# circletile/smvp-toolkit

Measured on AMD Instinct MI355X. Metric: fp64 CSR SpMV GFLOP/s (2*nnz flop per product; achieved HBM GB/s in roofline), higher is better.
Workload: dtype f64; 1 GPU; memplus.mtx x944 block-diagonal (substitute for the SURVEY 8(d) random model; that model: roofline.frac_sur...; format=csr, kernel=csr_stream_owner<8, 5, false>, nnz=119085600, rows=16763552, exchange=none

## Files before the change

### include/smvp_amd.h

```cpp
#ifndef SMVP_AMD_H
#define SMVP_AMD_H

#include <stddef.h>
#include <stdint.h>
#include <stdio.h>

#ifdef __cplusplus
extern "C" {
#endif

#define SMVP_VERSION_MAJOR 0
#define SMVP_VERSION_MINOR 6
#define SMVP_VERSION_REVISION 4

enum {
    SMVP_OK = 0,
    SMVP_ERR_INVALID = 1,
    SMVP_ERR_NO_DEVICE = 2,
    SMVP_ERR_HIP = 3,
    SMVP_ERR_ALLOC = 4,
    SMVP_ERR_IO = 5,
    SMVP_ERR_UNSUPPORTED = 6,
    SMVP_MM_COULD_NOT_READ_FILE = 11,
    SMVP_MM_PREMATURE_EOF = 12,
    SMVP_MM_NOT_MTX = 13,
    SMVP_MM_NO_HEADER = 14,
    SMVP_MM_UNSUPPORTED_TYPE = 15,
    SMVP_MM_LINE_TOO_LONG = 16,
    SMVP_MM_COULD_NOT_WRITE_FILE = 17
};
const char *smvp_last_error(void);
const char *smvp_version_string(void);
int smvp_set_option(const char *name, int value);
int smvp_get_option(const char *name, int *value);

typedef struct smvp_coo {
    int row;
    int col;
    double val;
} smvp_coo_t;

typedef char smvp_mm_typecode[4];

typedef struct smvp_time_stats {
    double time_total, time_avg, time_stdev, time_min, time_max;
} smvp_time_stats_t;

int smvp_mm_read_banner(FILE *f, smvp_mm_typecode *matcode);
int smvp_mm_read_mtx_crd_size(FILE *f, int *rows, int *cols, int *nnz);
int smvp_mm_read_coo_entries(FILE *f, const smvp_mm_typecode matcode, int nnz, smvp_coo_t *out);
int smvp_mm_read_header_path(const char *path, smvp_mm_typecode *matcode, int *rows, int *cols, int *nnz);
int smvp_mm_read_coo_path(const char *path, smvp_coo_t *out, int capacity,
                          smvp_mm_typecode *matcode, int *rows, int *cols, int *nnz);

int smvp_mm_expanded_count(const smvp_mm_typecode matcode, const smvp_coo_t *coo, int nnz, int *count);
int smvp_mm_expand_symmetric(const smvp_mm_typecode matcode, const smvp_coo_t *coo, int nnz, int rows, int cols,
                             smvp_coo_t *out, int capacity, int *nnz_out);

int smvp_cache_write_csr(const char *cache_path, const char *mtx_path, const smvp_mm_typecode matcode, int flags,
                         int rows, int cols, int nnz, const int *row_ptr, const int *col_ind, const double *val);
int smvp_cache_read_header(const char *cache_path, const char *mtx_path, smvp_mm_typecode *matcode, int *flags,
                           int *rows, int *cols, int *nnz);
int smvp_cache_read_csr(const char *cache_path, int rows, int nnz, int *row_ptr, int *col_ind, double *val);
int smvp_coo_from_csr(int rows, const int *row_ptr, const int *col_ind, const double *val, smvp_coo_t *out);

int smvp_csr_from_coo(const smvp_coo_t *coo, int rows, int nnz,
                      int *row_ptr, int *col_ind, double *val);
int smvp_tjds_from_coo(const smvp_coo_t *coo, int rows, int cols, int nnz,
                       int *perm, int *start_pos, int start_pos_capacity,
                       int *row_ind, double *val,
                       int *num_diag, int *ref_num_tjdiag, int *last_diag_single);

int smvp_csr_from_coo_device(const smvp_coo_t *d_coo, int rows, int cols, int nnz,
                             int *d_row_ptr, int *d_col_ind, double *d_val, void *stream);
int smvp_tjds_from_coo_device(const smvp_coo_t *d_coo, int rows, int cols, int nnz,
                              int *d_perm, int *d_start_pos, int start_pos_capacity,
                              int *d_row_ind, double *d_val,
                              int *num_diag, int *ref_num_tjdiag, int *last_diag_single, void *stream);

int smvp_device_count(int *count);
int smvp_device_info(int device, char *name, size_t name_cap, int *compute_units,
                     size_t *hbm_bytes);

enum {
    SMVP_CSR_KERNEL_AUTO = 0,
    SMVP_CSR_KERNEL_VECTOR = 1,
    SMVP_CSR_KERNEL_STREAM = 2,
    SMVP_CSR_KERNEL_STREAM_CARRY = 3,
    SMVP_CSR_KERNEL_COLSWEEP = 4,
    SMVP_CSR_KERNEL_BINNED = 5
};
enum {
    SMVP_MEM_HOST = 0,
    SMVP_MEM_DEVICE = 1
};

typedef struct smvp_csr smvp_csr_t;
typedef struct smvp_tjds smvp_tjds_t;

int smvp_csr_create(smvp_csr_t **out, int device, int rows, int cols, int nnz,
                    const int *row_ptr, const int *col_ind, const double *val,
                    int mem_kind, const int *host_row_ptr);
int smvp_csr_create_block(smvp_csr_t **out, int device, int rows, int cols, int nnz,
                          const int *row_ptr, const int *col_ind, const double *val,
                          int mem_kind, const int *host_row_ptr, long long first_row);
int smvp_csr_set_kernel(smvp_csr_t *h, int kernel, int param);
int smvp_csr_get_kernel(const smvp_csr_t *h, int *kernel, int *param);
int smvp_csr_gather_spread(smvp_csr_t *h, double *spread);
int smvp_csr_far_share(smvp_csr_t *h, double *share);
int smvp_csr_spmv(smvp_csr_t *h, const double *d_x, double *d_y, void *stream);
int smvp_csr_describe(const smvp_csr_t *h, char *kernel_name, size_t cap, double *alg_bytes);
int smvp_csr_plan_launches(const smvp_csr_t *h, int *launches);
typedef struct smvp_plan_info {
    double matrix_bytes;
    double plan_bytes;
    double build_ms;
} smvp_plan_info_t;
int smvp_csr_plan_info(const smvp_csr_t *h, smvp_plan_info_t *out);
int smvp_csr_spmm(smvp_csr_t *h, int k, const double *d_X, long long ldx, double *d_Y, long long ldy, void *stream);
int smvp_csr_spmm_describe(const smvp_csr_t *h, int k, char *kernel_name, size_t cap, double *alg_bytes, smvp_plan_info_t *plan);
int smvp_csr_create_transposed(smvp_csr_t **out, const smvp_csr_t *h, void *stream);
int smvp_csr_device_arrays(const smvp_csr_t *h, const int **d_row_ptr, const int **d_col_ind, const double **d_val);
void smvp_csr_destroy(smvp_csr_t *h);

int smvp_tjds_create(smvp_tjds_t **out, int device, int rows, int cols, int nnz, int num_diag,
                     const int *perm, const int *start_pos, const int *row_ind,
                     const double *val, int mem_kind);
int smvp_tjds_set_x(smvp_tjds_t *h, const double *d_x, void *stream);
int smvp_tjds_zero_y(smvp_tjds_t *h, double *d_y, void *stream);
int smvp_tjds_spmv(smvp_tjds_t *h, double *d_y, void *stream);
enum {
    SMVP_TJDS_MODE_AUTO = 0,
    SMVP_TJDS_MODE_ATOMIC = 1,
    SMVP_TJDS_MODE_TWO_PHASE = 2,
    SMVP_TJDS_MODE_ROW_GATHER = 3
};
int smvp_tjds_set_mode(smvp_tjds_t *h, int mode);
int smvp_tjds_set_tile(smvp_tjds_t *h, int entries_per_tile);
int smvp_tjds_set_value_cache(smvp_tjds_t *h, int min_tiles);
int smvp_tjds_get_value_cache(const smvp_tjds_t *h, int *min_tiles, long long *cached_entries);
int smvp_tjds_set_ref_quirks(smvp_tjds_t *h, int enable, int ref_num_tjdiag, int last_diag_single);
int smvp_tjds_describe(const smvp_tjds_t *h, char *kernel_name, size_t cap, double *alg_bytes);
int smvp_tjds_plan_info(const smvp_tjds_t *h, smvp_plan_info_t *out);
int smvp_tjds_spmv_transposed(smvp_tjds_t *h, const double *d_x, double *d_y, void *stream);
int smvp_tjds_transposed_describe(const smvp_tjds_t *h, char *kernel_name, size_t cap, double *alg_bytes);
int smvp_tjds_spmm_transposed(smvp_tjds_t *h, int k, const double *d_X, long long ldx, double *d_Y, long long ldy, void *stream);
int smvp_tjds_spmm_transposed_describe(const smvp_tjds_t *h, int k, char *kernel_name, size_t cap, double *alg_bytes);
int smvp_tjds_spmm(smvp_tjds_t *h, int k, const double *d_X, long long ldx, double *d_Y, long long ldy, void *stream);
int smvp_tjds_spmm_describe(const smvp_tjds_t *h, int k, char *kernel_name, size_t cap, double *alg_bytes, smvp_plan_info_t *plan);
void smvp_tjds_destroy(smvp_tjds_t *h);

typedef struct smvp_sharded smvp_sharded_t;
enum { SMVP_EXCHANGE_RCCL = 0, SMVP_EXCHANGE_COPIES = 1, SMVP_EXCHANGE_DIRECT = 2, SMVP_EXCHANGE_AUTO = 3 };
typedef struct smvp_shard_opts {
    unsigned struct_size;
    int chunks;
    int balance;
    int exchange;
} smvp_shard_opts_t;
void smvp_shard_opts_default(smvp_shard_opts_t *o);
int smvp_csr_sharded_create(smvp_sharded_t **out, int ngpus, const int *devices, int rows, int cols, int nnz,
                            const int *row_ptr, const int *col_ind, const double *val);
int smvp_csr_sharded_create_ex(smvp_sharded_t **out, int ngpus, const int *devices, int rows, int cols, int nnz,
                               const int *row_ptr, const int *col_ind, const double *val, const smvp_shard_opts_t *opts);
int smvp_tjds_sharded_create(smvp_sharded_t **out, int ngpus, const int *devices, const smvp_coo_t *coo,
                             int rows, int cols, int nnz);
int smvp_tjds_sharded_create_ex(smvp_sharded_t **out, int ngpus, const int *devices, const smvp_coo_t *coo,
                                int rows, int cols, int nnz, const smvp_shard_opts_t *opts);
int smvp_sharded_set_csr_kernel(smvp_sharded_t *h, int kernel, int param);
int smvp_sharded_probe_exchange(smvp_sharded_t *h, int reps);
int smvp_sharded_exchange_info(const smvp_sharded_t *h, int *active, int *available, double *ms, int *rccl_ranks);
int smvp_sharded_set_exchange(smvp_sharded_t *h, int exchange);
int smvp_sharded_set_x(smvp_sharded_t *h, const double *x_host);
enum { SMVP_GATHER_NONE = 0, SMVP_GATHER_OVERLAPPED = 1, SMVP_GATHER_AFTER = 2 };
int smvp_sharded_spmv(smvp_sharded_t *h, int allgather, int timed);
int smvp_sharded_synchronize(smvp_sharded_t *h, double *ms_of_last_timed_product);
int smvp_sharded_feed_back(smvp_sharded_t *h, int normalize);
int smvp_sharded_get_y(smvp_sharded_t *h, int slot, int gathered, double *y_host);
int smvp_sharded_info(const smvp_sharded_t *h, int *ngpus, int *rows_per_gpu);
int smvp_sharded_layout(const smvp_sharded_t *h, int *chunks, int *bounds, int *chunk_bounds);
void smvp_sharded_destroy(smvp_sharded_t *h);

#define SMVP_CSR_SWEEP_PARTS(rows_per_block, parts) ((rows_per_block) | (((parts) == 8 ? 3 : (parts) == 4 ? 2 : (parts) == 2 ? 1 : 0) << 24))
#define SMVP_CSR_SWEEP_PARAM(rows_per_block, parts, chunks) \
    (SMVP_CSR_SWEEP_PARTS(rows_per_block, parts) | (((chunks) == 4 ? 3 : (chunks) == 2 ? 2 : (chunks) == 1 ? 1 : 0) << 26))

typedef struct smvp_run_opts {
    unsigned struct_size;
    int device;
    int csr_kernel;
    int csr_param;
    int tjds_ref_quirks;
    int convert_on_device;
    int ngpus;
    int iterate;
    int normalize;
    int tjds_mode;
    int timing;
    int shard_exchange;
    int repeat_patience_us;
    const double *x;
} smvp_run_opts_t;
void smvp_run_opts_default(smvp_run_opts_t *o);

enum { SMVP_TIMING_AUTO = 0, SMVP_TIMING_EVENTS = 1, SMVP_TIMING_DEVICE = 2,
       SMVP_TIMING_DEVICE_GRAPH = 3  };
typedef struct smvp_run_info {
    int timing;
    int graph_replays;
    double wall_ms;
    double device_clock_khz;
    int repeat_launches;
    int repeat_gave_up;
} smvp_run_info_t;
int smvp_last_run_info(smvp_run_info_t *out);

int smvp_csr_compute(const smvp_coo_t *coo, int rows, int cols, int nnz, int iters,
                     const smvp_run_opts_t *opts, double *y, double *time_each_ms,
                     smvp_time_stats_t *stats);
int smvp_tjds_compute(const smvp_coo_t *coo, int rows, int cols, int nnz, int iters,
                      const smvp_run_opts_t *opts, double *y, double *time_each_ms,
                      smvp_time_stats_t *stats);

int smvp_time_stats(const double *time_each_ms, int iters, smvp_time_stats_t *out);
int smvp_generate_report_text(const char *input_file_name, const char *report_dir,
                              const char *alg_name, int nnz, int rows, int iters,
                              const double *y, const smvp_time_stats_t *stats,
                              unsigned long unix_time, char *out_path, size_t out_path_cap);

int smvp_cisr_coegen(const smvp_coo_t *coo, int rows, int nnz, int slots, FILE *out);
int smvp_cisr_coegen_path(const smvp_coo_t *coo, int rows, int nnz, int slots, const char *path);

enum {
    SMVP_SYNTH_MEMPLUS_SHAPED = 1,
    SMVP_SYNTH_UNIFORM = 2
};
int smvp_synth_row_lengths(int kind, uint64_t seed, int64_t rows_total, int64_t cols_total,
                           int param, int64_t row_begin, int64_t row_end, int *lens);
int smvp_synth_fill(int kind, uint64_t seed, int64_t rows_total, int64_t cols_total,
                    int param, int64_t row_begin, int64_t row_end, const int *row_ptr,
                    int *col_ind, double *val, int threads);
int smvp_partition_rows(const int *row_ptr, int rows, int parts, int *bounds);
int smvp_vector_random(double *x, int64_t n, uint64_t seed);

#ifdef __cplusplus
}
#endif
#endif
```

### smvp-toolkit_amd/csrc/smvp_engine.hip

```cpp
#include "smvp_engine.h"

#include <cmath>
#include <cstring>

using smvp::check_block_operands;
using smvp::check_device_indices;
using smvp::DeviceScope;
using smvp::kMaxEntries;
using smvp::refuse_capture;
using smvp::TjdsSource;
using smvp::to_device;
using smvp::upload;
using smvp::usable_device;
using smvp::wall_ms;

int smvp::usable_device(int device)
{
    int n = 0;
    if (hipGetDeviceCount(&n) != hipSuccess || n <= 0)
        return smvp::fail(SMVP_ERR_NO_DEVICE, "no HIP device is visible (this engine has no CPU path)");
    if (device < 0 || device >= n)
        return smvp::fail(SMVP_ERR_INVALID, "device %d out of range (%d visible)", device, n);
    return SMVP_OK;
}


struct TilePlan {
    int ntiles = 0;
    int *d_tile_row = nullptr;
    int *d_tile_next = nullptr;
    unsigned short *d_col16 = nullptr;
    int *d_col_base = nullptr;
    unsigned short *d_row_rel = nullptr;
    int *d_carry_row = nullptr;
    double *d_carry = nullptr;
    int *d_pos_sorted = nullptr, *d_meta = nullptr, *d_ovf_ptr = nullptr, *d_ovf_k = nullptr;
    double *d_ovf_val = nullptr;
    int *d_cache_ptr = nullptr;
    double *d_val_cache = nullptr;
    int cached_total = 0, ovf_total = 0;
    unsigned short *d_group_run = nullptr;
    unsigned *d_word32 = nullptr;
    int *d_run_ptr = nullptr, *d_run_tab = nullptr;
    int runs_total = 0;
    int sweep_alternate = 1, sweep_backward = 0;
};

struct SweepPlan {
    int rb = 0, per_launch = 0;
    int parts = 1;
    int g = 0;
    long long *d_ptr = nullptr;
    int *d_col = nullptr;
    double *d_val = nullptr;
    unsigned short *d_row = nullptr;
    double *d_part = nullptr;
};

struct BinnedSide {
    smvp::BinnedPlan bin;
    smvp_csr *near = nullptr;
    hipStream_t side = nullptr;
    hipEvent_t ev_fork = nullptr, ev_join = nullptr;
};

struct SpmmPlan {
    int *d_order = nullptr;
    bool planned = false;
    double build_ms = 0.0;
};

struct smvp_csr {
    int device = 0;
    int rows = 0, cols = 0, nnz = 0;
    long long row0 = 0;
    int *d_row_ptr = nullptr;
    int *d_col_ind = nullptr;
    double *d_val = nullptr;
    bool own_row_ptr = false, own_col_ind = false, own_val = false;
    std::vector<int> h_row_ptr;
    int max_row_len = 0;

    int flavor = smvp::kFlavorCsr;
    TjdsSource src;
    int cache_min_tiles = 2;
    bool plain_only = false;

    int kernel = SMVP_CSR_KERNEL_AUTO;
    int lanes_per_row = 64;
    int vpt = 4;
    bool tile_chosen = false;
    double spread = -2.0;
    double far_share = -2.0;
    double plan_build_ms = 0.0;

    TilePlan tile;
    SweepPlan sweep;
    BinnedSide binned;
    SpmmPlan spmm;
};

namespace {

void free_tile_plan(TilePlan *p)
{
    for (void *q : {(void *)p->d_tile_row, (void *)p->d_tile_next, (void *)p->d_col16, (void *)p->d_col_base, (void *)p->d_row_rel,
                    (void *)p->d_carry_row, (void *)p->d_carry, (void *)p->d_pos_sorted, (void *)p->d_meta, (void *)p->d_ovf_ptr,
                    (void *)p->d_ovf_k, (void *)p->d_ovf_val, (void *)p->d_cache_ptr, (void *)p->d_val_cache, (void *)p->d_group_run,
                    (void *)p->d_word32, (void *)p->d_run_ptr, (void *)p->d_run_tab})
        if (q)
            (void)hipFree(q);
    *p = TilePlan{};
}

void free_sweep_plan(SweepPlan *p)
{
    for (void *q : {(void *)p->d_ptr, (void *)p->d_col, (void *)p->d_val, (void *)p->d_row, (void *)p->d_part})
        if (q)
            (void)hipFree(q);
    *p = SweepPlan{};
}

void free_binned_side(BinnedSide *p)
{
    smvp_csr_destroy(p->near);
    smvp::free_binned_plan(&p->bin);
    if (p->side)
        (void)hipStreamDestroy(p->side);
    for (hipEvent_t e : {p->ev_fork, p->ev_join})
        if (e)
            (void)hipEventDestroy(e);
    *p = BinnedSide{};
}

void free_spmm_plan(SpmmPlan *p)
{
    if (p->d_order)
        (void)hipFree(p->d_order);
    *p = SpmmPlan{};
}

inline bool tile_ordered(int flavor) { return flavor == smvp::kFlavorTjdsS || flavor == smvp::kFlavorTjdsH; }
inline bool runs_on_tile_plan(int k) { return k != SMVP_CSR_KERNEL_VECTOR && k != SMVP_CSR_KERNEL_COLSWEEP && k != SMVP_CSR_KERNEL_BINNED; }
inline int owner_flavor(const smvp_csr *h) { return h->tile.d_col16 ? smvp::kFlavorCsr16 : h->flavor; }
inline double csr_matrix_bytes(const smvp_csr *h) { return 12.0 * h->nnz + 4.0 * (h->rows + 1.0); }
inline int sweep_strip_rows(const SweepPlan &s) { return (s.parts == smvp::kSweepXcdParts ? s.rb : s.rb * s.parts) / smvp::kSweepWaves; }

constexpr int kSweepMaxRb = 20480;
double sweep_rate(int rb)
{
    const struct { double lg, rate; } pts[] = {{10.0, 0.70}, {11.0, 0.80}, {12.0, 0.86}, {13.0, 1.0}, {14.32, 1.10}};
    constexpr int N = (int)(sizeof pts / sizeof pts[0]);
    const double lg = std::log2((double)std::max(rb, 1));
    if (lg <= pts[0].lg)
        return pts[0].rate * std::max(0.25, lg / pts[0].lg);
    for (int i = 0; i + 1 < N; ++i)
        if (lg <= pts[i + 1].lg)
            return pts[i].rate + (pts[i + 1].rate - pts[i].rate) * (lg - pts[i].lg) / (pts[i + 1].lg - pts[i].lg);
    return pts[N - 1].rate;
}

void choose_sweep_shape(int rows, int cols, int nnz, int want_rb, int *rb, int *per_launch)
{
    const double mean = rows > 0 ? std::max(1.0, (double)nnz / rows) : 1.0;
    int floor_rb = 1024;
    while (floor_rb < 8192 && (double)floor_rb * mean * 160.0 < (double)cols)
        floor_rb <<= 1;
    auto generations = [](int nrb) { return (nrb + 255) / 256; };
    std::vector<int> heights;
    for (int hgt : {kSweepMaxRb, 16384, 8192, 4096, 2048, 1024})
        if (hgt >= floor_rb)
            heights.push_back(hgt);
    for (int g = 1; g <= 16 && rows > 0; ++g) {
        const long long want = ((long long)rows + 256ll * g - 1) / (256ll * g);
        const int h4 = (int)std::min<long long>(kSweepMaxRb, (want + 3) / 4 * 4);
        if (h4 >= std::max(1024, floor_rb / 2))
            heights.push_back(h4);
    }
    int r = floor_rb;
    double best = -1.0;
    int best_gen = 1 << 30;
    for (int hgt : heights) {
        const int nrb = (rows + hgt - 1) / hgt;
        const int gen = std::max(1, generations(nrb));
        const double score = (double)nrb / (gen * 256.0) * sweep_rate(hgt);
        if (score > best * 1.01 || (score > best * 0.99 && gen < best_gen)) {
            best = std::max(best, score);
            best_gen = gen;
            r = hgt;
        }
    }
    if (want_rb > 0)
        r = want_rb;
    const int nrb = (rows + r - 1) / r;
    const int gen = std::max(1, generations(nrb));
    *rb = r;
    *per_launch = std::max(1, (nrb + gen - 1) / gen);
}

constexpr int kSweepPartsShift = 24, kSweepChunksShift = 26;
inline int sweep_param_rb(int param) { return param & ((1 << kSweepPartsShift) - 1); }
inline int sweep_param_parts(int param) { return 1 << ((param >> kSweepPartsShift) & 3); }
inline int sweep_param_chunks(int param) { const int c = (param >> kSweepChunksShift) & 3; return c == 3 ? 4 : c; }
bool sweep_param_ok(int param)
{
    const int rb = sweep_param_rb(param), parts = sweep_param_parts(param);
    if (param < 0 || (param >> (kSweepChunksShift + 2)) != 0)
        return false;
    if (rb == 0)
        return true;
    if (parts == smvp::kSweepXcdParts)
        return rb >= 256 && rb % 4 == 0 && rb <= kSweepMaxRb;
    return rb >= 256 && rb % 4 == 0 && (long long)rb * parts <= kSweepMaxRb;
}

int build_sweep_plan(smvp_csr *h, int want)
{
    SweepPlan &s = h->sweep;
    free_sweep_plan(&s);
    const int want_rb = sweep_param_rb(want);
    s.parts = sweep_param_parts(want);
    const bool xcd = s.parts == smvp::kSweepXcdParts;
    if (xcd) {
        int rb = want_rb;
        if (rb == 0) {
            const long long per_gen_max = 32ll * kSweepMaxRb;
            const long long gens = std::max<long long>(1, ((long long)h->rows + per_gen_max - 1) / per_gen_max);
            rb = (int)std::min<long long>(kSweepMaxRb, std::max<long long>(256, (((long long)h->rows + 32 * gens - 1) / (32 * gens) + 3) / 4 * 4));
        }
        s.rb = rb;
        s.per_launch = 256;
    } else {
        choose_sweep_shape(h->rows, h->cols, h->nnz, want_rb, &s.rb, &s.per_launch);
        while (s.parts > 1 && (long long)s.rb * s.parts > kSweepMaxRb)
            s.parts >>= 1;
    }
    const int strip_rows = sweep_strip_rows(s);
    s.g = smvp::sweep_chunks_in_flight(strip_rows, sweep_param_chunks(want));
    if (const hipError_t pe = smvp::prepare_csr_colsweep(); pe != hipSuccess)
        return smvp::fail(SMVP_ERR_HIP, "the column sweep cannot have its LDS: %s", hipGetErrorString(pe));
    const int nstrips = (h->rows + strip_rows - 1) / strip_rows;
    const size_t n = (size_t)std::max(h->nnz, 4);
    if (hipMalloc((void **)&s.d_ptr, ((size_t)nstrips * s.parts + 2) * sizeof(long long)) != hipSuccess ||
        hipMalloc((void **)&s.d_col, n * sizeof(int)) != hipSuccess ||
        hipMalloc((void **)&s.d_val, n * sizeof(double)) != hipSuccess ||
        hipMalloc((void **)&s.d_row, n * sizeof(unsigned short)) != hipSuccess ||
        (xcd && hipMalloc((void **)&s.d_part, sizeof(double) * smvp::kSweepXcdParts * (size_t)std::max(h->rows, 1)) != hipSuccess))
        return smvp::fail(SMVP_ERR_ALLOC, "cannot allocate the column-sweep plan (%d entries)", h->nnz);
    return smvp::build_colsweep_plan(h->d_row_ptr, h->d_col_ind, h->d_val, h->rows, h->cols, h->nnz, strip_rows, s.parts, smvp::kSweepChunk,
                                     smvp::kSweepRowBits, smvp::kSweepTurnCap, s.d_ptr, s.d_col, s.d_val, s.d_row, nullptr);
}

constexpr int kSpreadSamples = 64;
double csr_gather_spread(const smvp_csr *h)
{
    if ((long long)h->nnz < (long long)kSpreadSamples * smvp::kSpreadSpan || !h->d_col_ind)
        return -1.0;
    int *d_bits = nullptr;
    if (hipMalloc((void **)&d_bits, sizeof(int) * kSpreadSamples) != hipSuccess)
        return -1.0;
    int bits[kSpreadSamples];
    hipError_t e = smvp::launch_csr_line_spread(h->d_col_ind, h->nnz, kSpreadSamples, d_bits, nullptr);
    if (e == hipSuccess)
        e = hipMemcpy(bits, d_bits, sizeof bits, hipMemcpyDeviceToHost);
    (void)hipFree(d_bits);
    if (e != hipSuccess) {
        (void)hipGetLastError();
        return -1.0;
    }
    const double m = 512.0 * 1024.0;
    double lines = 0.0;
    for (int b : bits)
        lines += -m * std::log(std::max(1.0 - b / m, 1.0 / m));
    return std::min(1.0, lines / ((double)kSpreadSamples * smvp::kSpreadSpan));
}

constexpr double kSweepMinSpread = 0.6;

double measured_spread(smvp_csr *h)
{
    if (h->spread < -1.5)
        h->spread = h->flavor == smvp::kFlavorCsr ? csr_gather_spread(h) : -1.0;
    return h->spread;
}

double measured_far_share(smvp_csr *h)
{
    if (h->far_share < -1.5) {
        double share = -1.0;
        if (h->flavor != smvp::kFlavorCsr ||
            smvp::csr_far_share(h->d_row_ptr, h->d_col_ind, h->rows, h->nnz, smvp::kBinNearBand, h->row0, &share, nullptr) != SMVP_OK) {
            (void)hipGetLastError();
            share = -1.0;
        }
        h->far_share = share;
    }
    return h->far_share;
}

bool sweep_suits(smvp_csr *h)
{
    if (h->plain_only || h->flavor != smvp::kFlavorCsr || h->nnz < 4 * 1024 * 1024 || h->rows < 4096)
        return false;
    const double mean = (double)h->nnz / h->rows;
    if (mean < 4.0 || (double)h->cols * 8.0 < 8.0 * 1024 * 1024 || 8192.0 * mean * 160.0 < (double)h->cols ||
        (double)h->max_row_len > 256.0 * mean)
        return false;
    return measured_spread(h) >= kSweepMinSpread;
}

constexpr double kBinnedMinSpread = 0.2, kBinnedMinFarShare = 0.1;
bool binned_suits(smvp_csr *h)
{
    if (h->plain_only || h->flavor != smvp::kFlavorCsr || h->nnz < 4 * 1024 * 1024 || h->rows < 4096 ||
        (double)h->cols * 8.0 < 16.0 * 1024 * 1024)
        return false;
    return measured_spread(h) >= kBinnedMinSpread && measured_far_share(h) >= kBinnedMinFarShare;
}

void try_column_offsets(smvp_csr *h)
{
    if (h->flavor != smvp::kFlavorCsr || h->kernel != SMVP_CSR_KERNEL_STREAM || h->vpt < 4 || h->nnz <= 0 ||
        smvp::option("csr_col16", 1) == 0)
        return;
    std::vector<int> tiles;
    if (!h->tile_chosen && h->nnz >= 12 * 1024 * 1024)
        tiles.push_back(2048);
    tiles.push_back(smvp::kStreamBlock * h->vpt);
    const size_t max_tiles = ((size_t)h->nnz + 1023) / 1024 + 1;
    int *col_base = nullptr;
    unsigned short *col16 = nullptr;
    if (hipMalloc((void **)&col_base, max_tiles * sizeof(int)) == hipSuccess &&
        hipMalloc((void **)&col16, ((size_t)h->nnz + 8) * sizeof(unsigned short)) == hipSuccess) {
        for (int tile : tiles) {
            int fits = 0;
            if (smvp::build_column_offsets(h->d_col_ind, h->nnz, tile, col_base, col16, &fits, nullptr) == SMVP_OK && fits) {
                h->vpt = tile / smvp::kStreamBlock;
                h->tile.d_col_base = col_base;
                h->tile.d_col16 = col16;
                return;
            }
        }
    }
    (void)hipGetLastError();
    for (void *p : {(void *)col16, (void *)col_base})
        if (p)
            (void)hipFree(p);
}

constexpr double kSweepAlternateMinBytes = 256.0 * 1024 * 1024;

int build_tile_plan(smvp_csr *h)
{
    TilePlan &t = h->tile;
    free_tile_plan(&t);
    try_column_offsets(h);
    const int tile = smvp::kStreamBlock * h->vpt;
    const long long nnz = h->nnz;
    const int ntiles = (int)std::max<long long>(1, (nnz + tile - 1) / tile);
    std::vector<int> tile_row((size_t)ntiles + 1), carry_row((size_t)ntiles), tile_next((size_t)ntiles);
    const int *rp = h->h_row_ptr.data();
    int r = 0;
    for (int b = 0; b < ntiles; ++b) {
        const long long s = (long long)b * tile;
        const long long e = std::min(s + tile, nnz);
        while (r < h->rows && rp[r] < s)
            ++r;
        tile_row[(size_t)b] = r;
        const long long first = r < h->rows ? rp[r] : nnz;
        carry_row[(size_t)b] = (std::min(first, e) > s) ? r - 1 : -1;
    }
    tile_row[(size_t)ntiles] = h->rows;
    for (int b = 0; b < ntiles; ++b)
        tile_next[(size_t)b] = rp[tile_row[(size_t)b + 1]];
    if (int rc = upload(&t.d_tile_row, tile_row))
        return rc;
    if (h->kernel == SMVP_CSR_KERNEL_STREAM) {
        if (int rc = upload(&t.d_tile_next, tile_next))
            return rc;
        if (h->rows > 0 && smvp::option("csr_rowrel", 1) != 0) {
            std::vector<unsigned short> rel((size_t)h->rows);
            for (int b = 0; b < ntiles; ++b) {
                const long long s0 = (long long)b * tile;
                for (int rr = tile_row[(size_t)b]; rr < tile_row[(size_t)b + 1]; ++rr)
                    rel[(size_t)rr] = (unsigned short)(rp[rr] - s0);
            }
            if (int rc = upload(&t.d_row_rel, rel))
                return rc;
        }
    } else {
        if (int rc = upload(&t.d_carry_row, carry_row))
            return rc;
        HIP_TRY(hipMalloc((void **)&t.d_carry, std::max(ntiles, 1) * sizeof(double)));
        HIP_TRY(hipMemset(t.d_carry, 0, std::max(ntiles, 1) * sizeof(double)));
    }
    t.ntiles = ntiles;
    const int alternate = smvp::option("csr_sweep_alternate", -1);
    t.sweep_alternate = alternate < 0 ? 12.0 * (double)h->nnz + 12.0 * h->rows + 8.0 * h->cols > kSweepAlternateMinBytes : alternate != 0;
    if (tile_ordered(h->flavor)) {
        std::vector<int> ovf_ptr((size_t)ntiles + 1, 0);
        for (int b = 0; b < ntiles; ++b) {
            const long long e = std::min((long long)(b + 1) * tile, nnz);
            const bool owns = tile_row[(size_t)b] != tile_row[(size_t)b + 1];
            ovf_ptr[(size_t)b + 1] = ovf_ptr[(size_t)b] + (owns ? (int)(tile_next[(size_t)b] - e) : 0);
        }
        const int total = ovf_ptr[(size_t)ntiles];
        t.ovf_total = total;
        if (int rc = upload(&t.d_ovf_ptr, ovf_ptr))
            return rc;
        const size_t n = (size_t)std::max(h->nnz, 4), m = (size_t)std::max(total, 4);
        const bool half = h->flavor == smvp::kFlavorTjdsH;
        const TjdsSource &src = h->src;
        if (hipMalloc((void **)&t.d_ovf_val, m * sizeof(double)) != hipSuccess ||
            hipMalloc((void **)&t.d_ovf_k, m * sizeof(int)) != hipSuccess ||
            hipMalloc((void **)&t.d_cache_ptr, ((size_t)ntiles + 2) * sizeof(int)) != hipSuccess ||
            hipMalloc(half ? (void **)&t.d_word32 : (void **)&t.d_pos_sorted, n * sizeof(int)) != hipSuccess ||
            hipMalloc(half ? (void **)&t.d_run_ptr : (void **)&t.d_meta, (half ? (size_t)ntiles + 2 : n) * sizeof(int)) != hipSuccess)
            return smvp::fail(SMVP_ERR_ALLOC, "cannot allocate the tile-ordered TJDS streams");
        if (int rc = half ? smvp::build_tile_half_streams(src.pos, h->nnz, tile, src.start_pos, src.num_diag, h->d_val, h->cache_min_tiles,
                                                          t.d_word32, t.d_cache_ptr, t.d_run_ptr, &t.d_val_cache, &t.d_run_tab,
                                                          &t.d_group_run, &t.cached_total, &t.runs_total, nullptr)
                          : smvp::sort_tile_windows(src.pos, h->nnz, tile, src.start_pos, src.num_diag, smvp::kSlotBits, h->d_val,
                                                    h->cache_min_tiles, t.d_pos_sorted, t.d_meta, t.d_cache_ptr, &t.d_val_cache,
                                                    &t.cached_total, nullptr))
            return rc;
        if (int rc = smvp::build_tile_overflow(src.pos, t.d_ovf_ptr, total, ntiles, tile, h->nnz, src.start_pos, src.num_diag, h->d_val,
                                               t.d_ovf_val, t.d_ovf_k, src.unit_operand ? 1 : 0, nullptr))
            return rc;
    }
    return SMVP_OK;
}

int pow2_at_least(double v)
{
    int p = 2;
    while (p < 64 && p < v)
        p <<= 1;
    return p;
}

constexpr int kOwnerMaxRow = 16 * 1024;

bool choose_csr_kernel(smvp_csr *h, int kernel, int param)
{
    const double mean = h->rows > 0 ? (double)h->nnz / h->rows : 0.0;
    if (kernel == SMVP_CSR_KERNEL_AUTO)
        kernel = h->max_row_len > kOwnerMaxRow ? SMVP_CSR_KERNEL_STREAM_CARRY
                 : sweep_suits(h)              ? SMVP_CSR_KERNEL_COLSWEEP
                 : binned_suits(h)             ? SMVP_CSR_KERNEL_BINNED
                                               : SMVP_CSR_KERNEL_STREAM;
    if (kernel == SMVP_CSR_KERNEL_STREAM && param != 0 && param != 256 && param != 1024 && param != 2048)
        return false;
    if (kernel == SMVP_CSR_KERNEL_STREAM_CARRY && param != 0 && param != 1024 && param != 2048)
        return false;
    if (kernel == SMVP_CSR_KERNEL_COLSWEEP && !sweep_param_ok(param))
        return false;
    if (kernel == SMVP_CSR_KERNEL_BINNED && param < 0)
        return false;
    h->kernel = kernel;
    if (kernel == SMVP_CSR_KERNEL_COLSWEEP || kernel == SMVP_CSR_KERNEL_BINNED)
        return true;
    if (kernel == SMVP_CSR_KERNEL_VECTOR) {
        h->lanes_per_row = param > 0 ? param : pow2_at_least(mean);
    } else {
        int tile = param > 0 ? param : 0;
        h->tile_chosen = param > 0;
        if (tile == 0) {
            tile = (kernel == SMVP_CSR_KERNEL_STREAM && h->nnz < 512 * 1024) ? 256 : 1024;
            if ((tile_ordered(h->flavor)) && tile == 1024 && h->nnz >= 12 * 1024 * 1024)
                tile = 2048;
        }
        h->vpt = tile / smvp::kStreamBlock;
    }
    return true;
}

}

static int csr_create_impl(smvp_csr_t **out, int device, int rows, int cols, int nnz, const int *row_ptr, const int *col_ind, const double *val,
                           int mem_kind, const int *host_row_ptr, int flavor, const TjdsSource *src = nullptr, bool plain_only = false,
                           long long first_row = 0);

static int build_binned(smvp_csr *h, int band)
{
    free_binned_side(&h->binned);
    if (hipError_t le = smvp::binned_reserve_lds(); le != hipSuccess) {
        (void)hipGetLastError();
        return smvp::fail(SMVP_ERR_UNSUPPORTED, "the binned plan needs 154 KB of LDS per workgroup: %s", hipGetErrorString(le));
    }
    const bool window = smvp::option("binned_near", 0) == 0;
    if (int rc = smvp::build_binned_plan(h->d_row_ptr, h->d_col_ind, h->d_val, h->rows, h->cols, h->nnz, band, h->row0, window, &h->binned.bin, nullptr))
        return rc;
    if (h->binned.bin.nw.on) {
        if (smvp::option("binned_overlap", 1) != 0 && h->binned.bin.nf > 0) {
            HIP_TRY(hipStreamCreateWithFlags(&h->binned.side, hipStreamNonBlocking));
            HIP_TRY(hipEventCreateWithFlags(&h->binned.ev_fork, hipEventDisableTiming));
            HIP_TRY(hipEventCreateWithFlags(&h->binned.ev_join, hipEventDisableTiming));
        }
        return SMVP_OK;
    }
    return csr_create_impl(&h->binned.near, h->device, h->rows, h->cols, h->binned.bin.nnz_near, h->binned.bin.near_ptr, h->binned.bin.near_col, h->binned.bin.near_val,
                           SMVP_MEM_DEVICE, nullptr, smvp::kFlavorCsr, nullptr, true, h->row0);
}

static int plan_csr(smvp_csr *h, int kernel, int param, bool silent_fallback)
{
    if (!choose_csr_kernel(h, kernel, param))
        return smvp::fail(SMVP_ERR_INVALID, "entries per tile must be 256 (stream only), 1024 or 2048 for the kernel "
                                            "this matrix resolves to (column sweep: 256 ... 20480 rows per block, a multiple of 4; binned: the near band, >= 0)");
    const double t0 = wall_ms();
    free_sweep_plan(&h->sweep);
    free_binned_side(&h->binned);
    int rc = SMVP_OK;
    if (runs_on_tile_plan(h->kernel)) {
        rc = build_tile_plan(h);
    } else {
        free_tile_plan(&h->tile);
        if (h->kernel != SMVP_CSR_KERNEL_VECTOR)
            rc = h->kernel == SMVP_CSR_KERNEL_COLSWEEP ? build_sweep_plan(h, param) : build_binned(h, param);
        if (rc != SMVP_OK) {
            const std::string why = smvp_last_error();
            (void)hipGetLastError();
            free_sweep_plan(&h->sweep);
            free_binned_side(&h->binned);
            h->spread = -1.0;
            choose_csr_kernel(h, SMVP_CSR_KERNEL_STREAM, 0);
            const int tile_rc = build_tile_plan(h);
            if (tile_rc != SMVP_OK)
                free_tile_plan(&h->tile);
            rc = silent_fallback ? tile_rc : smvp::fail(rc, "%s", why.c_str());
        }
    }
    h->plan_build_ms = wall_ms() - t0;
    return rc;
}

static int csr_create_impl(smvp_csr_t **out, int device, int rows, int cols, int nnz, const int *row_ptr, const int *col_ind, const double *val,
                           int mem_kind, const int *host_row_ptr, int flavor, const TjdsSource *src, bool plain_only, long long first_row)
{
    const bool plain = flavor == smvp::kFlavorCsr;
    if (!out || rows < 0 || cols < 0 || nnz < 0 || !row_ptr ||
        (nnz > 0 && ((!col_ind && !tile_ordered(flavor)) || !val)))
        return smvp::fail(SMVP_ERR_INVALID, "smvp_csr_create: bad argument");
    if (mem_kind != SMVP_MEM_HOST && mem_kind != SMVP_MEM_DEVICE)
        return smvp::fail(SMVP_ERR_INVALID, "smvp_csr_create: bad mem_kind");
    if (nnz > kMaxEntries)
        return smvp::fail(SMVP_ERR_UNSUPPORTED, "smvp_csr_create: %d entries: shard blocks this large by rows", nnz);
    if (int rc = usable_device(device))
        return rc;
    DeviceScope on(device);

    smvp_csr *h = new smvp_csr;
    h->device = device;
    h->flavor = flavor;
    h->plain_only = plain_only;
    h->row0 = first_row;
    if (src)
        h->src = *src;
    if (h->src.unit_operand)
        h->cache_min_tiles = 0;
    h->rows = rows, h->cols = cols, h->nnz = nnz;
    h->h_row_ptr.resize((size_t)rows + 1);
    int rc = SMVP_OK;
    if (mem_kind == SMVP_MEM_HOST || host_row_ptr) {
        memcpy(h->h_row_ptr.data(), mem_kind == SMVP_MEM_HOST ? row_ptr : host_row_ptr, sizeof(int) * ((size_t)rows + 1));
    } else if (hipMemcpy(h->h_row_ptr.data(), row_ptr, sizeof(int) * ((size_t)rows + 1), hipMemcpyDeviceToHost) != hipSuccess) {
        rc = smvp::fail(SMVP_ERR_HIP, "smvp_csr_create: cannot read row_ptr back from the device");
    }
    if (rc == SMVP_OK) {
        const std::vector<int> &rp = h->h_row_ptr;
        bool ok = rp[0] == 0 && rp[(size_t)rows] == nnz;
        for (int r = 0; r < rows && ok; ++r) {
            ok = rp[(size_t)r] <= rp[(size_t)r + 1];
            h->max_row_len = std::max(h->max_row_len, rp[(size_t)r + 1] - rp[(size_t)r]);
        }
        if (!ok)
            rc = smvp::fail(SMVP_ERR_INVALID, "smvp_csr_create: row_ptr is not a non-decreasing 0..nnz sequence");
    }
    if (rc == SMVP_OK && mem_kind == SMVP_MEM_HOST) {
        for (int j = 0; j < nnz; ++j)
            if (col_ind[j] < 0 || col_ind[j] >= cols) {
                rc = smvp::fail(SMVP_ERR_INVALID, "smvp_csr_create: col_ind[%d] = %d outside [0, %d)", j, col_ind[j], cols);
                break;
            }
    }
    if (rc == SMVP_OK && mem_kind == SMVP_MEM_DEVICE &&
        (((uintptr_t)col_ind | (plain ? (uintptr_t)val : 0)) & 15u) != 0)
        rc = smvp::fail(SMVP_ERR_INVALID, "smvp_csr_create: adopted device arrays must be 16-byte aligned");
    if (rc == SMVP_OK && mem_kind == SMVP_MEM_DEVICE && col_ind)
        rc = check_device_indices(col_ind, nnz, cols, "smvp_csr_create: col_ind");
    if (rc == SMVP_OK)
        rc = to_device(&h->d_row_ptr, row_ptr, (size_t)rows + 1, mem_kind, &h->own_row_ptr);
    if (rc == SMVP_OK && col_ind)
        rc = to_device(&h->d_col_ind, col_ind, (size_t)nnz, mem_kind, &h->own_col_ind);
    if (rc == SMVP_OK)
        rc = to_device(&h->d_val, val, (size_t)nnz, mem_kind, &h->own_val);
    if (rc == SMVP_OK) {
        const double t0 = wall_ms();
        rc = plan_csr(h, plain ? SMVP_CSR_KERNEL_AUTO : SMVP_CSR_KERNEL_STREAM, 0, true);
        h->plan_build_ms = wall_ms() - t0;
    }
    if (rc != SMVP_OK) {
        smvp_csr_destroy(h);
        return rc;
    }
    *out = h;
    return SMVP_OK;
}

int smvp::csr_create_tjds(smvp_csr_t **out, int device, int rows, int cols, int nnz, const int *d_row_ptr, const int *d_col_ind,
                          const double *d_val, int flavor, const TjdsSource &src)
{
    return csr_create_impl(out, device, rows, cols, nnz, d_row_ptr, d_col_ind, d_val, SMVP_MEM_DEVICE, nullptr, flavor, &src);
}

bool smvp::csr_value_cache(const smvp_csr_t *h, int *min_tiles, long long *cached_entries)
{
    const bool on = h && tile_ordered(h->flavor);
    if (min_tiles)
        *min_tiles = on ? h->cache_min_tiles : 0;
    if (cached_entries)
        *cached_entries = on ? h->tile.cached_total : 0;
    return on;
}

int smvp::csr_replan_value_cache(smvp_csr_t *h, int min_tiles)
{
    h->cache_min_tiles = min_tiles;
    return build_tile_plan(h);
}

extern "C" int smvp_csr_create(smvp_csr_t **out, int device, int rows, int cols, int nnz,
                               const int *row_ptr, const int *col_ind, const double *val,
                               int mem_kind, const int *host_row_ptr)
{
    return csr_create_impl(out, device, rows, cols, nnz, row_ptr, col_ind, val, mem_kind, host_row_ptr, smvp::kFlavorCsr);
}

extern "C" int smvp_csr_create_block(smvp_csr_t **out, int device, int rows, int cols, int nnz,
                                     const int *row_ptr, const int *col_ind, const double *val,
                                     int mem_kind, const int *host_row_ptr, long long first_row)
{
    if (first_row < 0)
        return smvp::fail(SMVP_ERR_INVALID, "smvp_csr_create_block: first_row < 0");
    return csr_create_impl(out, device, rows, cols, nnz, row_ptr, col_ind, val, mem_kind, host_row_ptr, smvp::kFlavorCsr, nullptr,
                           false, first_row);
}

extern "C" int smvp_csr_far_share(smvp_csr_t *h, double *share)
{
    if (!h || !share)
        return smvp::fail(SMVP_ERR_INVALID, "smvp_csr_far_share: bad argument");
    DeviceScope on(h->device);
    *share = measured_far_share(h);
    return SMVP_OK;
}

extern "C" int smvp_csr_set_kernel(smvp_csr_t *h, int kernel, int param)
{
    if (!h)
        return smvp::fail(SMVP_ERR_INVALID, "null handle");
    if (h->flavor != smvp::kFlavorCsr && kernel != SMVP_CSR_KERNEL_STREAM)
        return smvp::fail(SMVP_ERR_UNSUPPORTED, "this matrix flavour runs on the stream kernel only");
    if (kernel < SMVP_CSR_KERNEL_AUTO || kernel > SMVP_CSR_KERNEL_BINNED)
        return smvp::fail(SMVP_ERR_INVALID, "unknown CSR kernel %d", kernel);
    if (kernel == SMVP_CSR_KERNEL_VECTOR && param != 0 &&
        (param < 2 || param > 64 || (param & (param - 1)) != 0))
        return smvp::fail(SMVP_ERR_INVALID, "lanes per row must be a power of two in [2, 64]");
    DeviceScope on(h->device);
    h->spread = h->far_share = -2.0;
    return plan_csr(h, kernel, param, false);
}

extern "C" int smvp_csr_get_kernel(const smvp_csr_t *h, int *kernel, int *param)
{
    if (!h)
        return smvp::fail(SMVP_ERR_INVALID, "null handle");
    if (kernel)
        *kernel = h->kernel;
    if (param)
        *param = h->kernel == SMVP_CSR_KERNEL_VECTOR ? h->lanes_per_row
                 : h->kernel == SMVP_CSR_KERNEL_COLSWEEP ? (h->sweep.rb | ((h->sweep.parts == 8 ? 3 : h->sweep.parts == 4 ? 2 : h->sweep.parts == 2 ? 1 : 0) << kSweepPartsShift))
                 : h->kernel == SMVP_CSR_KERNEL_BINNED   ? h->binned.bin.band
                                                         : h->vpt * smvp::kStreamBlock;
    return SMVP_OK;
}

extern "C" int smvp_csr_gather_spread(smvp_csr_t *h, double *spread)
{
    if (!h || !spread)
        return smvp::fail(SMVP_ERR_INVALID, "smvp_csr_gather_spread: bad argument");
    DeviceScope on(h->device);
    *spread = measured_spread(h);
    return SMVP_OK;
}

static void fill_owner_launch(const smvp_csr_t *h, const double *d_x, double *d_y, unsigned long long *stamps, smvp::OwnerLaunch *out)
{
    smvp::OwnerLaunch &l = *out;
    l.row_ptr = h->d_row_ptr, l.col_ind = h->d_col_ind, l.val = h->d_val, l.x = d_x, l.y = d_y;
    l.tile_row = h->tile.d_tile_row, l.tile_next = h->tile.d_tile_next;
    l.pos = h->src.pos, l.start_pos = h->src.start_pos;
    if (tile_ordered(h->flavor)) {
        l.pos = h->tile.d_pos_sorted, l.col_ind = h->tile.d_meta;
        l.ovf_ptr = h->tile.d_ovf_ptr, l.ovf_val = h->tile.d_ovf_val, l.ovf_k = h->tile.d_ovf_k;
        l.cache_ptr = h->tile.d_cache_ptr, l.val_cache = h->tile.d_val_cache;
        l.word32 = h->tile.d_word32, l.group_run = h->tile.d_group_run, l.run_ptr = h->tile.d_run_ptr, l.run_tab = h->tile.d_run_tab;
    }
    l.stamps = stamps;
    l.rows = h->rows, l.nnz = h->nnz, l.ntiles = h->tile.ntiles;
    l.col16 = h->tile.d_col16, l.col_base = h->tile.d_col_base;
    l.row_rel = h->tile.d_row_rel;
    l.unit_x = h->src.unit_operand ? 1 : 0;
}

int smvp::csr_repeat_grid(const smvp_csr_t *h)
{
    if (!h || h->kernel != SMVP_CSR_KERNEL_STREAM || !h->tile.d_tile_row || h->rows <= 0)
        return 0;
    DeviceScope on(h->device);
    return smvp::owner_repeat_grid(h->vpt, owner_flavor(h), h->tile.ntiles);
}

int smvp::csr_spmv_repeat(smvp_csr_t *h, const double *d_x, double *d_y, void *stream, unsigned long long *stamps, int reps, int grid,
                          unsigned *ctl_words, bool first_of_run, unsigned long long patience)
{
    DeviceScope on(h->device);
    smvp::OwnerLaunch l{};
    fill_owner_launch(h, d_x, d_y, stamps, &l);
    const hipError_t e = smvp::launch_csr_stream_owner_repeat(h->vpt, owner_flavor(h), l, reps, grid, ctl_words,
                                                              first_of_run, patience, (hipStream_t)stream);
    if (e != hipSuccess)
        return smvp::fail(SMVP_ERR_HIP, "repeating CSR launch failed: %s", hipGetErrorString(e));
    return SMVP_OK;
}

static int launched(hipError_t e)
{
    return e == hipSuccess ? (int)SMVP_OK : smvp::fail(SMVP_ERR_HIP, "CSR launch failed: %s", hipGetErrorString(e));
}

int smvp::csr_spmv_stamped(smvp_csr_t *h, const double *d_x, double *d_y, void *stream, unsigned long long *stamps)
{
    if (!h || (h->rows > 0 && !d_y) || (h->nnz > 0 && !d_x))
        return smvp::fail(SMVP_ERR_INVALID, "smvp_csr_spmv: bad argument");
    if ((h->kernel == SMVP_CSR_KERNEL_COLSWEEP && !h->sweep.d_ptr) || (h->kernel == SMVP_CSR_KERNEL_BINNED && !h->binned.near && !h->binned.bin.nw.on) ||
        (runs_on_tile_plan(h->kernel) && !h->tile.d_tile_row))
        return smvp::fail(SMVP_ERR_INVALID, "smvp_csr_spmv: the handle has no launch plan (a re-plan failed earlier)");
    DeviceScope on(h->device);
    hipStream_t st = (hipStream_t)stream;
    hipError_t e;
    if (h->kernel == SMVP_CSR_KERNEL_BINNED) {
        if (h->binned.bin.nw.on && h->binned.side) {
            HIP_TRY(hipEventRecord(h->binned.ev_fork, st));
            HIP_TRY(hipStreamWaitEvent(h->binned.side, h->binned.ev_fork, 0));
            if (int rc = launched(smvp::launch_binned_products(h->binned.bin, d_x, h->binned.side)))
                return rc;
            int rc = SMVP_OK;
            hipError_t je = hipEventRecord(h->binned.ev_join, h->binned.side);
            if (je == hipSuccess) {
                rc = launched(smvp::launch_near_window(h->binned.bin.nw, d_x, d_y, st));
                je = hipStreamWaitEvent(st, h->binned.ev_join, 0);
            }
            if (je != hipSuccess) {
                (void)hipStreamSynchronize(h->binned.side);
                return smvp::fail(SMVP_ERR_HIP, "joining the binned plan's side stream failed: %s", hipGetErrorString(je));
            }
            if (rc != SMVP_OK)
                return rc;
            return launched(smvp::launch_binned_sums(h->binned.bin, d_y, st));
        }
        if (h->binned.bin.nw.on) {
            if (int rc = launched(smvp::launch_near_window(h->binned.bin.nw, d_x, d_y, st)))
                return rc;
        } else if (int rc = smvp::csr_spmv_stamped(h->binned.near, d_x, d_y, stream, nullptr))
            return rc;
        if (int rc = launched(smvp::launch_binned_products(h->binned.bin, d_x, st)))
            return rc;
        e = smvp::launch_binned_sums(h->binned.bin, d_y, st);
    } else if (h->kernel == SMVP_CSR_KERNEL_COLSWEEP)
        e = smvp::launch_csr_colsweep(h->sweep.d_ptr, h->sweep.d_col, h->sweep.d_val, h->sweep.d_row, d_x, d_y, h->rows,
                                      sweep_strip_rows(h->sweep), h->sweep.parts, h->sweep.per_launch, h->sweep.g, h->sweep.d_part, st);
    else if (h->kernel == SMVP_CSR_KERNEL_VECTOR)
        e = smvp::launch_csr_vector(h->lanes_per_row, h->d_row_ptr, h->d_col_ind, h->d_val, d_x, d_y, h->rows, st);
    else if (h->kernel == SMVP_CSR_KERNEL_STREAM) {
        smvp::OwnerLaunch l{};
        fill_owner_launch(h, d_x, d_y, stamps, &l);
        l.backward = h->tile.sweep_backward;
        h->tile.sweep_backward = h->tile.sweep_alternate ? !l.backward : 0;
        e = smvp::launch_csr_stream_owner(h->vpt, owner_flavor(h), l, st);
    } else
        e = smvp::launch_csr_stream(h->vpt, h->d_row_ptr, h->d_col_ind, h->d_val, d_x, d_y, h->tile.d_tile_row,
                                    h->tile.d_carry_row, h->tile.d_carry, h->rows, h->nnz, h->tile.ntiles, st);
    return launched(e);
}

extern "C" int smvp_csr_spmv(smvp_csr_t *h, const double *d_x, double *d_y, void *stream)
{
    return smvp::csr_spmv_stamped(h, d_x, d_y, stream, nullptr);
}

int smvp::csr_stamp_slots(const smvp_csr_t *h)
{
    return h && h->kernel == SMVP_CSR_KERNEL_STREAM && h->tile.d_tile_row ? smvp::owner_stamp_slots(h->tile.ntiles, h->flavor) : 0;
}

std::string smvp::csr_owner_kernel_name(const smvp_csr_t *h)
{
    char name[64];
    snprintf(name, sizeof name, "csr_stream_owner<%d, %d, false>", h ? h->vpt : 0, h ? owner_flavor(h) : 0);
    return name;
}

extern "C" int smvp_csr_describe(const smvp_csr_t *h, char *kernel_name, size_t cap, double *alg_bytes)
{
    if (!h)
        return smvp::fail(SMVP_ERR_INVALID, "null handle");
    if (kernel_name && cap) {
        if (h->kernel == SMVP_CSR_KERNEL_BINNED && h->binned.bin.nw.on)
            snprintf(kernel_name, cap, "csr_binned: csr_near_window + csr_binned_far_products<2> + csr_binned_far_sums<%d, %d, 2>", h->binned.bin.slots,
                     h->binned.bin.threads_b);
        else if (h->kernel == SMVP_CSR_KERNEL_BINNED)
            snprintf(kernel_name, cap, "csr_binned: %s + csr_binned_far_products<2> + csr_binned_far_sums<%d, %d, 2>",
                     smvp::csr_owner_kernel_name(h->binned.near).c_str(), h->binned.bin.slots, h->binned.bin.threads_b);
        else if (h->kernel == SMVP_CSR_KERNEL_COLSWEEP)
            if (h->sweep.parts == smvp::kSweepXcdParts)
                snprintf(kernel_name, cap, "csr_colsweep<%d> (8 column parts, one per XCD) + sweep_combine", h->sweep.g);
            else if (h->sweep.parts > 1)
                snprintf(kernel_name, cap, "csr_colsweep<%d> (%d column parts)", h->sweep.g, h->sweep.parts);
            else
                snprintf(kernel_name, cap, "csr_colsweep<%d>", h->sweep.g);
        else if (h->kernel == SMVP_CSR_KERNEL_VECTOR)
            snprintf(kernel_name, cap, "csr_vector_rows<%d>", h->lanes_per_row);
        else if (h->kernel == SMVP_CSR_KERNEL_STREAM)
            snprintf(kernel_name, cap, "%s", smvp::csr_owner_kernel_name(h).c_str());
        else
            snprintf(kernel_name, cap, "csr_stream_tiles<%d>", h->vpt);
    }
    if (alg_bytes)
        *alg_bytes = csr_matrix_bytes(h) + 8.0 * h->cols + 8.0 * h->rows;
    return SMVP_OK;
}

extern "C" int smvp_csr_plan_launches(const smvp_csr_t *h, int *launches)
{
    if (!h || !launches)
        return smvp::fail(SMVP_ERR_INVALID, "smvp_csr_plan_launches: bad argument");
    *launches = 1;
    if (h->kernel == SMVP_CSR_KERNEL_COLSWEEP && h->sweep.rb > 0 && h->sweep.per_launch > 0) {
        const bool xcd = h->sweep.parts == smvp::kSweepXcdParts;
        const int nwg = (h->rows + h->sweep.rb - 1) / h->sweep.rb * (xcd ? smvp::kSweepXcdParts : 1);
        *launches = std::max(1, (nwg + h->sweep.per_launch - 1) / h->sweep.per_launch) + (xcd ? 1 : 0);
    } else if (h->kernel == SMVP_CSR_KERNEL_STREAM_CARRY && h->tile.ntiles > 1) {
        *launches = 2;
    } else if (h->kernel == SMVP_CSR_KERNEL_BINNED && h->binned.bin.nw.on) {
        *launches = 1 + (h->binned.bin.nw.n_out > 0 ? 1 : 0) + (h->binned.bin.nf > 0 ? 2 : 0);
    } else if (h->kernel == SMVP_CSR_KERNEL_BINNED && h->binned.near) {
        int near = 1;
        (void)smvp_csr_plan_launches(h->binned.near, &near);
        *launches = near + (h->binned.bin.nf > 0 ? 2 : 0);
    }
    return SMVP_OK;
}

double smvp::csr_plan_bytes(const smvp_csr_t *h)
{
    const double n = h->nnz, t = h->tile.ntiles;
    if (h->kernel == SMVP_CSR_KERNEL_BINNED)
        return (double)h->binned.bin.plan_bytes + (h->binned.near ? smvp::csr_plan_bytes(h->binned.near) : 0.0);
    if (h->kernel == SMVP_CSR_KERNEL_COLSWEEP) {
        const bool xcd = h->sweep.parts == smvp::kSweepXcdParts;
        const int strip_rows = std::max(1, sweep_strip_rows(h->sweep));
        return 14.0 * n + 8.0 * ((double)((h->rows + strip_rows - 1) / strip_rows) * h->sweep.parts + 2) + (xcd ? 64.0 * h->rows : 0.0);
    }
    if (h->kernel == SMVP_CSR_KERNEL_VECTOR)
        return 0.0;
    double b = 4.0 * (t + 1) + 4.0 * t;
    if (h->kernel == SMVP_CSR_KERNEL_STREAM_CARRY)
        b += 8.0 * t;
    if (h->tile.d_col16)
        b += 2.0 * n + 4.0 * (n / 1024 + 1);
    if (h->tile.d_row_rel)
        b += 2.0 * h->rows;
    if (tile_ordered(h->flavor)) {
        b += 4.0 * (t + 1) + 12.0 * h->tile.ovf_total + 4.0 * (t + 2) + 8.0 * h->tile.cached_total;
        b += h->flavor == smvp::kFlavorTjdsH ? 4.0 * n + 4.0 * (t + 2) + 8.0 * h->tile.runs_total + 2.0 * (n / 32 + 1) : 8.0 * n;
    }
    return b;
}

extern "C" int smvp_csr_plan_info(const smvp_csr_t *h, smvp_plan_info_t *out)
{
    if (!h || !out)
        return smvp::fail(SMVP_ERR_INVALID, "smvp_csr_plan_info: bad argument");
    out->matrix_bytes = csr_matrix_bytes(h);
    out->plan_bytes = smvp::csr_plan_bytes(h);
    out->build_ms = h->plan_build_ms;
    return SMVP_OK;
}

extern "C" int smvp_csr_spmm(smvp_csr_t *h, int k, const double *d_X, long long ldx, double *d_Y, long long ldy, void *stream)
{
    if (!h)
        return smvp::fail(SMVP_ERR_INVALID, "smvp_csr_spmm: null handle");
    if (h->flavor != smvp::kFlavorCsr)
        return smvp::fail(SMVP_ERR_UNSUPPORTED, "smvp_csr_spmm: plain CSR handles only (this one belongs to a TJDS matrix)");
    if (int rc = check_block_operands("smvp_csr_spmm", k, d_X, ldx, h->cols, d_Y, ldy, h->rows, h->nnz))
        return rc;
    DeviceScope on(h->device);
    hipStream_t st = (hipStream_t)stream;
    if (!h->spmm.planned) {
        if (int rc = refuse_capture(st, "smvp_csr_spmm: the first call on a handle builds its plan and cannot be captured "
                                        "(call it once outside the capture)"))
            return rc;
        const double t0 = wall_ms();
        int *order = h->spmm.d_order;
        if (h->rows > 0 && !order && hipMalloc((void **)&order, sizeof(int) * (size_t)h->rows) != hipSuccess)
            return smvp::fail(SMVP_ERR_ALLOC, "smvp_csr_spmm: cannot allocate the plan (%d rows)", h->rows);
        h->spmm.d_order = order;
        if (int rc = smvp::build_spmm_order(h->d_row_ptr, h->rows, h->max_row_len, h->spmm.d_order, st))
            return rc;
        h->spmm.planned = true;
        h->spmm.build_ms = wall_ms() - t0;
    }
    const hipError_t e = smvp::launch_csr_spmm(h->d_row_ptr, h->d_col_ind, h->d_val, h->spmm.d_order, d_X, ldx, d_Y, ldy, h->rows, k, st);
    if (e != hipSuccess)
        return smvp::fail(SMVP_ERR_HIP, "smvp_csr_spmm: launch failed: %s", hipGetErrorString(e));
    return SMVP_OK;
}

extern "C" int smvp_csr_spmm_describe(const smvp_csr_t *h, int k, char *kernel_name, size_t cap, double *alg_bytes, smvp_plan_info_t *plan)
{
    if (!h)
        return smvp::fail(SMVP_ERR_INVALID, "smvp_csr_spmm_describe: null handle");
    if (h->flavor != smvp::kFlavorCsr)
        return smvp::fail(SMVP_ERR_UNSUPPORTED, "smvp_csr_spmm_describe: plain CSR handles only");
    if (k < 1)
        return smvp::fail(SMVP_ERR_INVALID, "smvp_csr_spmm_describe: k = %d (need k >= 1)", k);
    if (kernel_name && cap)
        smvp::spmm_kernel_name(k, kernel_name, cap);
    if (alg_bytes)
        *alg_bytes = csr_matrix_bytes(h) + 8.0 * k * ((double)h->cols + h->rows);
    if (plan) {
        plan->matrix_bytes = csr_matrix_bytes(h);
        plan->plan_bytes = h->spmm.planned ? 4.0 * h->rows : 0.0;
        plan->build_ms = h->spmm.planned ? h->spmm.build_ms : 0.0;
    }
    return SMVP_OK;
}

extern "C" int smvp_csr_device_arrays(const smvp_csr_t *h, const int **d_row_ptr, const int **d_col_ind, const double **d_val)
{
    if (!h)
        return smvp::fail(SMVP_ERR_INVALID, "smvp_csr_device_arrays: null handle");
    if (h->flavor != smvp::kFlavorCsr)
        return smvp::fail(SMVP_ERR_UNSUPPORTED, "smvp_csr_device_arrays: plain CSR handles only (this one belongs to a TJDS matrix)");
    if (d_row_ptr)
        *d_row_ptr = h->d_row_ptr;
    if (d_col_ind)
        *d_col_ind = h->d_col_ind;
    if (d_val)
        *d_val = h->d_val;
    return SMVP_OK;
}

extern "C" int smvp_csr_create_transposed(smvp_csr_t **out, const smvp_csr_t *h, void *stream)
{
    if (out)
        *out = nullptr;
    if (!out || !h)
        return smvp::fail(SMVP_ERR_INVALID, "smvp_csr_create_transposed: null %s", out ? "handle" : "out");
    if (h->flavor != smvp::kFlavorCsr)
        return smvp::fail(SMVP_ERR_UNSUPPORTED, "smvp_csr_create_transposed: plain CSR handles only (this one belongs to a TJDS matrix)");
    DeviceScope on(h->device);
    hipStream_t st = (hipStream_t)stream;
    if (int rc = refuse_capture(st, "smvp_csr_create_transposed: allocates and synchronises, so it cannot be captured "
                                    "(the stream is capturing)"))
        return rc;
    const int t_rows = h->cols, t_cols = h->rows, nnz = h->nnz;
    int *t_row_ptr = nullptr, *t_col_ind = nullptr;
    double *t_val = nullptr;
    smvp_coo_t *coo = nullptr;
    auto release = [&]() {
        for (void *p : {(void *)t_row_ptr, (void *)t_col_ind, (void *)t_val, (void *)coo})
            if (p)
                (void)hipFree(p);
    };
    if (hipMalloc((void **)&t_row_ptr, sizeof(int) * ((size_t)t_rows + 4)) != hipSuccess ||
        hipMalloc((void **)&t_col_ind, sizeof(int) * std::max<size_t>((size_t)nnz, 4)) != hipSuccess ||
        hipMalloc((void **)&t_val, sizeof(double) * std::max<size_t>((size_t)nnz, 4)) != hipSuccess ||
        hipMalloc((void **)&coo, sizeof(smvp_coo_t) * std::max<size_t>((size_t)nnz, 4)) != hipSuccess) {
        (void)hipGetLastError();
        release();
        return smvp::fail(SMVP_ERR_ALLOC, "smvp_csr_create_transposed: cannot allocate the transposed arrays and the entry list (%d entries)", nnz);
    }
    int rc = SMVP_OK;
    const hipError_t e = smvp::launch_csr_swapped_coo(h->d_row_ptr, h->d_col_ind, h->d_val, h->rows, nnz, coo, st);
    if (e != hipSuccess)
        rc = smvp::fail(SMVP_ERR_HIP, "smvp_csr_create_transposed: launch failed: %s", hipGetErrorString(e));
    if (rc == SMVP_OK) {
        rc = smvp_csr_from_coo_device(coo, t_rows, t_cols, nnz, t_row_ptr, t_col_ind, t_val, stream);
        if (rc == SMVP_ERR_HIP && strstr(smvp_last_error(), "out of memory")) {
            (void)hipGetLastError();
            rc = smvp::fail(SMVP_ERR_ALLOC, "smvp_csr_create_transposed: cannot allocate the sort's buffers (%d entries)", nnz);
        }
    }
    if (rc != SMVP_OK)
        (void)hipStreamSynchronize(st);
    (void)hipFree(coo);
    coo = nullptr;
    smvp_csr_t *t = nullptr;
    if (rc == SMVP_OK)
        rc = csr_create_impl(&t, h->device, t_rows, t_cols, nnz, t_row_ptr, t_col_ind, t_val, SMVP_MEM_DEVICE, nullptr, smvp::kFlavorCsr);
    if (rc != SMVP_OK) {
        release();
        return rc;
    }
    t->own_row_ptr = t->own_col_ind = t->own_val = true;
    *out = t;
    return SMVP_OK;
}

extern "C" void smvp_csr_destroy(smvp_csr_t *h)
{
    if (!h)
        return;
    DeviceScope on(h->device);
    smvp::debug_owner_phases();
    smvp::debug_binned_phases();
    free_tile_plan(&h->tile);
    free_sweep_plan(&h->sweep);
    free_binned_side(&h->binned);
    free_spmm_plan(&h->spmm);
    if (h->own_row_ptr && h->d_row_ptr)
        (void)hipFree(h->d_row_ptr);
    if (h->own_col_ind && h->d_col_ind)
        (void)hipFree(h->d_col_ind);
    if (h->own_val && h->d_val)
        (void)hipFree(h->d_val);
    delete h;
}
```

### smvp-toolkit_amd/csrc/smvp_error.cpp

```cpp
#include "smvp_common.h"

#include <atomic>
#include <cstring>

namespace {
thread_local char g_err[512] = "";
}

namespace smvp {
int fail(int code, const char *fmt, ...)
{
    va_list ap;
    va_start(ap, fmt);
    vsnprintf(g_err, sizeof g_err, fmt, ap);
    va_end(ap);
    return code;
}
void clear_error() { g_err[0] = '\0'; }
}

extern "C" const char *smvp_last_error(void) { return g_err; }

extern "C" const char *smvp_version_string(void)
{
    static char v[32];
    snprintf(v, sizeof v, "%d.%d.%d", SMVP_VERSION_MAJOR, SMVP_VERSION_MINOR, SMVP_VERSION_REVISION);
    return v;
}

namespace {
struct Option { const char *name; std::atomic<int> value; };
Option g_options[] = {
    {"csr_col16", {-1}},
    {"csr_rowrel", {-1}},
    {"csr_sweep_alternate", {-1}},
    {"binned_near", {-1}},
    {"binned_overlap", {-1}},
    {"tjds_index", {-1}},
    {"sharded_threads", {-1}},
    {"mm_threads", {-1}},
};
Option *find_option(const char *name)
{
    if (name)
        for (Option &o : g_options)
            if (!strcmp(o.name, name))
                return &o;
    return nullptr;
}
}

namespace smvp {
int option(const char *name, int fallback)
{
    const Option *o = find_option(name);
    const int v = o ? o->value.load(std::memory_order_relaxed) : -1;
    return v < 0 ? fallback : v;
}
}

extern "C" int smvp_set_option(const char *name, int value)
{
    Option *o = find_option(name);
    if (!o)
        return smvp::fail(SMVP_ERR_INVALID, "smvp_set_option: no option called '%s'", name ? name : "(null)");
    o->value.store(value < 0 ? -1 : value, std::memory_order_relaxed);
    return SMVP_OK;
}

extern "C" int smvp_get_option(const char *name, int *value)
{
    const Option *o = find_option(name);
    if (!o || !value)
        return smvp::fail(SMVP_ERR_INVALID, "smvp_get_option: no option called '%s'", name ? name : "(null)");
    *value = o->value.load(std::memory_order_relaxed);
    return SMVP_OK;
}
```

### smvp-toolkit_amd/csrc/smvp_kernels.h

```cpp
#pragma once
#include <hip/hip_runtime.h>

#include "smvp_amd.h"
#include "smvp_tile_map.h"

namespace smvp {

constexpr int kVectorBlock = 256;
constexpr int kStreamBlock = 256;
constexpr int kLongRow = 32;
constexpr int kStreamOver = 1024;
constexpr int kStreamTileGroup = 64;
constexpr int kTjdsTileGroup = 32;
constexpr int kSweepBlock = 256;
constexpr int kSweepWaves = kSweepBlock / 64;
constexpr int kSweepUnroll = 4;
constexpr int kSweepChunk = 64 * kSweepUnroll;
constexpr int kSweepXcdParts = 8;
constexpr int kSweepRowBits = 13;
constexpr int kSweepTurnCap = (1 << (16 - kSweepRowBits)) - 1;
constexpr int kTjdsBlock = 256;
constexpr int kTjdsDiagChunk = 8;

constexpr int kSpmmMaxVectors = 16;
constexpr int kSpmmBlockRows = 4096;
int build_spmm_order(const int *row_ptr, int rows, int longest_row, int *order, hipStream_t stream);
hipError_t launch_csr_spmm(const int *row_ptr, const int *col_ind, const double *val, const int *order, const double *X,
                           long long ldx, double *Y, long long ldy, int rows, int k, hipStream_t stream);
void spmm_kernel_name(int k, char *name, size_t cap);

hipError_t launch_tjds_transposed(const int *start_pos, const int *row_ind, const double *val, const int *perm, const double *x,
                                  double *y, int cols, int num_diag, hipStream_t stream);
const char *tjds_transposed_kernel_name();
hipError_t launch_tjds_spmm_transposed(const int *start_pos, const int *row_ind, const double *val, const int *perm, const double *X,
                                       long long ldx, double *Y, long long ldy, int cols, int num_diag, int k, hipStream_t stream);
void tjds_spmm_transposed_kernel_name(int k, char *name, size_t cap);
int build_tjds_spmm_plan(const int *row_ind, const int *start_pos, const int *perm, int num_diag, int nnz, int rows, int *ptr,
                         int *pos, int *col, int *order, hipStream_t stream);
hipError_t launch_tjds_spmm(const int *ptr, const int *pos, const int *col, const double *val, const int *order, const double *X,
                            long long ldx, double *Y, long long ldy, int rows, int k, hipStream_t stream);
void tjds_spmm_kernel_name(int k, char *name, size_t cap);
hipError_t launch_csr_swapped_coo(const int *row_ptr, const int *col_ind, const double *val, int rows, int nnz, smvp_coo_t *coo,
                                  hipStream_t stream);

hipError_t launch_csr_vector(int lanes_per_row, const int *row_ptr, const int *col_ind, const double *val,
                             const double *x, double *y, int rows, hipStream_t stream);
hipError_t launch_csr_stream(int vpt, const int *row_ptr, const int *col_ind, const double *val,
                             const double *x, double *y, const int *tile_row, const int *carry_row,
                             double *carry, int rows, int nnz, int ntiles, hipStream_t stream);
constexpr int kFlavorCsr = 0;
constexpr int kFlavorTjdsK = 2;
constexpr int kFlavorTjdsS = 3;
constexpr int kFlavorTjdsH = 4;
constexpr int kFlavorCsr16 = 5;
constexpr int kSlotBits = 11;

struct OwnerLaunch {
    const int *row_ptr = nullptr, *col_ind = nullptr;
    const double *val = nullptr, *x = nullptr;
    double *y = nullptr;
    const int *tile_row = nullptr, *tile_next = nullptr;
    const int *pos = nullptr;
    const int *start_pos = nullptr;
    unsigned long long *stamps = nullptr;
    const int *ovf_ptr = nullptr, *ovf_k = nullptr;
    const double *ovf_val = nullptr;
    const int *cache_ptr = nullptr;
    const double *val_cache = nullptr;
    const unsigned short *col16 = nullptr;
    const int *col_base = nullptr;
    const unsigned short *group_run = nullptr;
    const unsigned *word32 = nullptr;
    int unit_x = 0;
    const int *run_ptr = nullptr, *run_tab = nullptr;
    const unsigned short *row_rel = nullptr;
    int rows = 0, nnz = 0, ntiles = 0;
    int backward = 0;
};
hipError_t launch_csr_stream_owner(int vpt, int flavor, const OwnerLaunch &l, hipStream_t stream);
void debug_owner_phases();
void debug_binned_phases();
int owner_stamp_slots(int ntiles, int flavor);
constexpr int kRepeatCtlWords = 32 * 66;
constexpr unsigned kRepeatPatienceDefaultUs = 50000;
int owner_repeat_grid(int vpt, int flavor, int ntiles);
hipError_t launch_owner_csr_ilp(int vpt, int flavor, const OwnerLaunch &l, const void *extra, unsigned grid_x, int group, hipStream_t stream);
hipError_t launch_csr_stream_owner_repeat(int vpt, int flavor, const OwnerLaunch &l, int reps, int grid, unsigned *ctl_words,
                                          bool first_of_run, unsigned long long patience_ticks, hipStream_t stream);
inline unsigned long long repeat_patience_ticks(int us) { return us < 0 ? 0ull : 100ull * (unsigned)(us ? us : (int)kRepeatPatienceDefaultUs); }
hipError_t launch_stamp_reduce(const unsigned long long *stamps, int slots_per_product, int products,
                               unsigned long long *first_last, hipStream_t stream);
hipError_t launch_tjds_products(const int *start_pos, const double *val, const double *x_perm, double *prod,
                                const int4 *work, int nwork, int cols, hipStream_t stream);
hipError_t launch_tjds_scatter(bool operand_by_row, const int *start_pos, const int *row_ind, const double *val,
                               const double *x_perm, double *y, const int4 *work, int nwork, int cols,
                               hipStream_t stream);
hipError_t launch_tjds_permute(const int *perm, const double *x, double *x_perm, int cols, hipStream_t stream);
hipError_t launch_find_out_of_range(const int *a, long long n, int limit, int *bad, hipStream_t stream);
hipError_t launch_normalize_max(double *v, long long n, unsigned long long *scratch, hipStream_t stream);
hipError_t launch_fill(double *p, double v, long long n, hipStream_t stream);

hipError_t launch_csr_colsweep(const long long *strip_ptr, const int *e_col, const double *e_val, const unsigned short *e_row,
                               const double *x, double *y, int rows, int strip_rows, int parts, int per_launch, int g, double *ypart,
                               hipStream_t stream);
hipError_t prepare_csr_colsweep();
int sweep_chunks_in_flight(int strip_rows, int asked);
constexpr int kSpreadSpan = 64 * 1024;
hipError_t launch_csr_line_spread(const int *col_ind, long long nnz, int samples, int *distinct, hipStream_t stream);

constexpr int kBinColBits = 14;
constexpr int kBinSlots = 8192;
constexpr int kBinRowCap = 1024;
constexpr int kBinBucket = kBinSlots - kBinRowCap;
constexpr int kBinThreads = 1024;
constexpr int kBinShiftCap = 1024;
constexpr int kBinNearBand = 4096;

struct BinnedStream {
    int groups = 0, padded = 0, cells = 0;
    unsigned short *word = nullptr;
    int *chunk = nullptr;
    int *ptr = nullptr;
    int *shift_ptr = nullptr;
    int *shift = nullptr;
};

constexpr int kNwRowBlock = 8192;
constexpr int kNwBand = 4096;
constexpr int kNwShortCap = 16;
constexpr int kNwLongCap = 1024;
struct NearWindow {
    bool on = false;
    int rows = 0, cols = 0, nblocks = 0, n_out = 0;
    long long row0 = 0;
    long long slots = 0;
    int *wave_ptr = nullptr;
    int *wave_n1 = nullptr, *wave_n2 = nullptr;
    unsigned short *perm16 = nullptr;
    double *sval = nullptr;
    unsigned short *sword = nullptr;
    int *blk_long_ptr = nullptr;
    unsigned short *long_row16 = nullptr;
    int *out_row = nullptr, *out_ptr = nullptr, *out_col = nullptr;
    double *out_val = nullptr;
    size_t plan_bytes = 0;
};
void free_near_window(NearWindow *p);
int build_near_window(const int *near_ptr, const int *near_col, const double *near_val, const int *capped, int rows, int cols,
                      int nnz_near, int band, long long row0, NearWindow *out, hipStream_t stream);
hipError_t launch_near_window(const NearWindow &p, const double *x, double *y, hipStream_t stream);

struct BinnedPlan {
    int band = kBinNearBand;
    long long row0 = 0;
    int rows = 0, cols = 0, nnz = 0, nnz_near = 0, nf = 0;
    int ncb = 0, nrb = 0, q = 1, nfr = 0, splits = 1;
    int slots = kBinSlots, threads_b = kBinThreads;
    int *near_ptr = nullptr, *near_col = nullptr;
    double *near_val = nullptr;
    NearWindow nw;
    double *a_val = nullptr;
    BinnedStream a, b;
    double *bins = nullptr;
    int *fr_row = nullptr, *fr_ptr = nullptr, *blk_fr = nullptr;
    int4 *b_desc = nullptr;
    unsigned *fr32 = nullptr;
    size_t plan_bytes = 0;
};
void free_binned_plan(BinnedPlan *p);
int build_binned_plan(const int *d_row_ptr, const int *d_col_ind, const double *d_val, int rows, int cols, int nnz, int band,
                      long long row0, bool near_window, BinnedPlan *out, hipStream_t stream);
hipError_t binned_reserve_lds();
hipError_t near_window_reserve_lds();
hipError_t launch_binned_products(const BinnedPlan &p, const double *x, hipStream_t stream);
hipError_t launch_binned_sums(const BinnedPlan &p, double *y, hipStream_t stream);
int csr_far_share(const int *d_row_ptr, const int *d_col_ind, int rows, int nnz, int band, long long row0, double *share, hipStream_t stream);

template <int N>
__device__ __forceinline__ double dpp_row_shl(double v)
{
    int lo = __double2loint(v), hi = __double2hiint(v);
    lo = __builtin_amdgcn_update_dpp(0, lo, 0x100 + N, 0xf, 0xf, true);
    hi = __builtin_amdgcn_update_dpp(0, hi, 0x100 + N, 0xf, 0xf, true);
    return __hiloint2double(hi, lo);
}

__device__ __forceinline__ double wave_sum_dpp(double v)
{
#if defined(__HIP_DEVICE_COMPILE__) && !defined(__GFX9__)
#error "wave_sum_dpp: four DPP rows of 16 lanes = one wave64 (gfx9 / CDNA only)"
#endif
    v += dpp_row_shl<8>(v);
    v += dpp_row_shl<4>(v);
    v += dpp_row_shl<2>(v);
    v += dpp_row_shl<1>(v);
    const int lo = __double2loint(v), hi = __double2hiint(v);
    double r[4];
#pragma unroll
    for (int k = 0; k < 4; ++k)
        r[k] = __hiloint2double(__builtin_amdgcn_readlane(hi, 16 * k), __builtin_amdgcn_readlane(lo, 16 * k));
    return (r[0] + r[1]) + (r[2] + r[3]);
}


}
```

### smvp-toolkit_amd/csrc/smvp_kernels.hip

```cpp
#include "smvp_kernels.h"

#include <algorithm>
#include <cstdio>
#include <cstdlib>

namespace smvp {

template <int WIDTH>
__device__ __forceinline__ double shfl_down_sum(double v)
{
#pragma unroll
    for (int off = WIDTH / 2; off > 0; off >>= 1)
        v += __shfl_down(v, off, WIDTH);
    return v;
}


#ifndef SMVP_TU_ILP
template <int T>
__global__ __launch_bounds__(kVectorBlock) void csr_vector_rows(
    const int *__restrict__ row_ptr, const int *__restrict__ col_ind, const double *__restrict__ val,
    const double *__restrict__ x, double *__restrict__ y, int rows, int row0)
{
    const long long gid = (long long)blockIdx.x * kVectorBlock + threadIdx.x;
    const long long row = row0 + gid / T;
    const int lane = threadIdx.x & (T - 1);
    int a = 0, z = 0;
    if (row < rows) {
        a = row_ptr[row];
        z = row_ptr[row + 1];
    }
    double acc = 0.0;
    for (int j = a + lane; j < z; j += T)
        acc += val[j] * x[col_ind[j]];
    acc = shfl_down_sum<T>(acc);
    if (lane == 0 && row < rows)
        y[row] = acc;
}

template <int VPT>
__global__ __launch_bounds__(kStreamBlock) void csr_stream_tiles(
    const int *__restrict__ row_ptr, const int *__restrict__ col_ind, const double *__restrict__ val,
    const double *__restrict__ x, double *__restrict__ y, const int *__restrict__ tile_row,
    double *__restrict__ carry, int rows, int nnz, int ntiles, int tile_group)
{
    constexpr int TILE = kStreamBlock * VPT;
    constexpr int QCAP = TILE / kLongRow + 1;
    __shared__ double prod[TILE];
    __shared__ int long_rows[QCAP];
    __shared__ int long_count;

    const int b = tile_of_block(blockIdx.x, tile_group);
    if (b >= ntiles)
        return;
    const int t = threadIdx.x;
    const long long s = (long long)b * TILE;
    const int e = (int)(s + TILE < (long long)nnz ? s + TILE : (long long)nnz);
    if (t == 0)
        long_count = 0;
    const int rlo = tile_row[b];
    const int rhi = tile_row[b + 1];

    const long long j0 = s + (long long)t * VPT;
    double p[VPT];
    if (j0 + VPT <= (long long)nnz) {
        int c[VPT];
        double v[VPT];
#pragma unroll
        for (int k = 0; k < VPT; k += 4)
            *reinterpret_cast<int4 *>(&c[k]) = *reinterpret_cast<const int4 *>(col_ind + j0 + k);
#pragma unroll
        for (int k = 0; k < VPT; k += 2)
            *reinterpret_cast<double2 *>(&v[k]) = *reinterpret_cast<const double2 *>(val + j0 + k);
#pragma unroll
        for (int k = 0; k < VPT; ++k)
            p[k] = v[k] * x[c[k]];
    } else {
#pragma unroll
        for (int k = 0; k < VPT; ++k)
            p[k] = (j0 + k < (long long)nnz) ? val[j0 + k] * x[col_ind[j0 + k]] : 0.0;
    }
#pragma unroll
    for (int k = 0; k < VPT; k += 2)
        *reinterpret_cast<double2 *>(&prod[t * VPT + k]) = make_double2(p[k], p[k + 1]);
    __syncthreads();

    const int lo = (int)s;
    if (t < 64) {
        const int first = rlo < rows ? row_ptr[rlo] : nnz;
        const int head = (first < e ? first : e) - lo;
        double acc = 0.0;
        for (int i = t; i < head; i += 64)
            acc += prod[i];
        acc = shfl_down_sum<64>(acc);
        if (t == 0)
            carry[b] = acc;
    }

    for (int r = rlo + t; r < rhi; r += kStreamBlock) {
        const int a = row_ptr[r];
        const int nxt = row_ptr[r + 1];
        const int z = nxt < e ? nxt : e;
        if (z - a <= kLongRow) {
            double acc = 0.0;
            for (int i = a - lo; i < z - lo; ++i)
                acc += prod[i];
            y[r] = acc;
        } else {
            long_rows[atomicAdd(&long_count, 1)] = r;
        }
    }
    __syncthreads();

    const int nlong = long_count;
    const int lane = t & 63;
    for (int q = t >> 6; q < nlong; q += kStreamBlock / 64) {
        const int r = long_rows[q];
        const int a = row_ptr[r];
        const int nxt = row_ptr[r + 1];
        const int z = nxt < e ? nxt : e;
        double acc = 0.0;
        for (int i = a - lo + lane; i < z - lo; i += 64)
            acc += prod[i];
        acc = shfl_down_sum<64>(acc);
        if (lane == 0)
            y[r] = acc;
    }
}

#endif
typedef int int4v __attribute__((ext_vector_type(4)));

struct OwnerExtra {
    const int *pos = nullptr;
    const int *start_pos = nullptr;
    const int *ovf_ptr = nullptr;
    const double *ovf_val = nullptr;
    const int *ovf_k = nullptr;
    const int *cache_ptr = nullptr;
    const double *val_cache = nullptr;
    const unsigned short *col16 = nullptr;
    const int *col_base = nullptr;
    const unsigned *word32 = nullptr;
    const unsigned short *group_run = nullptr;
    const int *run_ptr = nullptr;
    const int *run_tab = nullptr;
    int unit_x = 0;
    const unsigned short *row_rel = nullptr;
    unsigned long long *stamps = nullptr;
    int back_grid = 0;
};

[[maybe_unused]] static inline OwnerExtra owner_extra_of(const OwnerLaunch &l, unsigned long long *stamps)
{
    OwnerExtra ex{};
    ex.pos = l.pos, ex.start_pos = l.start_pos, ex.ovf_ptr = l.ovf_ptr, ex.ovf_val = l.ovf_val, ex.ovf_k = l.ovf_k;
    ex.cache_ptr = l.cache_ptr, ex.val_cache = l.val_cache;
    ex.col16 = l.col16, ex.col_base = l.col_base;
    ex.unit_x = l.unit_x, ex.word32 = l.word32, ex.group_run = l.group_run, ex.run_ptr = l.run_ptr, ex.run_tab = l.run_tab;
    ex.row_rel = l.row_rel;
    ex.stamps = stamps;
    return ex;
}

struct OwnerArgs {
    const int *__restrict__ col_ind;
    const double *__restrict__ val;
    const double *__restrict__ x;
    const int *__restrict__ pos;
    const int *__restrict__ start_pos;
    const double *__restrict__ ovf_val;
    const int *__restrict__ ovf_k;
    int unit_x;
};

template <int FLAVOR>
__device__ __forceinline__ double owner_product_slow(const OwnerArgs &a, long long j)
{
    if constexpr (FLAVOR == kFlavorCsr || FLAVOR == kFlavorCsr16)
        return a.val[j] * a.x[a.col_ind[j]];
    else if constexpr (FLAVOR == kFlavorTjdsK)
        return a.val[a.pos[j]] * a.x[a.col_ind[j]];
    else {
        const int p = a.pos[j];
        return a.val[p] * a.x[p - a.start_pos[(unsigned)a.col_ind[j] >> kSlotBits]];
    }
}

template <int FLAVOR>
__device__ __forceinline__ double owner_overflow_product(const OwnerArgs &a, int ovf_base, int e, int i)
{
    if constexpr (FLAVOR == kFlavorTjdsS || FLAVOR == kFlavorTjdsH)
        return a.unit_x ? a.val[a.ovf_k[ovf_base + i]] : a.ovf_val[ovf_base + i] * a.x[a.ovf_k[ovf_base + i]];
    else
        return owner_product_slow<FLAVOR>(a, (long long)e + i);
}

#if defined(SMVP_PHASE_STAMPS) && defined(SMVP_TU_ILP)
#undef SMVP_PHASE_STAMPS
#define SMVP_ILP_UNIT_UNUSED
#endif
#ifdef SMVP_PHASE_STAMPS
__device__ unsigned long long g_owner_phase[8];
#define SMVP_PHASE(n)                                                                        \
    do {                                                                                     \
        if (threadIdx.x == 0 && (blockIdx.x & 127) == 5) {                                   \
            const unsigned long long now_ = wall_clock64();                                  \
            if ((n) > 0)                                                                     \
                atomicAdd(&g_owner_phase[(n)-1], now_ - phase_prev_);                        \
            else                                                                             \
                atomicAdd(&g_owner_phase[7], 1ull);                                          \
            phase_prev_ = now_;                                                              \
        }                                                                                    \
    } while (0)
#else
#define SMVP_PHASE(n) do { } while (0)
#endif

#ifndef SMVP_TJDS_NEUTRALISE
#define SMVP_TJDS_NEUTRALISE 0
#endif

template <int VPT, int FLAVOR, bool STAMPED>
__device__ __forceinline__ void owner_body(
    const int *__restrict__ row_ptr, const int *__restrict__ col_ind, const double *__restrict__ val,
    const double *__restrict__ x, double *__restrict__ y, const int *__restrict__ tile_row,
    const int *__restrict__ tile_next, int rows, int nnz_arg, int ntiles, int tile_group_arg, const OwnerExtra &ex, const int block)
{
    const OwnerArgs a = {col_ind, val, x, ex.pos, ex.start_pos, ex.ovf_val, ex.ovf_k, FLAVOR == kFlavorTjdsH ? ex.unit_x : 0};
    constexpr int TILE = kStreamBlock * VPT;
    constexpr int QCAP = (TILE + kStreamOver) / kLongRow + 1;
    constexpr bool CSR = FLAVOR == kFlavorCsr || FLAVOR == kFlavorCsr16;
    constexpr bool COL16 = FLAVOR == kFlavorCsr16;
    constexpr bool HALF = FLAVOR == kFlavorTjdsH;
    constexpr bool TJDS = FLAVOR == kFlavorTjdsK || FLAVOR == kFlavorTjdsS || HALF;
    constexpr bool SORTED = FLAVOR == kFlavorTjdsS || HALF;
    static_assert(TILE <= (1 << kSlotBits), "slot bits");
    __shared__ double prod[TILE + kStreamOver];
    __shared__ int long_rows[QCAP];
    __shared__ int long_a[QCAP];
    __shared__ int long_z[QCAP];
    __shared__ int long_count;
    __shared__ double wave_sum[kStreamBlock / 64];

    const int t = threadIdx.x;
#ifdef SMVP_PHASE_STAMPS
    unsigned long long phase_prev_ = 0;
#endif
    unsigned long long *stamp = nullptr;
    if constexpr (STAMPED) {
        stamp = ex.stamps + 2 * ((size_t)block * (kStreamBlock / 64) + (t >> 6));
        if ((t & 63) == 0)
            stamp[0] = wall_clock64();
    }
#define SMVP_OWNER_EXIT()                                         \
    do {                                                          \
        if constexpr (STAMPED) {                                  \
            asm volatile("s_waitcnt vmcnt(0)" ::: "memory");      \
            if ((t & 63) == 0)                                    \
                stamp[1] = wall_clock64();                        \
        }                                                         \
        return;                                                   \
    } while (0)

    const int b = tile_of_block_swept(block, tile_group_arg, ex.back_grid);
    if (b >= ntiles)
        SMVP_OWNER_EXIT();
    const int nnz = nnz_arg;
    const long long s = (long long)b * TILE;
    const long long j0 = s + (long long)t * VPT;

    const bool whole = j0 + VPT <= (long long)nnz;
    int c[VPT];
    int pj[VPT];
    double v[VPT];
    const bool full_tile = s + TILE <= (long long)nnz;
    int grp[HALF ? VPT : 1];
    int run0 = 0;
    int2 run_tbl = make_int2(0, 0);
    if constexpr (HALF) {
        if (full_tile) {
            run0 = ex.run_ptr[b];
            const int nruns = ex.run_ptr[b + 1] - run0;
            const int ln = t & 63;
            if (ln < nruns)
                run_tbl = reinterpret_cast<const int2 *>(ex.run_tab)[run0 + ln];
        }
    }
    if constexpr (HALF) {
        if (full_tile) {
#pragma unroll
            for (int k = 0; k < VPT; ++k) {
                if constexpr (VPT == 1) {
                    pj[k] = (int)ex.word32[s + k * kStreamBlock + t];
                } else {
                    pj[k] = (int)__builtin_nontemporal_load(ex.word32 + s + k * kStreamBlock + t);
                }
                const unsigned gw = reinterpret_cast<const unsigned *>(ex.group_run)[((size_t)b * (TILE / 32) + k * (kStreamBlock / 32) +
                                                                                     2 * __builtin_amdgcn_readfirstlane(t >> 6)) >> 1];
                grp[k] = (t & 32) ? (int)(gw >> 16) : (int)(gw & 0xffffu);
            }
        }
    } else if constexpr (SORTED) {
        if (full_tile) {
#pragma unroll
            for (int k = 0; k < VPT; ++k) {
                if constexpr (VPT > 1) {
                    pj[k] = __builtin_nontemporal_load(a.pos + s + k * kStreamBlock + t);
                    c[k] = __builtin_nontemporal_load(a.col_ind + s + k * kStreamBlock + t);
                } else {
                    pj[k] = a.pos[s + k * kStreamBlock + t];
                    c[k] = a.col_ind[s + k * kStreamBlock + t];
                }
            }
        }
    } else if (whole) {
        if constexpr (VPT >= 4) {
            if constexpr (COL16) {
                const int base = ex.col_base[b];
                if (base >= 0) {
#pragma unroll
                    for (int k = 0; k < VPT; k += 4) {
                        const uint2 w = *reinterpret_cast<const uint2 *>(ex.col16 + j0 + k);
                        c[k] = base + (int)(w.x & 0xffffu), c[k + 1] = base + (int)(w.x >> 16);
                        c[k + 2] = base + (int)(w.y & 0xffffu), c[k + 3] = base + (int)(w.y >> 16);
                    }
                } else {
#pragma unroll
                    for (int k = 0; k < VPT; k += 4)
                        *reinterpret_cast<int4 *>(&c[k]) = *reinterpret_cast<const int4 *>(a.col_ind + j0 + k);
                }
            } else {
#pragma unroll
                for (int k = 0; k < VPT; k += 4)
                    *reinterpret_cast<int4 *>(&c[k]) = *reinterpret_cast<const int4 *>(a.col_ind + j0 + k);
            }
            if constexpr (TJDS) {
#pragma unroll
                for (int k = 0; k < VPT; k += 4)
                    *reinterpret_cast<int4v *>(&pj[k]) = __builtin_nontemporal_load(reinterpret_cast<const int4v *>(a.pos + j0 + k));
            }
            if constexpr (CSR) {
#pragma unroll
                for (int k = 0; k < VPT; k += 2)
                    *reinterpret_cast<double2 *>(&v[k]) = *reinterpret_cast<const double2 *>(a.val + j0 + k);
            }
        } else {
            c[0] = a.col_ind[j0];
            if constexpr (TJDS)
                pj[0] = a.pos[j0];
            if constexpr (CSR)
                v[0] = a.val[j0];
        }
    }
    const int rlo = tile_row[b];
    const int rhi = tile_row[b + 1];
    if (rlo == rhi)
        SMVP_OWNER_EXIT();
    SMVP_PHASE(0);
    const int lo = (int)s;
    const int e = (int)(s + TILE < (long long)nnz ? s + TILE : (long long)nnz);
    const int zend = tile_next[b];
    const int ext = zend - e;
    const unsigned short *__restrict__ row_rel = ex.row_rel;
    auto row_bounds = [&](int r, int &ra, int &rz) {
        if (row_rel) {
            ra = row_rel[r];
            rz = r + 1 < rhi ? (int)row_rel[r + 1] : zend - lo;
        } else {
            ra = row_ptr[r] - lo;
            rz = row_ptr[r + 1] - lo;
        }
    };
    const bool giant = ext > kStreamOver;
    if (t == 0)
        long_count = 0;
    const bool over0 = !giant && t < ext;
    double p[VPT];
    double po = 0.0;
    int rp_a = 0, rp_b = 0, rp_a2 = 0, rp_b2 = 0;
    int ovf_base = 0, cache0 = 0, in_place = 0;
    if constexpr (SORTED) {
        ovf_base = ex.ovf_ptr[b];
        cache0 = ex.cache_ptr[b];
        in_place = (e - lo) - (ex.cache_ptr[b + 1] - cache0);
    }
    if constexpr (SORTED) {
        if (full_tile && rlo + t < rhi)
            row_bounds(rlo + t, rp_a, rp_b);
        if (full_tile && rlo + t + kStreamBlock < rhi)
            row_bounds(rlo + t + kStreamBlock, rp_a2, rp_b2);
        int co = 0;
        double vo = 0.0;
        const bool unit_x = HALF && ex.unit_x;
        if (over0 && !(SMVP_TJDS_NEUTRALISE & 8)) {
            co = a.ovf_k[ovf_base + t];
            if (!unit_x)
                vo = a.ovf_val[ovf_base + t];
        }
        if (full_tile) {
            int slot[VPT];
#pragma unroll
            for (int k = 0; k < VPT; ++k) {
                if constexpr (HALF)
                    c[k] = (int)((unsigned)pj[k] >> 16), pj[k] &= 0xffff;
                slot[k] = c[k] & ((1 << kSlotBits) - 1);
                if constexpr (HALF) {
                    const int r = grp[k] + (((c[k] >> kSlotBits) - grp[k]) & 31);
                    int base = __shfl(run_tbl.x, r & 63), sub = __shfl(run_tbl.y, r & 63);
                    if (r >= 64) {
                        const int2 w = reinterpret_cast<const int2 *>(ex.run_tab)[run0 + r];
                        base = w.x, sub = w.y;
                    }
                    pj[k] += base;
                    c[k] = pj[k] - sub;
                } else {
                    c[k] = pj[k] - a.start_pos[(unsigned)c[k] >> kSlotBits];
                }
            }
            double xk[VPT];
#pragma unroll
            for (int k = 0; k < VPT; ++k) {
                const int idx = k * kStreamBlock + t;
                const double *src = idx < in_place ? a.val + pj[k] : ex.val_cache + (cache0 + (idx - in_place));
                if ((SMVP_TJDS_NEUTRALISE & 2) && idx < in_place)
                    v[k] = 1.0;
                else if ((SMVP_TJDS_NEUTRALISE & 4) && idx >= in_place)
                    v[k] = 1.0;
                else
                    v[k] = *src;
            }
            double xo = 0.0;
            if (unit_x) {
#pragma unroll
                for (int k = 0; k < VPT; ++k)
                    xk[k] = 1.0;
                if (over0)
                    vo = a.val[co], xo = 1.0;
            } else {
#pragma unroll
                for (int k = 0; k < VPT; ++k)
                    xk[k] = (SMVP_TJDS_NEUTRALISE & 1) ? 1.0 : a.x[c[k]];
                xo = over0 && !(SMVP_TJDS_NEUTRALISE & 8) ? a.x[co] : 0.0;
            }
#pragma unroll
            for (int k = 0; k < VPT; ++k)
                prod[slot[k]] = v[k] * xk[k];
            po = vo * xo;
        } else {
            for (int k = 0; k < VPT; ++k) {
                const int idx = k * kStreamBlock + t;
                if (s + idx < (long long)nnz) {
                    if constexpr (HALF) {
                        const unsigned w32 = ex.word32[s + idx];
                        const int m = (int)(w32 >> 16), g = ex.group_run[(size_t)b * (TILE / 32) + (idx >> 5)];
                        const int r = g + (((m >> kSlotBits) - g) & 31);
                        const int2 w = reinterpret_cast<const int2 *>(ex.run_tab)[ex.run_ptr[b] + r];
                        const int pw = w.x + (int)(w32 & 0xffffu);
                        const double vv = idx < in_place ? a.val[pw] : ex.val_cache[cache0 + (idx - in_place)];
                        prod[m & ((1 << kSlotBits) - 1)] = unit_x ? vv : vv * a.x[pw - w.y];
                    } else {
                        const int pw = a.pos[s + idx];
                        const double vv = idx < in_place ? a.val[pw] : ex.val_cache[cache0 + (idx - in_place)];
                        const int m = a.col_ind[s + idx];
                        prod[m & ((1 << kSlotBits) - 1)] = vv * a.x[pw - a.start_pos[(unsigned)m >> kSlotBits]];
                    }
                }
            }
            if (over0)
                po = unit_x ? a.val[co] : vo * a.x[co];
        }
    } else if (whole) {
        if (rlo + t < rhi)
            row_bounds(rlo + t, rp_a, rp_b);
        if (rlo + t + kStreamBlock < rhi)
            row_bounds(rlo + t + kStreamBlock, rp_a2, rp_b2);
        int co = 0, pjo = 0;
        double vo = 0.0;
        if (over0) {
            co = a.col_ind[e + t];
            if constexpr (TJDS)
                pjo = a.pos[e + t];
            if constexpr (CSR)
                vo = a.val[e + t];
        }
        double xk[VPT];
        if constexpr (TJDS) {
#pragma unroll
            for (int k = 0; k < VPT; ++k)
                v[k] = a.val[pj[k]];
            if (over0)
                vo = a.val[pjo];
        }
#pragma unroll
        for (int k = 0; k < VPT; ++k)
            xk[k] = a.x[c[k]];
        const double xo = over0 ? a.x[co] : 0.0;
#pragma unroll
        for (int k = 0; k < VPT; ++k)
            p[k] = v[k] * xk[k];
        po = vo * xo;
    } else {
#pragma unroll
        for (int k = 0; k < VPT; ++k)
            p[k] = (j0 + k < (long long)nnz) ? owner_product_slow<FLAVOR>(a, j0 + k) : 0.0;
        if (over0)
            po = owner_product_slow<FLAVOR>(a, e + t);
    }
    if constexpr (!SORTED) {
        if constexpr (VPT >= 2) {
#pragma unroll
            for (int k = 0; k < VPT; k += 2)
                *reinterpret_cast<double2 *>(&prod[t * VPT + k]) = make_double2(p[k], p[k + 1]);
        } else {
            prod[t] = p[0];
        }
    }
    if (over0)
        prod[e - lo + t] = po;
    if (!giant)
        for (int i = t + kStreamBlock; i < ext; i += kStreamBlock)
            prod[e - lo + i] = owner_overflow_product<FLAVOR>(a, ovf_base, e, i);
    SMVP_PHASE(1);
    __syncthreads();
    SMVP_PHASE(2);

    const int last = rhi - 1;
    auto finish_row = [&](int r, int ra, int rz) {
        if (rz - ra <= kLongRow) {
            double acc = 0.0;
            for (int i = ra; i < rz; i += 4) {
                const double v0 = prod[i], v1 = prod[i + 1 < rz ? i + 1 : i], v2 = prod[i + 2 < rz ? i + 2 : i],
                             v3 = prod[i + 3 < rz ? i + 3 : i];
                acc += v0;
                if (i + 1 < rz)
                    acc += v1;
                if (i + 2 < rz)
                    acc += v2;
                if (i + 3 < rz)
                    acc += v3;
            }
            if constexpr (VPT == 1)
                y[r] = acc;
            else
                __builtin_nontemporal_store(acc, &y[r]);
        } else {
            const int q = atomicAdd(&long_count, 1);
            long_rows[q] = r;
            long_a[q] = ra;
            long_z[q] = rz;
        }
    };
    int r_next = rlo + t;
    if (full_tile) {
        if (r_next < rhi && !(giant && r_next == last))
            finish_row(r_next, rp_a, rp_b);
        r_next += kStreamBlock;
        if (r_next < rhi && !(giant && r_next == last))
            finish_row(r_next, rp_a2, rp_b2);
        r_next += kStreamBlock;
    }
    for (int r = r_next; r < rhi; r += kStreamBlock) {
        if (giant && r == last)
            continue;
        int ra, rz;
        row_bounds(r, ra, rz);
        finish_row(r, ra, rz);
    }
    SMVP_PHASE(3);
    __syncthreads();
    SMVP_PHASE(4);

    const int nlong = long_count;
    const int lane = t & 63;
    for (int q = t >> 6; q < nlong; q += kStreamBlock / 64) {
        const int zq = long_z[q];
        double acc = 0.0;
        for (int i = long_a[q] + lane; i < zq; i += 64)
            acc += prod[i];
        acc = wave_sum_dpp(acc);
        if (lane == 0)
            y[long_rows[q]] = acc;
    }
    SMVP_PHASE(5);

    if (giant) {
        const int ra = row_ptr[last];
        double acc = 0.0;
        for (int i = ra - lo + t; i < e - lo; i += kStreamBlock)
            acc += prod[i];
        for (int j = e + t; j < zend; j += 4 * kStreamBlock) {
            double pg[4];
#pragma unroll
            for (int u = 0; u < 4; ++u) {
                const int jj = j + u * kStreamBlock;
                pg[u] = jj < zend ? owner_overflow_product<FLAVOR>(a, ovf_base, e, jj - e) : 0.0;
            }
#pragma unroll
            for (int u = 0; u < 4; ++u)
                acc += pg[u];
        }
        acc = shfl_down_sum<64>(acc);
        if (lane == 0)
            wave_sum[t >> 6] = acc;
        __syncthreads();
        if (t == 0) {
            double total = 0.0;
#pragma unroll
            for (int w = 0; w < kStreamBlock / 64; ++w)
                total += wave_sum[w];
            y[last] = total;
        }
    }
    SMVP_OWNER_EXIT();
#undef SMVP_OWNER_EXIT
}

template <int VPT, int FLAVOR, bool STAMPED>
__global__ __launch_bounds__(kStreamBlock) void csr_stream_owner(
    const int *__restrict__ row_ptr, const int *__restrict__ col_ind, const double *__restrict__ val,
    const double *__restrict__ x, double *__restrict__ y, const int *__restrict__ tile_row,
    const int *__restrict__ tile_next, int rows, int nnz_arg, int ntiles, int tile_group_arg, const OwnerExtra ex)
{
    owner_body<VPT, FLAVOR, STAMPED>(row_ptr, col_ind, val, x, y, tile_row, tile_next, rows, nnz_arg, ntiles, tile_group_arg, ex,
                                     (int)blockIdx.x);
}

#ifndef SMVP_TU_ILP
constexpr int kRepeatMaxShards = 32;
constexpr unsigned kRepeatAbort = 0x80000000u;

struct RepeatCtl {
    unsigned *sticky = nullptr;
    unsigned *shard = nullptr;
    unsigned *top = nullptr;
    unsigned *go = nullptr;
    unsigned long long *stamps = nullptr;
    int reps = 0, grid_virtual = 0, slots_per_product = 0;
    int shards = 1;
    unsigned long long patience = 0;
};

template <int VPT, int FLAVOR>
__global__ __launch_bounds__(kStreamBlock) void csr_stream_owner_repeat(
    const int *__restrict__ row_ptr, const int *__restrict__ col_ind, const double *__restrict__ val,
    const double *__restrict__ x, double *__restrict__ y, const int *__restrict__ tile_row,
    const int *__restrict__ tile_next, int rows, int nnz_arg, int ntiles, int tile_group_arg, const OwnerExtra ex, const RepeatCtl ctl)
{
    __shared__ unsigned go;
    const int t = threadIdx.x;
    const unsigned nwg = gridDim.x, me = blockIdx.x;
    const unsigned S = (unsigned)ctl.shards;
    const unsigned sh = me % S;
    const unsigned members = (nwg - sh + S - 1) / S;
    const unsigned arrivals = S > 1 ? (nwg < S ? nwg : S) : nwg;
    unsigned long long *stamp = ctl.stamps + 2 * ((size_t)me * (kStreamBlock / 64) + (t >> 6));
    if (t == 0) {
        go = __hip_atomic_load(ctl.sticky, __ATOMIC_RELAXED, __HIP_MEMORY_SCOPE_AGENT) ? 0u : 1u;
        if (!go)
            atomicOr(ctl.top, kRepeatAbort);
    }
    __syncthreads();
    if (!go)
        return;
    for (int rep = 0; rep < ctl.reps; ++rep) {
        __syncthreads();
        if (t == 0) {
            const unsigned gen = (unsigned)rep + 1u;
            const unsigned long long t0 = wall_clock64();
            unsigned seen = 0;
            if (S > 1) {
                const unsigned before = atomicAdd(ctl.shard + 32 * sh, 1u);
                if (before + 1u == members * gen) {
                    const unsigned tb = atomicAdd(ctl.top, 1u);
                    if ((tb & ~kRepeatAbort) + 1u == arrivals * gen)
                        for (unsigned q = 0; q < S; ++q)
                            __hip_atomic_fetch_max(ctl.go + 32 * q, gen, __ATOMIC_RELAXED, __HIP_MEMORY_SCOPE_AGENT);
                }
                for (;;) {
                    const unsigned g = __hip_atomic_load(ctl.go + 32 * sh, __ATOMIC_RELAXED, __HIP_MEMORY_SCOPE_AGENT);
                    if (g >= gen && g != kRepeatAbort)
                        break;
                    if (g == kRepeatAbort) {
                        seen = kRepeatAbort;
                        break;
                    }
                    if (wall_clock64() - t0 > ctl.patience) {
                        atomicOr(ctl.top, kRepeatAbort);
                        __hip_atomic_store(ctl.sticky, 1u, __ATOMIC_RELAXED, __HIP_MEMORY_SCOPE_AGENT);
                        for (unsigned q = 0; q < S; ++q)
                            __hip_atomic_fetch_max(ctl.go + 32 * q, kRepeatAbort, __ATOMIC_RELAXED, __HIP_MEMORY_SCOPE_AGENT);
                        seen = kRepeatAbort;
                        break;
                    }
                    __builtin_amdgcn_s_sleep(2);
                }
            } else {
                atomicAdd(ctl.top, 1u);
                for (;;) {
                    seen = __hip_atomic_load(ctl.top, __ATOMIC_RELAXED, __HIP_MEMORY_SCOPE_AGENT);
                    if ((seen & kRepeatAbort) || (seen & ~kRepeatAbort) >= arrivals * gen)
                        break;
                    if (wall_clock64() - t0 > ctl.patience) {
                        atomicOr(ctl.top, kRepeatAbort);
                        __hip_atomic_store(ctl.sticky, 1u, __ATOMIC_RELAXED, __HIP_MEMORY_SCOPE_AGENT);
                        seen = kRepeatAbort;
                        break;
                    }
                    __builtin_amdgcn_s_sleep(1);
                }
            }
            go = seen & kRepeatAbort ? 0u : 1u;
        }
        __syncthreads();
        if (!go)
            return;
        if ((t & 63) == 0)
            stamp[0] = wall_clock64();
        for (int vb = (int)me; vb < ctl.grid_virtual; vb += (int)nwg) {
            if (vb != (int)me)
                __syncthreads();
            owner_body<VPT, FLAVOR, false>(row_ptr, col_ind, val, x, y, tile_row, tile_next, rows, nnz_arg, ntiles, tile_group_arg, ex, vb);
        }
        asm volatile("s_waitcnt vmcnt(0)" ::: "memory");
        if ((t & 63) == 0)
            stamp[1] = wall_clock64();
        stamp += 2 * (size_t)ctl.slots_per_product;
    }
}

__global__ __launch_bounds__(256) void stamp_reduce(const unsigned long long *__restrict__ stamps, int slots_per_product,
                                                    unsigned long long *__restrict__ first_last)
{
    __shared__ unsigned long long lo_s[256 / 64], hi_s[256 / 64];
    const unsigned long long *s = stamps + (size_t)blockIdx.x * slots_per_product * 2;
    unsigned long long lo = ~0ull, hi = 0ull;
    for (int i = threadIdx.x; i < slots_per_product; i += 256) {
        const unsigned long long f = s[2 * i], l = s[2 * i + 1];
        lo = f < lo ? f : lo;
        hi = l > hi ? l : hi;
    }
#pragma unroll
    for (int off = 32; off > 0; off >>= 1) {
        const unsigned long long ol = __shfl_down(lo, off, 64), oh = __shfl_down(hi, off, 64);
        lo = ol < lo ? ol : lo;
        hi = oh > hi ? oh : hi;
    }
    if ((threadIdx.x & 63) == 0) {
        lo_s[threadIdx.x >> 6] = lo;
        hi_s[threadIdx.x >> 6] = hi;
    }
    __syncthreads();
    if (threadIdx.x == 0) {
        for (int w = 1; w < 256 / 64; ++w) {
            lo = lo_s[w] < lo ? lo_s[w] : lo;
            hi = hi_s[w] > hi ? hi_s[w] : hi;
        }
        first_last[2 * blockIdx.x] = lo;
        first_last[2 * blockIdx.x + 1] = hi;
    }
}

__global__ __launch_bounds__(256) void csr_stream_carry_fixup(
    const int *__restrict__ carry_row, const double *__restrict__ carry, double *__restrict__ y, int ntiles)
{
    const int b = blockIdx.x * 256 + threadIdx.x;
    if (b >= ntiles)
        return;
    const int r = carry_row[b];
    if (r < 0 || (b > 0 && carry_row[b - 1] == r))
        return;
    double acc = y[r];
    for (int k = b; k < ntiles && carry_row[k] == r; ++k)
        acc += carry[k];
    y[r] = acc;
}

template <bool OPERAND_BY_ROW>
__global__ __launch_bounds__(kTjdsBlock) void tjds_colmajor_scatter(
    const int *__restrict__ start_pos, const int *__restrict__ row_ind, const double *__restrict__ val,
    const double *__restrict__ x_perm, double *__restrict__ y, const int4 *__restrict__ work, int cols)
{
    const int4 w = work[blockIdx.x];
    const int k = w.x + threadIdx.x;
    const double xk = (!OPERAND_BY_ROW && k < cols) ? x_perm[k] : 0.0;
    int r[kTjdsDiagChunk];
    double v[kTjdsDiagChunk];
#pragma unroll
    for (int i = 0; i < kTjdsDiagChunk; ++i) {
        const int d = w.y + i;
        r[i] = -1;
        v[i] = 0.0;
        if (d < w.z) {
            const int base = start_pos[d];
            if (k < start_pos[d + 1] - base) {
                r[i] = row_ind[base + k];
                v[i] = val[base + k];
            }
        }
    }
#pragma unroll
    for (int i = 0; i < kTjdsDiagChunk; ++i) {
        if (r[i] >= 0) {
            const double xv = OPERAND_BY_ROW ? x_perm[r[i]] : xk;
            unsafeAtomicAdd(&y[r[i]], v[i] * xv);
        }
    }
}

__global__ __launch_bounds__(kTjdsBlock) void tjds_colmajor_products(
    const int *__restrict__ start_pos, const double *__restrict__ val, const double *__restrict__ x_perm,
    double *__restrict__ prod, const int4 *__restrict__ work, int cols)
{
    const int4 w = work[blockIdx.x];
    const int k = w.x + threadIdx.x;
    const double xk = k < cols ? x_perm[k] : 0.0;
    int j[kTjdsDiagChunk];
    double v[kTjdsDiagChunk];
#pragma unroll
    for (int i = 0; i < kTjdsDiagChunk; ++i) {
        const int d = w.y + i;
        j[i] = -1;
        v[i] = 0.0;
        if (d < w.z) {
            const int base = start_pos[d];
            if (k < start_pos[d + 1] - base) {
                j[i] = base + k;
                v[i] = val[base + k];
            }
        }
    }
#pragma unroll
    for (int i = 0; i < kTjdsDiagChunk; ++i)
        if (j[i] >= 0)
            __builtin_nontemporal_store(v[i] * xk, &prod[j[i]]);
}

__global__ __launch_bounds__(256) void tjds_permute_operand(
    const int *__restrict__ perm, const double *__restrict__ x, double *__restrict__ x_perm, int cols)
{
    const int k = blockIdx.x * 256 + threadIdx.x;
    if (k < cols)
        x_perm[k] = x[perm[k]];
}

__global__ __launch_bounds__(256) void find_out_of_range(const int *__restrict__ a, long long n, int limit,
                                                          int *__restrict__ bad)
{
    const long long stride = (long long)gridDim.x * 256;
    for (long long i = (long long)blockIdx.x * 256 + threadIdx.x; i < n; i += stride) {
        const int v = a[i];
        if (v < 0 || v >= limit)
            atomicMax(bad, (int)(i < 2147483646ll ? i + 1 : 2147483647ll));
    }
}

__global__ __launch_bounds__(256) void vector_absmax(const double *__restrict__ v, long long n,
                                                      unsigned long long *__restrict__ bits)
{
    double m = 0.0;
    const long long stride = (long long)gridDim.x * 256;
    for (long long i = (long long)blockIdx.x * 256 + threadIdx.x; i < n; i += stride) {
        const double a = fabs(v[i]);
        m = a > m ? a : m;
    }
#pragma unroll
    for (int off = 32; off > 0; off >>= 1) {
        const double o = __shfl_down(m, off, 64);
        m = o > m ? o : m;
    }
    if ((threadIdx.x & 63) == 0)
        atomicMax(bits, (unsigned long long)__double_as_longlong(m));
}

__global__ __launch_bounds__(256) void vector_divide(double *__restrict__ v, long long n,
                                                      const unsigned long long *__restrict__ bits)
{
    const double m = __longlong_as_double((long long)*bits);
    const long long i = (long long)blockIdx.x * 256 + threadIdx.x;
    if (i < n && m > 0.0)
        v[i] = v[i] / m;
}

__global__ __launch_bounds__(256) void fill_value(double *__restrict__ p, double v, long long n)
{
    const long long i = (long long)blockIdx.x * 256 + threadIdx.x;
    if (i < n)
        p[i] = v;
}

static hipError_t launch_csr_vector_rows(int lanes_per_row, const int *row_ptr, const int *col_ind, const double *val,
                                         const double *x, double *y, int rows, int row0, int n, hipStream_t stream)
{
    const unsigned grid = (unsigned)(((long long)n * lanes_per_row + kVectorBlock - 1) / kVectorBlock);
#define SMVP_VEC_CASE(T)                                                                              \
    case T:                                                                                           \
        hipLaunchKernelGGL(csr_vector_rows<T>, dim3(grid), dim3(kVectorBlock), 0, stream, row_ptr,   \
                           col_ind, val, x, y, rows, row0);                                           \
        break;
    switch (lanes_per_row) {
        SMVP_VEC_CASE(2)
        SMVP_VEC_CASE(4)
        SMVP_VEC_CASE(8)
        SMVP_VEC_CASE(16)
        SMVP_VEC_CASE(32)
        SMVP_VEC_CASE(64)
    default:
        return hipErrorInvalidValue;
    }
#undef SMVP_VEC_CASE
    return hipGetLastError();
}

hipError_t launch_csr_vector(int lanes_per_row, const int *row_ptr, const int *col_ind, const double *val,
                             const double *x, double *y, int rows, hipStream_t stream)
{
    if (lanes_per_row < 1)
        return hipErrorInvalidValue;
    const int chunk = (int)(((long long)1 << 31) / lanes_per_row);
    for (int row0 = 0; row0 < rows; row0 += chunk) {
        const int n = std::min(chunk, rows - row0);
        if (hipError_t e = launch_csr_vector_rows(lanes_per_row, row_ptr, col_ind, val, x, y, rows, row0, n, stream))
            return e;
        if (rows - row0 <= chunk)
            break;
    }
    return hipSuccess;
}

static int tile_group(int ntiles, int wanted = kStreamTileGroup) { return tile_group_of(ntiles, wanted); }

hipError_t launch_csr_stream(int vpt, const int *row_ptr, const int *col_ind, const double *val,
                             const double *x, double *y, const int *tile_row, const int *carry_row,
                             double *carry, int rows, int nnz, int ntiles, hipStream_t stream)
{
    if (rows <= 0)
        return hipSuccess;
    const int group = tile_group(ntiles);
    const dim3 grid((unsigned)((ntiles + 8 * group - 1) / (8 * group)) * 8u * group);
    switch (vpt) {
    case 4:
        hipLaunchKernelGGL(csr_stream_tiles<4>, grid, dim3(kStreamBlock), 0, stream, row_ptr, col_ind, val, x, y,
                           tile_row, carry, rows, nnz, ntiles, group);
        break;
    case 8:
        hipLaunchKernelGGL(csr_stream_tiles<8>, grid, dim3(kStreamBlock), 0, stream, row_ptr, col_ind, val, x, y,
                           tile_row, carry, rows, nnz, ntiles, group);
        break;
    default:
        return hipErrorInvalidValue;
    }
    hipError_t e = hipGetLastError();
    if (e != hipSuccess)
        return e;
    if (ntiles > 1) {
        hipLaunchKernelGGL(csr_stream_carry_fixup, dim3((ntiles + 255) / 256), dim3(256), 0, stream, carry_row,
                           carry, y, ntiles);
        e = hipGetLastError();
    }
    return e;
}

static unsigned owner_grid(int ntiles, int group) { return tile_grid_of(ntiles, group); }

static int flavor_group(int flavor) { return flavor == kFlavorTjdsS || flavor == kFlavorTjdsH ? kTjdsTileGroup : kStreamTileGroup; }

int owner_stamp_slots(int ntiles, int flavor)
{
    return (int)owner_grid(ntiles, tile_group(ntiles, flavor_group(flavor))) * (kStreamBlock / 64);
}

hipError_t launch_csr_stream_owner(int vpt, int flavor, const OwnerLaunch &l, hipStream_t stream)
{
    if (l.rows <= 0)
        return hipSuccess;
    const int group = tile_group(l.ntiles, flavor_group(flavor));
    const dim3 grid(owner_grid(l.ntiles, group));
    OwnerExtra ex = owner_extra_of(l, l.stamps);
    ex.back_grid = l.backward ? (int)grid.x : 0;
#define SMVP_OWNER_ST(V, F, S)                                                                                     \
    hipLaunchKernelGGL((csr_stream_owner<V, F, S>), grid, dim3(kStreamBlock), 0, stream, l.row_ptr, l.col_ind, l.val, \
                       l.x, l.y, l.tile_row, l.tile_next, l.rows, l.nnz, l.ntiles, group, ex)
#define SMVP_OWNER(V, F)                  \
    if (vpt == V && flavor == F) {        \
        if (l.stamps)                     \
            SMVP_OWNER_ST(V, F, true);    \
        else                              \
            SMVP_OWNER_ST(V, F, false);   \
        return hipGetLastError();         \
    }
#ifdef SMVP_PHASE_STAMPS
    SMVP_OWNER(1, kFlavorCsr)
    SMVP_OWNER(4, kFlavorCsr)
    SMVP_OWNER(8, kFlavorCsr)
    SMVP_OWNER(4, kFlavorCsr16)
    SMVP_OWNER(8, kFlavorCsr16)
#else
    if (flavor == kFlavorCsr || flavor == kFlavorCsr16)
        return launch_owner_csr_ilp(vpt, flavor, l, &ex, grid.x, group, stream);
#endif
    SMVP_OWNER(1, kFlavorTjdsK)
    SMVP_OWNER(4, kFlavorTjdsK)
    SMVP_OWNER(8, kFlavorTjdsK)
    SMVP_OWNER(1, kFlavorTjdsS)
    SMVP_OWNER(4, kFlavorTjdsS)
    SMVP_OWNER(8, kFlavorTjdsS)
    SMVP_OWNER(1, kFlavorTjdsH)
    SMVP_OWNER(4, kFlavorTjdsH)
    SMVP_OWNER(8, kFlavorTjdsH)
#undef SMVP_OWNER
#undef SMVP_OWNER_ST
    return hipErrorInvalidValue;
}

template <int V, int F>
static int repeat_capacity()
{
    int per_cu = 0, dev = 0, cus = 0;
    if (hipOccupancyMaxActiveBlocksPerMultiprocessor(&per_cu, csr_stream_owner_repeat<V, F>, kStreamBlock, 0) != hipSuccess ||
        hipGetDevice(&dev) != hipSuccess || hipDeviceGetAttribute(&cus, hipDeviceAttributeMultiprocessorCount, dev) != hipSuccess) {
        (void)hipGetLastError();
        return 0;
    }
    return per_cu > 1 ? (per_cu - 1) * cus * 3 / 4 : 0;
}

#define SMVP_REPEAT_FORMS(X) \
    X(1, kFlavorCsr) X(4, kFlavorCsr) X(8, kFlavorCsr) X(4, kFlavorCsr16) X(8, kFlavorCsr16) \
    X(1, kFlavorTjdsS) X(4, kFlavorTjdsS) X(8, kFlavorTjdsS) X(1, kFlavorTjdsH) X(4, kFlavorTjdsH) X(8, kFlavorTjdsH)

int owner_repeat_grid(int vpt, int flavor, int ntiles)
{
    if (ntiles <= 0)
        return 0;
    int cap = 0;
#define X(V, F)                     \
    if (vpt == V && flavor == F)    \
        cap = repeat_capacity<V, F>();
    SMVP_REPEAT_FORMS(X)
#undef X
    if (cap <= 0)
        return 0;
    const int full = (int)owner_grid(ntiles, tile_group(ntiles, flavor_group(flavor)));
    return full <= cap ? full : 0;
}

hipError_t launch_csr_stream_owner_repeat(int vpt, int flavor, const OwnerLaunch &l, int reps, int grid, unsigned *ctl_words,
                                          bool first_of_run, unsigned long long patience_ticks, hipStream_t stream)
{
    if (l.rows <= 0)
        return hipSuccess;
    const int group = tile_group(l.ntiles, flavor_group(flavor));
    RepeatCtl ctl{};
    ctl.sticky = ctl_words;
    ctl.shard = ctl_words + 32, ctl.go = ctl_words + 32 * (1 + kRepeatMaxShards), ctl.top = ctl_words + kRepeatCtlWords - 32;
    ctl.shards = grid <= 24 ? 1 : grid <= 640 ? 8 : 16;
    ctl.stamps = l.stamps;
    ctl.reps = reps, ctl.grid_virtual = (int)owner_grid(l.ntiles, group), ctl.slots_per_product = grid * (kStreamBlock / 64);
    ctl.patience = patience_ticks;
    if (reps <= 0 || grid <= 0 || ctl.grid_virtual <= 0 || !ctl.stamps || !ctl_words)
        return hipErrorInvalidValue;
    static_assert(kRepeatCtlWords == 32 * (2 + 2 * kRepeatMaxShards), "sticky + shards + go words + top, one 128-byte line each");
    hipError_t e = first_of_run ? hipMemsetAsync(ctl_words, 0, sizeof(unsigned) * kRepeatCtlWords, stream)
                                : hipMemsetAsync(ctl_words + 32, 0, sizeof(unsigned) * (kRepeatCtlWords - 32), stream);
    if (e != hipSuccess)
        return e;
    const OwnerExtra ex = owner_extra_of(l, nullptr);
#define X(V, F)                                                                                                                    \
    if (vpt == V && flavor == F) {                                                                                                 \
        hipLaunchKernelGGL((csr_stream_owner_repeat<V, F>), dim3((unsigned)grid), dim3(kStreamBlock), 0, stream, l.row_ptr, l.col_ind, \
                           l.val, l.x, l.y, l.tile_row, l.tile_next, l.rows, l.nnz, l.ntiles, group, ex, ctl);                     \
        return hipGetLastError();                                                                                                  \
    }
    SMVP_REPEAT_FORMS(X)
#undef X
    return hipErrorInvalidValue;
}

#ifdef SMVP_PHASE_STAMPS
void debug_owner_phases()
{
    unsigned long long h[8] = {0, 0, 0, 0, 0, 0, 0, 0}, z[8] = {0, 0, 0, 0, 0, 0, 0, 0};
    if (hipMemcpyFromSymbol(h, HIP_SYMBOL(g_owner_phase), sizeof h) != hipSuccess || h[7] == 0)
        return;
    const double n = (double)h[7];
    fprintf(stderr, "[owner dbg] mean us per workgroup over %.0f: loads + gathers + LDS writes %.2f | barrier %.2f | lane-per-row sums %.2f | "
                    "barrier %.2f | long rows %.2f\n", n, h[0] * 0.01 / n, h[1] * 0.01 / n, h[2] * 0.01 / n, h[3] * 0.01 / n, h[4] * 0.01 / n);
    (void)hipMemcpyToSymbol(HIP_SYMBOL(g_owner_phase), z, sizeof z);
}
#else
void debug_owner_phases() {}
#endif

hipError_t launch_stamp_reduce(const unsigned long long *stamps, int slots_per_product, int products,
                               unsigned long long *first_last, hipStream_t stream)
{
    if (products <= 0)
        return hipSuccess;
    hipLaunchKernelGGL(stamp_reduce, dim3(products), dim3(256), 0, stream, stamps, slots_per_product, first_last);
    return hipGetLastError();
}

hipError_t launch_tjds_products(const int *start_pos, const double *val, const double *x_perm, double *prod,
                                const int4 *work, int nwork, int cols, hipStream_t stream)
{
    if (nwork <= 0)
        return hipSuccess;
    hipLaunchKernelGGL(tjds_colmajor_products, dim3(nwork), dim3(kTjdsBlock), 0, stream, start_pos, val, x_perm, prod,
                       work, cols);
    return hipGetLastError();
}

hipError_t launch_tjds_scatter(bool operand_by_row, const int *start_pos, const int *row_ind, const double *val,
                               const double *x_perm, double *y, const int4 *work, int nwork, int cols,
                               hipStream_t stream)
{
    if (nwork <= 0)
        return hipSuccess;
    if (operand_by_row)
        hipLaunchKernelGGL(tjds_colmajor_scatter<true>, dim3(nwork), dim3(kTjdsBlock), 0, stream, start_pos,
                           row_ind, val, x_perm, y, work, cols);
    else
        hipLaunchKernelGGL(tjds_colmajor_scatter<false>, dim3(nwork), dim3(kTjdsBlock), 0, stream, start_pos,
                           row_ind, val, x_perm, y, work, cols);
    return hipGetLastError();
}

hipError_t launch_tjds_permute(const int *perm, const double *x, double *x_perm, int cols, hipStream_t stream)
{
    if (cols <= 0)
        return hipSuccess;
    hipLaunchKernelGGL(tjds_permute_operand, dim3((cols + 255) / 256), dim3(256), 0, stream, perm, x, x_perm, cols);
    return hipGetLastError();
}

hipError_t launch_find_out_of_range(const int *a, long long n, int limit, int *bad, hipStream_t stream)
{
    if (n <= 0)
        return hipSuccess;
    const long long want = (n + 255) / 256;
    hipLaunchKernelGGL(find_out_of_range, dim3((unsigned)(want < 8192 ? want : 8192)), dim3(256), 0, stream, a, n,
                       limit, bad);
    return hipGetLastError();
}

hipError_t launch_normalize_max(double *v, long long n, unsigned long long *scratch, hipStream_t stream)
{
    if (n <= 0)
        return hipSuccess;
    hipError_t e = hipMemsetAsync(scratch, 0, sizeof(unsigned long long), stream);
    if (e != hipSuccess)
        return e;
    const long long want = (n + 255) / 256;
    hipLaunchKernelGGL(vector_absmax, dim3((unsigned)(want < 2048 ? want : 2048)), dim3(256), 0, stream, v, n, scratch);
    hipLaunchKernelGGL(vector_divide, dim3((unsigned)want), dim3(256), 0, stream, v, n, scratch);
    return hipGetLastError();
}

hipError_t launch_fill(double *p, double v, long long n, hipStream_t stream)
{
    if (n <= 0)
        return hipSuccess;
    hipLaunchKernelGGL(fill_value, dim3((unsigned)((n + 255) / 256)), dim3(256), 0, stream, p, v, n);
    return hipGetLastError();
}

#else
#ifdef SMVP_ILP_UNIT_UNUSED
hipError_t launch_owner_csr_ilp(int, int, const OwnerLaunch &, const void *, unsigned, int, hipStream_t) { return hipErrorInvalidValue; }
#else
hipError_t launch_owner_csr_ilp(int vpt, int flavor, const OwnerLaunch &l, const void *extra, unsigned grid_x, int group, hipStream_t stream)
{
    const OwnerExtra &ex = *static_cast<const OwnerExtra *>(extra);
    const dim3 grid(grid_x);
#define SMVP_OWNER_ST(V, F, S)                                                                                     \
    hipLaunchKernelGGL((csr_stream_owner<V, F, S>), grid, dim3(kStreamBlock), 0, stream, l.row_ptr, l.col_ind, l.val, \
                       l.x, l.y, l.tile_row, l.tile_next, l.rows, l.nnz, l.ntiles, group, ex)
#define SMVP_OWNER(V, F)                  \
    if (vpt == V && flavor == F) {        \
        if (l.stamps)                     \
            SMVP_OWNER_ST(V, F, true);    \
        else                              \
            SMVP_OWNER_ST(V, F, false);   \
        return hipGetLastError();         \
    }
    SMVP_OWNER(1, kFlavorCsr)
    SMVP_OWNER(4, kFlavorCsr)
    SMVP_OWNER(8, kFlavorCsr)
    SMVP_OWNER(4, kFlavorCsr16)
    SMVP_OWNER(8, kFlavorCsr16)
#undef SMVP_OWNER
#undef SMVP_OWNER_ST
    return hipErrorInvalidValue;
}
#endif
#endif

}

namespace smvp {

#ifdef SMVP_TU_ILP
template <int G>
__global__ __launch_bounds__(kSweepBlock) void csr_colsweep(
    const long long *__restrict__ strip_ptr, const int *__restrict__ e_col, const double *__restrict__ e_val,
    const unsigned short *__restrict__ e_row, const double *__restrict__ x, double *__restrict__ y, int rows, int strip_rows,
    int nstrips, int wg_first, int parts, double *__restrict__ ypart, long long ypart_stride)
{
    constexpr int U = kSweepUnroll, E = G * U;
    constexpr long long STEP = (long long)G * kSweepChunk;
    extern __shared__ double sums_all[];
    const int lane = threadIdx.x & 63;
    const int wave = __builtin_amdgcn_readfirstlane((int)threadIdx.x >> 6);
    int strip = (wg_first + (int)blockIdx.x) * kSweepWaves + wave;
    bool live = strip < nstrips * parts;
    long long part_rows0 = -1;
    if (parts == kSweepXcdParts) {
        const int b = wg_first + (int)blockIdx.x, part = b % kSweepXcdParts, real = (b / kSweepXcdParts) * kSweepWaves + wave;
        live = real < nstrips;
        strip = real * kSweepXcdParts + part;
        part_rows0 = (long long)part * ypart_stride + (long long)real * strip_rows;
        if (!live)
            return;
    }
    if (!live && parts == 1)
        return;
    typedef __attribute__((address_space(3))) volatile double lds_double;
    lds_double *sums = (lds_double *)sums_all + (size_t)wave * strip_rows;
    const long long a = live ? strip_ptr[strip] : 0, z = live ? strip_ptr[strip + 1] : 0;

    auto fetch = [&](long long base, int (&c)[E], double (&v)[E], int (&w)[E]) {
        if (base + STEP <= z) {
#pragma unroll
            for (int e = 0; e < E; ++e) {
                const long long j = base + e * 64 + lane;
                c[e] = __builtin_nontemporal_load(e_col + j);
                v[e] = __builtin_nontemporal_load(e_val + j);
                w[e] = __builtin_nontemporal_load(e_row + j);
            }
        } else {
#pragma unroll
            for (int e = 0; e < E; ++e) {
                const long long j = base + e * 64 + lane;
                const bool in = j < z;
                c[e] = in ? e_col[j] : 0;
                v[e] = in ? e_val[j] : 0.0;
                w[e] = in ? (int)e_row[j] : -1;
            }
        }
    };
    int c[E], w[E];
    double v[E];
    if (a < z)
        fetch(a, c, v, w);
    for (int i = lane; i < strip_rows; i += 64)
        sums[i] = 0.0;
    for (long long base = a; base < z; base += STEP) {
        double p[E];
#pragma unroll
        for (int e = 0; e < E; ++e)
            p[e] = x[c[e]];
        int cn[E], wn[E];
        double vn[E];
        if (base + STEP < z)
            fetch(base + STEP, cn, vn, wn);
#pragma unroll
        for (int e = 0; e < E; ++e)
            p[e] = v[e] * p[e];
#pragma unroll
        for (int g = 0; g < G; ++g) {
            int row[U], turn[U];
#pragma unroll
            for (int u = 0; u < U; ++u) {
                row[u] = w[g * U + u] < 0 ? 0 : w[g * U + u] & ((1 << kSweepRowBits) - 1);
                turn[u] = w[g * U + u] >> kSweepRowBits;
            }
            for (int k = 0;; ++k) {
                double cur[U];
                bool later = false;
#pragma unroll
                for (int u = 0; u < U; ++u)
                    cur[u] = sums[row[u]];
#pragma unroll
                for (int u = 0; u < U; ++u) {
                    if (turn[u] == k)
                        sums[row[u]] = cur[u] + p[g * U + u];
                    later = later || (turn[u] > k && turn[u] < kSweepTurnCap);
                }
                if (!__any(later))
                    break;
            }
#pragma unroll
            for (int u = 0; u < U; ++u) {
                unsigned long long m = __ballot(turn[u] == kSweepTurnCap);
                while (m) {
                    const int l = __ffsll((long long)m) - 1;
                    if (lane == l)
                        sums[row[u]] = sums[row[u]] + p[g * U + u];
                    m &= m - 1;
                }
            }
        }
#pragma unroll
        for (int e = 0; e < E; ++e) {
            c[e] = cn[e];
            v[e] = vn[e];
            w[e] = wn[e];
        }
    }
    if (parts == kSweepXcdParts) {
        const long long r0 = part_rows0 - (part_rows0 / ypart_stride) * ypart_stride;
        for (int i = lane; i < strip_rows && r0 + i < rows; i += 64)
            ypart[part_rows0 + i] = sums[i];
        return;
    }
    if (parts == 1) {
        const long long r0 = (long long)strip * strip_rows;
        for (int i = lane; i < strip_rows && r0 + i < rows; i += 64)
            __builtin_nontemporal_store(sums[i], &y[r0 + i]);
        return;
    }
    __syncthreads();
    const int strips_here = kSweepWaves / parts;
    lds_double *all = (lds_double *)sums_all;
    for (int s = 0; s < strips_here; ++s) {
        const long long r0 = ((long long)(wg_first + (int)blockIdx.x) * strips_here + s) * strip_rows;
        for (int i = (int)threadIdx.x; i < strip_rows && r0 + i < rows; i += kSweepBlock) {
            double acc = all[(size_t)(s * parts) * strip_rows + i];
            for (int q = 1; q < parts; ++q)
                acc += all[(size_t)(s * parts + q) * strip_rows + i];
            __builtin_nontemporal_store(acc, &y[r0 + i]);
        }
    }
}

__global__ __launch_bounds__(256) void sweep_combine(const double *__restrict__ ypart, long long stride, double *__restrict__ y, int rows)
{
    const long long r = (long long)blockIdx.x * 256 + threadIdx.x;
    if (r >= rows)
        return;
    double acc = ypart[r];
#pragma unroll
    for (int q = 1; q < kSweepXcdParts; ++q)
        acc += ypart[(long long)q * stride + r];
    __builtin_nontemporal_store(acc, &y[r]);
}

int sweep_chunks_in_flight(int strip_rows, int asked)
{
    return asked == 1 || asked == 2 || asked == 4 ? asked : (strip_rows >= 768 ? 2 : 1);
}

constexpr size_t kSweepMaxLds = 160u * 1024;
hipError_t prepare_csr_colsweep()
{
    for (const void *f : {(const void *)csr_colsweep<1>, (const void *)csr_colsweep<2>, (const void *)csr_colsweep<4>}) {
        const hipError_t e = hipFuncSetAttribute(f, hipFuncAttributeMaxDynamicSharedMemorySize, (int)kSweepMaxLds);
        if (e != hipSuccess)
            return e;
    }
    return hipSuccess;
}

hipError_t launch_csr_colsweep(const long long *strip_ptr, const int *e_col, const double *e_val, const unsigned short *e_row,
                               const double *x, double *y, int rows, int strip_rows, int parts, int per_launch, int g, double *ypart,
                               hipStream_t stream)
{
    if (rows <= 0)
        return hipSuccess;
    const bool xcd = parts == kSweepXcdParts;
    if ((parts != 1 && parts != 2 && parts != 4 && !xcd) || (xcd && (!ypart || (per_launch > 0 && per_launch % kSweepXcdParts != 0))))
        return hipErrorInvalidValue;
    const int nstrips = (rows + strip_rows - 1) / strip_rows;
    const int nwg = xcd ? (nstrips + kSweepWaves - 1) / kSweepWaves * kSweepXcdParts
                        : (int)(((long long)nstrips * parts + kSweepWaves - 1) / kSweepWaves);
    const long long ypart_stride = rows;
    const size_t lds = sizeof(double) * (size_t)strip_rows * kSweepWaves;
    if (per_launch <= 0)
        per_launch = nwg;
    if (lds > kSweepMaxLds)
        return hipErrorInvalidValue;
    for (int first = 0; first < nwg; first += per_launch) {
        const unsigned grid = (unsigned)(nwg - first < per_launch ? nwg - first : per_launch);
#define SMVP_SWEEP(GG)                                                                                                   \
    hipLaunchKernelGGL(csr_colsweep<GG>, dim3(grid), dim3(kSweepBlock), lds, stream, strip_ptr, e_col, e_val, e_row, x, y, \
                       rows, strip_rows, nstrips, first, parts, ypart, ypart_stride)
        if (g == 4)
            SMVP_SWEEP(4);
        else if (g == 2)
            SMVP_SWEEP(2);
        else
            SMVP_SWEEP(1);
#undef SMVP_SWEEP
    }
    if (xcd)
        hipLaunchKernelGGL(sweep_combine, dim3((unsigned)((rows + 255) / 256)), dim3(256), 0, stream, ypart, ypart_stride, y, rows);
    return hipGetLastError();
}

#else
__global__ __launch_bounds__(1024) void csr_line_spread(const int *__restrict__ col_ind, long long nnz, int samples,
                                                        int *__restrict__ set_bits)
{
    constexpr int WORDS = 16 * 1024;
    __shared__ unsigned map[WORDS];
    __shared__ int total;
    for (int i = threadIdx.x; i < WORDS; i += 1024)
        map[i] = 0u;
    if (threadIdx.x == 0)
        total = 0;
    __syncthreads();
    const long long first = samples > 1 ? (nnz - kSpreadSpan) / (samples - 1) * blockIdx.x : 0;
    for (int i = threadIdx.x; i < kSpreadSpan; i += 1024) {
        const long long j = first + i;
        if (j < nnz) {
            const unsigned line = (unsigned)col_ind[j] >> 4;
            const unsigned h = (line * 2654435761u) >> (32 - 19);
            atomicOr(&map[h >> 5], 1u << (h & 31));
        }
    }
    __syncthreads();
    int n = 0;
    for (int i = threadIdx.x; i < WORDS; i += 1024)
        n += __popc(map[i]);
    atomicAdd(&total, n);
    __syncthreads();
    if (threadIdx.x == 0)
        set_bits[blockIdx.x] = total;
}

hipError_t launch_csr_line_spread(const int *col_ind, long long nnz, int samples, int *set_bits, hipStream_t stream)
{
    if (samples <= 0 || nnz < kSpreadSpan)
        return hipErrorInvalidValue;
    hipLaunchKernelGGL(csr_line_spread, dim3(samples), dim3(1024), 0, stream, col_ind, nnz, samples, set_bits);
    return hipGetLastError();
}

#endif

}
```

### smvp-toolkit_amd/csrc/smvp_tile_map.h

```cpp
#pragma once

#if defined(__HIPCC__)
#define SMVP_HOST_DEVICE __host__ __device__
#else
#define SMVP_HOST_DEVICE
#endif

namespace smvp {

inline int tile_group_of(int ntiles, int wanted)
{
    const int fit = ntiles / 64;
    return fit < 1 ? 1 : (fit < wanted ? fit : wanted);
}

inline unsigned tile_grid_of(int ntiles, int group) { return (unsigned)((ntiles + 8 * group - 1) / (8 * group)) * 8u * group; }

SMVP_HOST_DEVICE inline __attribute__((always_inline)) int tile_of_block(int block, int group)
{
    const int xcd = block & 7, seq = block >> 3;
    return (seq / group) * (8 * group) + xcd * group + seq % group;
}

SMVP_HOST_DEVICE inline __attribute__((always_inline)) int tile_of_block_swept(int block, int group, int back_grid)
{
    return tile_of_block(back_grid ? back_grid - 1 - block : block, group);
}

}
```

### smvp-toolkit_amd/python/smvp_toolkit_amd/__init__.py

```python
import ctypes as C
import os

import numpy as np

_HERE = os.path.dirname(os.path.abspath(__file__))
PKG_ROOT = os.path.dirname(os.path.dirname(_HERE))
REPO_ROOT = os.path.dirname(PKG_ROOT)
LIB_PATH = os.environ.get("SMVP_LIB_PATH") or os.path.join(PKG_ROOT, "lib", "libsmvp_amd.so")
CLI_PATH = os.path.join(PKG_ROOT, "bin", "smvp-toolkit-cli")

OK = 0
ERR_INVALID, ERR_NO_DEVICE, ERR_HIP, ERR_ALLOC, ERR_IO, ERR_UNSUPPORTED = 1, 2, 3, 4, 5, 6
MM_COULD_NOT_READ_FILE, MM_PREMATURE_EOF, MM_NOT_MTX, MM_NO_HEADER, MM_UNSUPPORTED_TYPE = 11, 12, 13, 14, 15
CSR_KERNEL_AUTO, CSR_KERNEL_VECTOR, CSR_KERNEL_STREAM, CSR_KERNEL_STREAM_CARRY, CSR_KERNEL_COLSWEEP = 0, 1, 2, 3, 4
CSR_KERNEL_BINNED = 5
MEM_HOST, MEM_DEVICE = 0, 1
SYNTH_MEMPLUS_SHAPED, SYNTH_UNIFORM = 1, 2
TJDS_MODE_AUTO, TJDS_MODE_ATOMIC, TJDS_MODE_TWO_PHASE, TJDS_MODE_ROW_GATHER = 0, 1, 2, 3
TIMING_AUTO, TIMING_EVENTS, TIMING_DEVICE, TIMING_DEVICE_GRAPH = 0, 1, 2, 3
MAX_ENTRIES = 2 ** 31 - 1 - 65536

COO_DTYPE = np.dtype([("row", "<i4"), ("col", "<i4"), ("val", "<f8")], align=True)


def set_option(name, value):
    _check(lib().smvp_set_option(name.encode(), -1 if value is None else int(value)), "smvp_set_option")


def get_option(name):
    v = C.c_int()
    _check(lib().smvp_get_option(name.encode(), C.byref(v)), "smvp_get_option")
    return v.value


class option:

    def __init__(self, name, value):
        self.name, self.value = name, value

    def __enter__(self):
        self.old = get_option(self.name)
        set_option(self.name, self.value)
        return self

    def __exit__(self, *exc):
        set_option(self.name, self.old)
        return False


def sweep_parts(rows_per_block, parts, chunks=0):
    return int(rows_per_block) | ({1: 0, 2: 1, 4: 2, 8: 3}[int(parts)] << 24) | ({0: 0, 1: 1, 2: 2, 4: 3}[int(chunks)] << 26)


class TimeStats(C.Structure):
    _fields_ = [(n, C.c_double) for n in ("time_total", "time_avg", "time_stdev", "time_min", "time_max")]


class RunOpts(C.Structure):
    _fields_ = [("struct_size", C.c_uint), ("device", C.c_int), ("csr_kernel", C.c_int), ("csr_param", C.c_int),
                ("tjds_ref_quirks", C.c_int), ("convert_on_device", C.c_int), ("ngpus", C.c_int),
                ("iterate", C.c_int), ("normalize", C.c_int), ("tjds_mode", C.c_int), ("timing", C.c_int),
                ("shard_exchange", C.c_int), ("repeat_patience_us", C.c_int), ("x", C.c_void_p)]


class PlanInfo(C.Structure):
    _fields_ = [("matrix_bytes", C.c_double), ("plan_bytes", C.c_double), ("build_ms", C.c_double)]


class RunInfo(C.Structure):
    _fields_ = [("timing", C.c_int), ("graph_replays", C.c_int), ("wall_ms", C.c_double), ("device_clock_khz", C.c_double),
                ("repeat_launches", C.c_int), ("repeat_gave_up", C.c_int)]


class ShardOpts(C.Structure):
    _fields_ = [("struct_size", C.c_uint), ("chunks", C.c_int), ("balance", C.c_int), ("exchange", C.c_int)]


GATHER_NONE, GATHER_OVERLAPPED, GATHER_AFTER = 0, 1, 2
EXCHANGE_RCCL, EXCHANGE_COPIES, EXCHANGE_DIRECT, EXCHANGE_AUTO = 0, 1, 2, 3
EXCHANGE_NAMES = {EXCHANGE_RCCL: "rccl", EXCHANGE_COPIES: "copies", EXCHANGE_DIRECT: "direct", EXCHANGE_AUTO: "auto"}


class SmvpError(RuntimeError):
    def __init__(self, code, where, msg=None):
        self.code = code
        if msg is None:
            msg = lib().smvp_last_error().decode(errors="replace")
        super().__init__("%s failed with status %d: %s" % (where, code, msg))


def _check_entries(nnz, where):
    if nnz > MAX_ENTRIES:
        raise SmvpError(ERR_UNSUPPORTED, where, "%d entries: more than the %d a matrix may hold" % (nnz, MAX_ENTRIES))


_lib = None

EXPORTS = [
    "smvp_last_error", "smvp_version_string", "smvp_set_option", "smvp_get_option",
    "smvp_mm_read_banner", "smvp_mm_read_mtx_crd_size", "smvp_mm_read_coo_entries",
    "smvp_mm_read_header_path", "smvp_mm_read_coo_path", "smvp_mm_expanded_count", "smvp_mm_expand_symmetric",
    "smvp_cache_write_csr", "smvp_cache_read_header", "smvp_cache_read_csr", "smvp_coo_from_csr",
    "smvp_csr_from_coo", "smvp_tjds_from_coo", "smvp_csr_from_coo_device", "smvp_tjds_from_coo_device",
    "smvp_device_count", "smvp_device_info", "smvp_csr_plan_info", "smvp_tjds_plan_info",
    "smvp_csr_create", "smvp_csr_create_block", "smvp_csr_far_share", "smvp_csr_set_kernel", "smvp_csr_get_kernel", "smvp_csr_gather_spread", "smvp_csr_spmv",
    "smvp_csr_describe", "smvp_csr_plan_launches", "smvp_csr_destroy", "smvp_csr_spmm", "smvp_csr_spmm_describe",
    "smvp_csr_create_transposed", "smvp_csr_device_arrays", "smvp_tjds_spmv_transposed", "smvp_tjds_transposed_describe",
    "smvp_tjds_spmm_transposed", "smvp_tjds_spmm_transposed_describe", "smvp_tjds_spmm", "smvp_tjds_spmm_describe",
    "smvp_tjds_create", "smvp_tjds_set_x", "smvp_tjds_zero_y", "smvp_tjds_spmv",
    "smvp_tjds_set_ref_quirks", "smvp_tjds_set_mode", "smvp_tjds_set_tile", "smvp_tjds_set_value_cache", "smvp_tjds_get_value_cache", "smvp_tjds_describe", "smvp_tjds_destroy",
    "smvp_shard_opts_default", "smvp_csr_sharded_create", "smvp_csr_sharded_create_ex", "smvp_tjds_sharded_create",
    "smvp_tjds_sharded_create_ex", "smvp_sharded_layout", "smvp_sharded_set_csr_kernel", "smvp_sharded_probe_exchange", "smvp_sharded_exchange_info", "smvp_sharded_set_exchange", "smvp_sharded_set_x", "smvp_sharded_spmv",
    "smvp_sharded_synchronize", "smvp_sharded_feed_back", "smvp_sharded_get_y", "smvp_sharded_info", "smvp_sharded_destroy",
    "smvp_run_opts_default", "smvp_csr_compute", "smvp_tjds_compute", "smvp_last_run_info",
    "smvp_time_stats", "smvp_generate_report_text", "smvp_cisr_coegen", "smvp_cisr_coegen_path",
    "smvp_synth_row_lengths", "smvp_synth_fill", "smvp_partition_rows", "smvp_vector_random",
]


def lib():
    global _lib
    if _lib is None:
        if not os.path.exists(LIB_PATH):
            raise RuntimeError("%s is missing: run `python -c 'import __graft_entry__ as g; g.build()'` "
                               "or `make -C smvp-toolkit_amd` first" % LIB_PATH)
        L = C.CDLL(LIB_PATH)
        L.smvp_last_error.restype = C.c_char_p
        L.smvp_version_string.restype = C.c_char_p
        L.smvp_set_option.argtypes = [C.c_char_p, C.c_int]
        L.smvp_get_option.argtypes = [C.c_char_p, C.POINTER(C.c_int)]
        vp, ci = C.c_void_p, C.c_int
        L.smvp_csr_create.argtypes = [C.POINTER(vp), ci, ci, ci, ci, vp, vp, vp, ci, vp]
        L.smvp_csr_create_block.argtypes = [C.POINTER(vp), ci, ci, ci, ci, vp, vp, vp, ci, vp, C.c_longlong]
        L.smvp_csr_far_share.argtypes = [vp, C.POINTER(C.c_double)]
        L.smvp_csr_set_kernel.argtypes = [vp, ci, ci]
        L.smvp_csr_get_kernel.argtypes = [vp, C.POINTER(ci), C.POINTER(ci)]
        L.smvp_csr_gather_spread.argtypes = [vp, C.POINTER(C.c_double)]
        L.smvp_csr_spmv.argtypes = [vp, vp, vp, vp]
        L.smvp_csr_describe.argtypes = [vp, C.c_char_p, C.c_size_t, C.POINTER(C.c_double)]
        L.smvp_csr_plan_launches.argtypes = [vp, C.POINTER(ci)]
        L.smvp_csr_plan_info.argtypes = [vp, C.POINTER(PlanInfo)]
        L.smvp_tjds_plan_info.argtypes = [vp, C.POINTER(PlanInfo)]
        L.smvp_csr_destroy.argtypes = [vp]
        L.smvp_csr_destroy.restype = None
        L.smvp_csr_spmm.argtypes = [vp, ci, vp, C.c_longlong, vp, C.c_longlong, vp]
        L.smvp_csr_spmm_describe.argtypes = [vp, ci, C.c_char_p, C.c_size_t, C.POINTER(C.c_double), C.POINTER(PlanInfo)]
        L.smvp_csr_create_transposed.argtypes = [C.POINTER(vp), vp, vp]
        L.smvp_csr_device_arrays.argtypes = [vp, C.POINTER(vp), C.POINTER(vp), C.POINTER(vp)]
        L.smvp_tjds_spmv_transposed.argtypes = [vp, vp, vp, vp]
        L.smvp_tjds_transposed_describe.argtypes = [vp, C.c_char_p, C.c_size_t, C.POINTER(C.c_double)]
        L.smvp_tjds_spmm_transposed.argtypes = [vp, ci, vp, C.c_longlong, vp, C.c_longlong, vp]
        L.smvp_tjds_spmm_transposed_describe.argtypes = [vp, ci, C.c_char_p, C.c_size_t, C.POINTER(C.c_double)]
        L.smvp_tjds_spmm.argtypes = [vp, ci, vp, C.c_longlong, vp, C.c_longlong, vp]
        L.smvp_tjds_spmm_describe.argtypes = [vp, ci, C.c_char_p, C.c_size_t, C.POINTER(C.c_double), C.POINTER(PlanInfo)]
        L.smvp_tjds_create.argtypes = [C.POINTER(vp), ci, ci, ci, ci, ci, vp, vp, vp, vp, ci]
        L.smvp_tjds_set_x.argtypes = [vp, vp, vp]
        L.smvp_tjds_zero_y.argtypes = [vp, vp, vp]
        L.smvp_tjds_spmv.argtypes = [vp, vp, vp]
        L.smvp_tjds_set_ref_quirks.argtypes = [vp, ci, ci, ci]
        L.smvp_tjds_set_mode.argtypes = [vp, ci]
        L.smvp_tjds_set_tile.argtypes = [vp, ci]
        L.smvp_tjds_set_value_cache.argtypes = [vp, ci]
        L.smvp_tjds_get_value_cache.argtypes = [vp, C.POINTER(ci), C.POINTER(C.c_longlong)]
        L.smvp_last_run_info.argtypes = [C.POINTER(RunInfo)]
        L.smvp_tjds_describe.argtypes = [vp, C.c_char_p, C.c_size_t, C.POINTER(C.c_double)]
        L.smvp_tjds_destroy.argtypes = [vp]
        L.smvp_tjds_destroy.restype = None
        L.smvp_csr_from_coo.argtypes = [vp, ci, ci, vp, vp, vp]
        L.smvp_tjds_from_coo.argtypes = [vp, ci, ci, ci, vp, vp, ci, vp, vp, C.POINTER(ci), C.POINTER(ci), C.POINTER(ci)]
        L.smvp_csr_sharded_create.argtypes = [C.POINTER(vp), ci, vp, ci, ci, ci, vp, vp, vp]
        L.smvp_tjds_sharded_create.argtypes = [C.POINTER(vp), ci, vp, vp, ci, ci, ci]
        L.smvp_csr_sharded_create_ex.argtypes = [C.POINTER(vp), ci, vp, ci, ci, ci, vp, vp, vp, C.POINTER(ShardOpts)]
        L.smvp_tjds_sharded_create_ex.argtypes = [C.POINTER(vp), ci, vp, vp, ci, ci, ci, C.POINTER(ShardOpts)]
        L.smvp_shard_opts_default.argtypes = [C.POINTER(ShardOpts)]
        L.smvp_shard_opts_default.restype = None
        L.smvp_sharded_layout.argtypes = [vp, C.POINTER(ci), vp, vp]
        L.smvp_sharded_set_csr_kernel.argtypes = [vp, ci, ci]
        L.smvp_sharded_probe_exchange.argtypes = [vp, ci]
        L.smvp_sharded_exchange_info.argtypes = [vp, C.POINTER(ci), C.POINTER(ci), vp, C.POINTER(ci)]
        L.smvp_sharded_set_exchange.argtypes = [vp, ci]
        L.smvp_sharded_set_x.argtypes = [vp, vp]
        L.smvp_sharded_spmv.argtypes = [vp, ci, ci]
        L.smvp_sharded_synchronize.argtypes = [vp, C.POINTER(C.c_double)]
        L.smvp_sharded_get_y.argtypes = [vp, ci, ci, vp]
        L.smvp_sharded_feed_back.argtypes = [vp, ci]
        L.smvp_sharded_info.argtypes = [vp, C.POINTER(ci), C.POINTER(ci)]
        L.smvp_sharded_destroy.argtypes = [vp]
        L.smvp_sharded_destroy.restype = None
        L.smvp_csr_from_coo_device.argtypes = [vp, ci, ci, ci, vp, vp, vp, vp]
        L.smvp_tjds_from_coo_device.argtypes = [vp, ci, ci, ci, vp, vp, ci, vp, vp, C.POINTER(ci), C.POINTER(ci),
                                                C.POINTER(ci), vp]
        L.smvp_csr_compute.argtypes = [vp, ci, ci, ci, ci, C.POINTER(RunOpts), vp, vp, C.POINTER(TimeStats)]
        L.smvp_tjds_compute.argtypes = [vp, ci, ci, ci, ci, C.POINTER(RunOpts), vp, vp, C.POINTER(TimeStats)]
        L.smvp_run_opts_default.argtypes = [C.POINTER(RunOpts)]
        L.smvp_run_opts_default.restype = None
        L.smvp_time_stats.argtypes = [vp, ci, C.POINTER(TimeStats)]
        L.smvp_generate_report_text.argtypes = [C.c_char_p, C.c_char_p, C.c_char_p, ci, ci, ci, vp,
                                                C.POINTER(TimeStats), C.c_ulong, C.c_char_p, C.c_size_t]
        i64, u64 = C.c_int64, C.c_uint64
        L.smvp_synth_row_lengths.argtypes = [ci, u64, i64, i64, ci, i64, i64, vp]
        L.smvp_synth_fill.argtypes = [ci, u64, i64, i64, ci, i64, i64, vp, vp, vp, ci]
        L.smvp_partition_rows.argtypes = [vp, ci, ci, vp]
        L.smvp_vector_random.argtypes = [vp, C.c_int64, C.c_uint64]
        L.smvp_mm_read_header_path.argtypes = [C.c_char_p, vp, C.POINTER(ci), C.POINTER(ci), C.POINTER(ci)]
        L.smvp_mm_read_coo_path.argtypes = [C.c_char_p, vp, ci, vp, C.POINTER(ci), C.POINTER(ci), C.POINTER(ci)]
        L.smvp_mm_expanded_count.argtypes = [vp, vp, ci, C.POINTER(ci)]
        L.smvp_mm_expand_symmetric.argtypes = [vp, vp, ci, ci, ci, vp, ci, C.POINTER(ci)]
        L.smvp_cache_write_csr.argtypes = [C.c_char_p, C.c_char_p, vp, ci, ci, ci, ci, vp, vp, vp]
        L.smvp_cache_read_header.argtypes = [C.c_char_p, C.c_char_p, vp, C.POINTER(ci), C.POINTER(ci), C.POINTER(ci), C.POINTER(ci)]
        L.smvp_cache_read_csr.argtypes = [C.c_char_p, ci, ci, vp, vp, vp]
        L.smvp_coo_from_csr.argtypes = [ci, vp, vp, vp, vp]
        L.smvp_cisr_coegen_path.argtypes = [vp, ci, ci, ci, C.c_char_p]
        L.smvp_device_count.argtypes = [C.POINTER(ci)]
        L.smvp_device_info.argtypes = [ci, C.c_char_p, C.c_size_t, C.POINTER(ci), C.POINTER(C.c_size_t)]
        _lib = L
    return _lib


def _check(code, where):
    if code != OK:
        raise SmvpError(code, where)


def _p(a):
    return a.ctypes.data_as(C.c_void_p)


def _arr(a, dtype):
    a = np.ascontiguousarray(a, dtype=dtype)
    return a if a.size else np.zeros(1, dtype=dtype)


def mm_read_header(path):
    tc = C.create_string_buffer(4)
    m, n, nz = C.c_int(), C.c_int(), C.c_int()
    rc = lib().smvp_mm_read_header_path(os.fsencode(path), C.cast(tc, C.c_void_p), C.byref(m), C.byref(n), C.byref(nz))
    return rc, tc.raw.decode(), m.value, n.value, nz.value


def mm_read_coo(path):
    rc, tc, m, n, nz = mm_read_header(path)
    _check(rc, "smvp_mm_read_header_path")
    coo = np.zeros(max(nz, 1), dtype=COO_DTYPE)
    tcb = C.create_string_buffer(4)
    mm, nn, nzz = C.c_int(), C.c_int(), C.c_int()
    _check(lib().smvp_mm_read_coo_path(os.fsencode(path), _p(coo), nz, C.cast(tcb, C.c_void_p), C.byref(mm),
                                       C.byref(nn), C.byref(nzz)), "smvp_mm_read_coo_path")
    return tcb.raw.decode(), mm.value, nn.value, coo[:nz]


def mm_expand_symmetric(typecode, coo, rows, cols):
    nnz = len(coo)
    coo = _arr(coo, COO_DTYPE)
    tc = C.create_string_buffer(typecode.encode()[:4].ljust(4), 4)
    want = C.c_int()
    _check(lib().smvp_mm_expanded_count(C.cast(tc, C.c_void_p), _p(coo), nnz, C.byref(want)), "smvp_mm_expanded_count")
    out = np.zeros(max(want.value, 1), dtype=COO_DTYPE)
    got = C.c_int()
    _check(lib().smvp_mm_expand_symmetric(C.cast(tc, C.c_void_p), _p(coo), nnz, rows, cols, _p(out), want.value,
                                          C.byref(got)), "smvp_mm_expand_symmetric")
    return out[:got.value]


def cache_write_csr(cache_path, mtx_path, typecode, rows, cols, row_ptr, col_ind, val, expanded=False):
    rp, ci, v = _arr(row_ptr, np.int32), _arr(col_ind, np.int32), _arr(val, np.float64)
    tc = C.create_string_buffer(typecode.encode()[:4].ljust(4), 4)
    _check(lib().smvp_cache_write_csr(os.fsencode(cache_path), os.fsencode(mtx_path), C.cast(tc, C.c_void_p), int(expanded),
                                      rows, cols, int(rp[rows]), _p(rp), _p(ci), _p(v)), "smvp_cache_write_csr")


def cache_read_csr(cache_path, mtx_path=None):
    tc = C.create_string_buffer(4)
    fl, m, n, nz = C.c_int(), C.c_int(), C.c_int(), C.c_int()
    _check(lib().smvp_cache_read_header(os.fsencode(cache_path), None if mtx_path is None else os.fsencode(mtx_path),
                                        C.cast(tc, C.c_void_p), C.byref(fl), C.byref(m), C.byref(n), C.byref(nz)),
           "smvp_cache_read_header")
    rp = np.zeros(m.value + 1, dtype=np.int32)
    ci = np.zeros(max(nz.value, 1), dtype=np.int32)
    v = np.zeros(max(nz.value, 1), dtype=np.float64)
    _check(lib().smvp_cache_read_csr(os.fsencode(cache_path), m.value, nz.value, _p(rp), _p(ci), _p(v)), "smvp_cache_read_csr")
    return tc.raw.decode(), bool(fl.value & 1), m.value, n.value, rp, ci[:nz.value], v[:nz.value]


def coo_from_csr(rows, row_ptr, col_ind, val):
    rp, ci, v = _arr(row_ptr, np.int32), _arr(col_ind, np.int32), _arr(val, np.float64)
    out = np.zeros(max(int(rp[rows]), 1), dtype=COO_DTYPE)
    _check(lib().smvp_coo_from_csr(rows, _p(rp), _p(ci), _p(v), _p(out)), "smvp_coo_from_csr")
    return out[:int(rp[rows])]


def cisr_coegen(coo, rows, slots, path):
    n = len(coo)
    _check(lib().smvp_cisr_coegen_path(_p(_arr(coo, COO_DTYPE)), rows, n, slots, os.fsencode(path)), "smvp_cisr_coegen_path")
    return open(path).read()


def make_coo(rows_idx, cols_idx, vals):
    coo = np.zeros(len(rows_idx), dtype=COO_DTYPE)
    coo["row"], coo["col"], coo["val"] = rows_idx, cols_idx, vals
    return coo


def csr_from_coo(coo, rows):
    coo = np.ascontiguousarray(coo, dtype=COO_DTYPE)
    nnz = len(coo)
    row_ptr = np.zeros(rows + 1, dtype=np.int32)
    col_ind = np.zeros(max(nnz, 1), dtype=np.int32)
    val = np.zeros(max(nnz, 1), dtype=np.float64)
    _check(lib().smvp_csr_from_coo(_p(_arr(coo, COO_DTYPE)), rows, nnz, _p(row_ptr), _p(col_ind), _p(val)),
           "smvp_csr_from_coo")
    return row_ptr, col_ind[:nnz], val[:nnz]


class TjdsArrays:
    """perm / start_pos / row_ind / val plus the two reference-quirk scalars."""


def tjds_from_coo(coo, rows, cols):
    coo = np.ascontiguousarray(coo, dtype=COO_DTYPE)
    nnz = len(coo)
    t = TjdsArrays()
    t.rows, t.cols, t.nnz = rows, cols, nnz
    perm = np.zeros(max(cols, 1), dtype=np.int32)
    cap = max(rows, nnz) + 2
    sp = np.zeros(cap, dtype=np.int32)
    row_ind = np.zeros(max(nnz, 1), dtype=np.int32)
    val = np.zeros(max(nnz, 1), dtype=np.float64)
    nd, rn, ls = C.c_int(), C.c_int(), C.c_int()
    _check(lib().smvp_tjds_from_coo(_p(_arr(coo, COO_DTYPE)), rows, cols, nnz, _p(perm), _p(sp), cap, _p(row_ind),
                                    _p(val), C.byref(nd), C.byref(rn), C.byref(ls)), "smvp_tjds_from_coo")
    t.num_diag, t.ref_num_tjdiag, t.last_diag_single = nd.value, rn.value, ls.value
    t.perm, t.start_pos = perm[:cols], sp[:t.num_diag + 1].copy()
    t.row_ind, t.val = row_ind[:nnz], val[:nnz]
    return t


def csr_from_coo_device(d_coo, rows, cols, nnz, stream=None):
    import torch

    _check_entries(nnz, "smvp_csr_from_coo_device")

    row_ptr = torch.empty(rows + 1, dtype=torch.int32, device=d_coo.device)
    col_ind = torch.empty(max(nnz, 1), dtype=torch.int32, device=d_coo.device)
    val = torch.empty(max(nnz, 1), dtype=torch.float64, device=d_coo.device)
    _check(lib().smvp_csr_from_coo_device(_dev_ptr(d_coo), rows, cols, nnz, _dev_ptr(row_ptr), _dev_ptr(col_ind),
                                          _dev_ptr(val), _stream_ptr(stream)), "smvp_csr_from_coo_device")
    return row_ptr, col_ind[:nnz], val[:nnz]


def tjds_from_coo_device(d_coo, rows, cols, nnz, stream=None):
    import torch

    _check_entries(nnz, "smvp_tjds_from_coo_device")

    t = TjdsArrays()
    t.rows, t.cols, t.nnz = rows, cols, nnz
    cap = max(rows, nnz) + 2
    perm = torch.empty(max(cols, 1), dtype=torch.int32, device=d_coo.device)
    sp = torch.empty(cap, dtype=torch.int32, device=d_coo.device)
    row_ind = torch.empty(max(nnz, 1), dtype=torch.int32, device=d_coo.device)
    val = torch.empty(max(nnz, 1), dtype=torch.float64, device=d_coo.device)
    nd, rn, ls = C.c_int(), C.c_int(), C.c_int()
    _check(lib().smvp_tjds_from_coo_device(_dev_ptr(d_coo), rows, cols, nnz, _dev_ptr(perm), _dev_ptr(sp), cap,
                                           _dev_ptr(row_ind), _dev_ptr(val), C.byref(nd), C.byref(rn), C.byref(ls),
                                           _stream_ptr(stream)), "smvp_tjds_from_coo_device")
    t.num_diag, t.ref_num_tjdiag, t.last_diag_single = nd.value, rn.value, ls.value
    t.perm, t.start_pos = perm[:cols], sp[:t.num_diag + 1]
    t.row_ind, t.val = row_ind[:nnz], val[:nnz]
    return t


def partition_rows(row_ptr, parts):
    row_ptr = np.ascontiguousarray(row_ptr, dtype=np.int32)
    bounds = np.zeros(parts + 1, dtype=np.int32)
    _check(lib().smvp_partition_rows(_p(row_ptr), len(row_ptr) - 1, parts, _p(bounds)), "smvp_partition_rows")
    return bounds


def vector_random(n, seed=67890):
    x = np.zeros(max(n, 1), dtype=np.float64)
    _check(lib().smvp_vector_random(_p(x), n, seed), "smvp_vector_random")
    return x[:n]


def synth_csr(kind, seed, rows_total, cols_total, param=0, row_begin=0, row_end=None, threads=None):
    row_end = rows_total if row_end is None else row_end
    n = row_end - row_begin
    lens = np.zeros(max(n, 1), dtype=np.int32)
    _check(lib().smvp_synth_row_lengths(kind, seed, rows_total, cols_total, param, row_begin, row_end, _p(lens)),
           "smvp_synth_row_lengths")
    row_ptr64 = np.zeros(n + 1, dtype=np.int64)
    np.cumsum(lens[:n], out=row_ptr64[1:])
    if row_ptr64[-1] >= 2 ** 31:
        raise ValueError("row block holds %d entries: 32-bit indices (the reference's) cannot address it" % row_ptr64[-1])
    row_ptr = row_ptr64.astype(np.int32)
    nnz = int(row_ptr[-1])
    col_ind = np.empty(max(nnz, 1), dtype=np.int32)
    val = np.empty(max(nnz, 1), dtype=np.float64)
    if threads is None:
        threads = max(1, min(16, (os.cpu_count() or 1)))
    _check(lib().smvp_synth_fill(kind, seed, rows_total, cols_total, param, row_begin, row_end, _p(row_ptr),
                                 _p(col_ind), _p(val), threads), "smvp_synth_fill")
    return row_ptr, col_ind[:nnz], val[:nnz]


def device_count():
    n = C.c_int()
    _check(lib().smvp_device_count(C.byref(n)), "smvp_device_count")
    return n.value


def device_info(device=0):
    name = C.create_string_buffer(256)
    cus, mem = C.c_int(), C.c_size_t()
    _check(lib().smvp_device_info(device, name, 256, C.byref(cus), C.byref(mem)), "smvp_device_info")
    return name.value.decode(), cus.value, mem.value


def _dev_ptr(t):
    if t is None:
        return None
    if isinstance(t, int):
        return C.c_void_p(t)
    return C.c_void_p(t.data_ptr())


def _stream_ptr(stream):
    if stream is None:
        return None
    if isinstance(stream, int):
        return C.c_void_p(stream)
    return C.c_void_p(stream.cuda_stream)


def spmm_operands(X, Y, rows, cols):
    for name, t, n in (("X", X, cols), ("Y", Y, rows)):
        if not hasattr(t, "stride") or not hasattr(t, "dim") or t.dim() != 2:
            raise ValueError("%s must be a 2-D tensor" % name)
        if str(t.dtype) != "torch.float64":
            raise ValueError("%s must be float64, not %s" % (name, t.dtype))
        if t.shape[0] != n:
            raise ValueError("%s has %d rows, the matrix needs %d" % (name, t.shape[0], n))
    k = X.shape[1]
    if k < 1 or Y.shape[1] != k:
        raise ValueError("X and Y need the same number of columns k >= 1 (X has %d, Y %d)" % (X.shape[1], Y.shape[1]))
    for name, t in (("X", X), ("Y", Y)):
        if t.stride(1) != 1 or t.stride(0) < k:
            raise ValueError("%s must be row-major with contiguous rows (stride(1) == 1, stride(0) >= k); its strides are %s"
                             % (name, tuple(t.stride())))
    return k, X.stride(0), Y.stride(0)


def transposed_operands(x, y, rows, cols):
    for name, t, n in (("x", x, rows), ("y", y, cols)):
        if not hasattr(t, "is_contiguous") or not hasattr(t, "numel"):
            raise ValueError("%s must be a tensor" % name)
        if str(t.dtype) != "torch.float64":
            raise ValueError("%s must be float64, not %s" % (name, t.dtype))
        if t.numel() != n:
            raise ValueError("%s has %d elements, the matrix needs %d" % (name, t.numel(), n))
        if not t.is_contiguous():
            raise ValueError("%s must be contiguous; its strides are %s" % (name, tuple(t.stride())))


class CsrMatrix:

    def __init__(self, rows, cols, row_ptr, col_ind, val, device=0, first_row=0):
        self.rows, self.cols = rows, cols
        self._h = C.c_void_p()
        self._keep = None
        if isinstance(row_ptr, np.ndarray):
            rp, ci, v = _arr(row_ptr, np.int32), _arr(col_ind, np.int32), _arr(val, np.float64)
            self.nnz = int(rp[rows]) if rows >= 0 else 0
            _check(lib().smvp_csr_create_block(C.byref(self._h), device, rows, cols, self.nnz, _p(rp), _p(ci), _p(v),
                                               MEM_HOST, None, int(first_row)), "smvp_csr_create_block")
        else:
            host_rp = _arr(row_ptr.cpu().numpy(), np.int32)
            self.nnz = int(host_rp[rows])
            self._keep = (row_ptr, col_ind, val)
            _check(lib().smvp_csr_create_block(C.byref(self._h), device, rows, cols, self.nnz, _dev_ptr(row_ptr),
                                               _dev_ptr(col_ind), _dev_ptr(val), MEM_DEVICE, _p(host_rp), int(first_row)),
                   "smvp_csr_create_block")

    def set_kernel(self, kernel, param=0):
        _check(lib().smvp_csr_set_kernel(self._h, kernel, param), "smvp_csr_set_kernel")

    def get_kernel(self):
        k, p = C.c_int(), C.c_int()
        _check(lib().smvp_csr_get_kernel(self._h, C.byref(k), C.byref(p)), "smvp_csr_get_kernel")
        return k.value, p.value

    def launches(self):
        n = C.c_int()
        _check(lib().smvp_csr_plan_launches(self._h, C.byref(n)), "smvp_csr_plan_launches")
        return n.value

    def plan_info(self):
        i = PlanInfo()
        _check(lib().smvp_csr_plan_info(self._h, C.byref(i)), "smvp_csr_plan_info")
        return {"matrix_bytes": i.matrix_bytes, "plan_bytes": i.plan_bytes, "build_ms": i.build_ms}

    def far_share(self):
        v = C.c_double()
        _check(lib().smvp_csr_far_share(self._h, C.byref(v)), "smvp_csr_far_share")
        return v.value

    def gather_spread(self):
        v = C.c_double()
        _check(lib().smvp_csr_gather_spread(self._h, C.byref(v)), "smvp_csr_gather_spread")
        return v.value

    def spmv(self, x, y, stream=None):
        _check(lib().smvp_csr_spmv(self._h, _dev_ptr(x), _dev_ptr(y), _stream_ptr(stream)), "smvp_csr_spmv")

    def describe(self):
        name = C.create_string_buffer(256)
        b = C.c_double()
        _check(lib().smvp_csr_describe(self._h, name, 256, C.byref(b)), "smvp_csr_describe")
        return name.value.decode(), b.value

    def spmm(self, X, Y, stream=None):
        k, ldx, ldy = spmm_operands(X, Y, self.rows, self.cols)
        if not (X.is_cuda and Y.is_cuda):
            raise ValueError("X and Y must be device tensors")
        _check(lib().smvp_csr_spmm(self._h, k, _dev_ptr(X), ldx, _dev_ptr(Y), ldy, _stream_ptr(stream)), "smvp_csr_spmm")

    def spmm_describe(self, k):
        name = C.create_string_buffer(256)
        b = C.c_double()
        i = PlanInfo()
        _check(lib().smvp_csr_spmm_describe(self._h, k, name, 256, C.byref(b), C.byref(i)), "smvp_csr_spmm_describe")
        return name.value.decode(), b.value, {"plan_bytes": i.plan_bytes, "build_ms": i.build_ms}

    @classmethod
    def _wrap(cls, handle, rows, cols, nnz):
        m = cls.__new__(cls)
        m.rows, m.cols, m.nnz = rows, cols, nnz
        m._h, m._keep = handle, None
        return m

    def transposed(self, stream=None):
        h = C.c_void_p()
        _check(lib().smvp_csr_create_transposed(C.byref(h), self._h, _stream_ptr(stream)), "smvp_csr_create_transposed")
        return CsrMatrix._wrap(h, self.cols, self.rows, self.nnz)

    def device_arrays(self):
        rp, ci, v = C.c_void_p(), C.c_void_p(), C.c_void_p()
        _check(lib().smvp_csr_device_arrays(self._h, C.byref(rp), C.byref(ci), C.byref(v)), "smvp_csr_device_arrays")
        return rp.value or 0, ci.value or 0, v.value or 0

    def close(self):
        if self._h:
            lib().smvp_csr_destroy(self._h)
            self._h = C.c_void_p()

    def __del__(self):
        try:
            self.close()
        except Exception:
            pass


class TjdsMatrix:

    def __init__(self, t, device=0):
        self.rows, self.cols, self.nnz = t.rows, t.cols, t.nnz
        self._t = t
        self._h = C.c_void_p()
        if isinstance(t.perm, np.ndarray):
            _check(lib().smvp_tjds_create(C.byref(self._h), device, t.rows, t.cols, t.nnz, t.num_diag,
                                          _p(_arr(t.perm, np.int32)), _p(_arr(t.start_pos, np.int32)),
                                          _p(_arr(t.row_ind, np.int32)), _p(_arr(t.val, np.float64)), MEM_HOST),
                   "smvp_tjds_create")
        else:
            _check(lib().smvp_tjds_create(C.byref(self._h), device, t.rows, t.cols, t.nnz, t.num_diag,
                                          _dev_ptr(t.perm), _dev_ptr(t.start_pos), _dev_ptr(t.row_ind),
                                          _dev_ptr(t.val), MEM_DEVICE), "smvp_tjds_create")

    def set_x(self, x, stream=None):
        _check(lib().smvp_tjds_set_x(self._h, _dev_ptr(x), _stream_ptr(stream)), "smvp_tjds_set_x")

    def zero_y(self, y, stream=None):
        _check(lib().smvp_tjds_zero_y(self._h, _dev_ptr(y), _stream_ptr(stream)), "smvp_tjds_zero_y")

    def spmv(self, y, stream=None):
        _check(lib().smvp_tjds_spmv(self._h, _dev_ptr(y), _stream_ptr(stream)), "smvp_tjds_spmv")

    def spmv_transposed(self, x, y, stream=None):
        transposed_operands(x, y, self.rows, self.cols)
        if not (x.is_cuda and y.is_cuda):
            raise ValueError("x and y must be device tensors")
        _check(lib().smvp_tjds_spmv_transposed(self._h, _dev_ptr(x), _dev_ptr(y), _stream_ptr(stream)),
               "smvp_tjds_spmv_transposed")

    def transposed_describe(self):
        name = C.create_string_buffer(128)
        b = C.c_double()
        _check(lib().smvp_tjds_transposed_describe(self._h, name, 128, C.byref(b)), "smvp_tjds_transposed_describe")
        return name.value.decode(), b.value

    def spmm_transposed(self, X, Y, stream=None):
        k, ldx, ldy = spmm_operands(X, Y, self.cols, self.rows)
        if not (X.is_cuda and Y.is_cuda):
            raise ValueError("X and Y must be device tensors")
        _check(lib().smvp_tjds_spmm_transposed(self._h, k, _dev_ptr(X), ldx, _dev_ptr(Y), ldy, _stream_ptr(stream)),
               "smvp_tjds_spmm_transposed")

    def spmm_transposed_describe(self, k):
        name = C.create_string_buffer(256)
        b = C.c_double()
        _check(lib().smvp_tjds_spmm_transposed_describe(self._h, k, name, 256, C.byref(b)), "smvp_tjds_spmm_transposed_describe")
        return name.value.decode(), b.value

    def spmm(self, X, Y, stream=None):
        k, ldx, ldy = spmm_operands(X, Y, self.rows, self.cols)
        if not (X.is_cuda and Y.is_cuda):
            raise ValueError("X and Y must be device tensors")
        _check(lib().smvp_tjds_spmm(self._h, k, _dev_ptr(X), ldx, _dev_ptr(Y), ldy, _stream_ptr(stream)), "smvp_tjds_spmm")

    def spmm_describe(self, k):
        name = C.create_string_buffer(256)
        b = C.c_double()
        i = PlanInfo()
        _check(lib().smvp_tjds_spmm_describe(self._h, k, name, 256, C.byref(b), C.byref(i)), "smvp_tjds_spmm_describe")
        return name.value.decode(), b.value, {"plan_bytes": i.plan_bytes, "build_ms": i.build_ms}

    def set_mode(self, mode):
        _check(lib().smvp_tjds_set_mode(self._h, mode), "smvp_tjds_set_mode")

    def set_tile(self, entries_per_tile):
        _check(lib().smvp_tjds_set_tile(self._h, entries_per_tile), "smvp_tjds_set_tile")

    def set_value_cache(self, min_tiles):
        _check(lib().smvp_tjds_set_value_cache(self._h, int(min_tiles)), "smvp_tjds_set_value_cache")

    def get_value_cache(self):
        m, n = C.c_int(), C.c_longlong()
        _check(lib().smvp_tjds_get_value_cache(self._h, C.byref(m), C.byref(n)), "smvp_tjds_get_value_cache")
        return m.value, n.value

    def plan_info(self):
        i = PlanInfo()
        _check(lib().smvp_tjds_plan_info(self._h, C.byref(i)), "smvp_tjds_plan_info")
        return {"matrix_bytes": i.matrix_bytes, "plan_bytes": i.plan_bytes, "build_ms": i.build_ms}

    def set_ref_quirks(self, enable=True):
        _check(lib().smvp_tjds_set_ref_quirks(self._h, int(enable), self._t.ref_num_tjdiag,
                                              self._t.last_diag_single), "smvp_tjds_set_ref_quirks")

    def describe(self):
        name = C.create_string_buffer(128)
        b = C.c_double()
        _check(lib().smvp_tjds_describe(self._h, name, 128, C.byref(b)), "smvp_tjds_describe")
        return name.value.decode(), b.value

    def close(self):
        if self._h:
            lib().smvp_tjds_destroy(self._h)
            self._h = C.c_void_p()

    def __del__(self):
        try:
            self.close()
        except Exception:
            pass


class ShardedMatrix:

    def __init__(self, fmt, ngpus, rows, cols, coo=None, csr=None, devices=None, chunks=0, balance=True, exchange=EXCHANGE_AUTO):
        self._h = C.c_void_p()
        devs = None if devices is None else (C.c_int * ngpus)(*devices)
        o = ShardOpts()
        lib().smvp_shard_opts_default(C.byref(o))
        o.chunks, o.balance, o.exchange = int(chunks), int(balance), int(exchange)
        if fmt == "csr":
            rp, ci, v = csr
            nnz = int(rp[rows])
            _check(lib().smvp_csr_sharded_create_ex(C.byref(self._h), ngpus, devs, rows, cols, nnz, _p(_arr(rp, np.int32)),
                                                    _p(_arr(ci, np.int32)), _p(_arr(v, np.float64)), C.byref(o)),
                   "smvp_csr_sharded_create_ex")
        else:
            nnz = len(coo)
            _check(lib().smvp_tjds_sharded_create_ex(C.byref(self._h), ngpus, devs, _p(_arr(coo, COO_DTYPE)), rows, cols,
                                                     nnz, C.byref(o)), "smvp_tjds_sharded_create_ex")
        self.rows, self.cols = rows, cols

    def layout(self):
        n, _ = self.info()
        c = C.c_int()
        _check(lib().smvp_sharded_layout(self._h, C.byref(c), None, None), "smvp_sharded_layout")
        bounds = np.zeros(n + 1, dtype=np.int32)
        cb = np.zeros(n * (c.value + 1), dtype=np.int32)
        _check(lib().smvp_sharded_layout(self._h, C.byref(c), _p(bounds), _p(cb)), "smvp_sharded_layout")
        return c.value, bounds, cb.reshape(n, c.value + 1)

    def set_csr_kernel(self, kernel, param=0):
        _check(lib().smvp_sharded_set_csr_kernel(self._h, kernel, param), "smvp_sharded_set_csr_kernel")

    def probe_exchange(self, reps=3):
        _check(lib().smvp_sharded_probe_exchange(self._h, int(reps)), "smvp_sharded_probe_exchange")
        return self.exchange_info()

    def exchange_info(self):
        act, av, rk = C.c_int(), C.c_int(), C.c_int()
        ms = (C.c_double * 3)()
        _check(lib().smvp_sharded_exchange_info(self._h, C.byref(act), C.byref(av), ms, C.byref(rk)), "smvp_sharded_exchange_info")
        return {"active": act.value, "active_name": EXCHANGE_NAMES[act.value],
                "available": [e for e in range(3) if av.value >> e & 1],
                "ms": {EXCHANGE_NAMES[e]: ms[e] for e in range(3) if ms[e] >= 0}, "rccl_ranks": rk.value}

    def set_exchange(self, exchange):
        _check(lib().smvp_sharded_set_exchange(self._h, int(exchange)), "smvp_sharded_set_exchange")

    def set_x(self, x=None):
        keep = None if x is None else _arr(x, np.float64)
        _check(lib().smvp_sharded_set_x(self._h, None if keep is None else _p(keep)), "smvp_sharded_set_x")

    def spmv(self, allgather=GATHER_OVERLAPPED, timed=True):
        _check(lib().smvp_sharded_spmv(self._h, int(allgather), int(timed)), "smvp_sharded_spmv")

    def feed_back(self, normalize=False):
        _check(lib().smvp_sharded_feed_back(self._h, int(normalize)), "smvp_sharded_feed_back")

    def synchronize(self):
        ms = C.c_double()
        _check(lib().smvp_sharded_synchronize(self._h, C.byref(ms)), "smvp_sharded_synchronize")
        return ms.value

    def get_y(self, slot=0, gathered=True):
        y = np.zeros(max(self.rows, 1), dtype=np.float64)
        _check(lib().smvp_sharded_get_y(self._h, slot, int(gathered), _p(y)), "smvp_sharded_get_y")
        return y[:self.rows]

    def info(self):
        n, b = C.c_int(), C.c_int()
        _check(lib().smvp_sharded_info(self._h, C.byref(n), C.byref(b)), "smvp_sharded_info")
        return n.value, b.value

    def close(self):
        if self._h:
            lib().smvp_sharded_destroy(self._h)
            self._h = C.c_void_p()

    def __del__(self):
        try:
            self.close()
        except Exception:
            pass


def _run_opts(device, csr_kernel, csr_param, ref_quirks, x, device_convert=False, ngpus=0, iterate=False,
              normalize=False, tjds_mode=TJDS_MODE_AUTO, timing=TIMING_AUTO, exchange=EXCHANGE_AUTO, repeat_patience_us=0):
    o = RunOpts()
    lib().smvp_run_opts_default(C.byref(o))
    o.device, o.csr_kernel, o.csr_param, o.tjds_ref_quirks = device, csr_kernel, csr_param, int(ref_quirks)
    o.convert_on_device, o.ngpus = int(device_convert), int(ngpus)
    o.iterate, o.normalize = int(iterate), int(normalize)
    o.tjds_mode, o.timing, o.shard_exchange = int(tjds_mode), int(timing), int(exchange)
    o.repeat_patience_us = int(repeat_patience_us)
    keep = None
    if x is not None:
        keep = _arr(x, np.float64)
        o.x = keep.ctypes.data
    return o, keep


def last_run_info():
    r = RunInfo()
    _check(lib().smvp_last_run_info(C.byref(r)), "smvp_last_run_info")
    return r


def csr_compute(coo, rows, cols, iters=1, device=0, kernel=CSR_KERNEL_AUTO, param=0, x=None, device_convert=False,
                ngpus=0, iterate=False, normalize=False, timing=TIMING_AUTO, exchange=EXCHANGE_AUTO, repeat_patience_us=0):
    nnz = len(coo)
    coo = _arr(coo, COO_DTYPE)
    y = np.zeros(max(rows, 1), dtype=np.float64)
    ms = np.zeros(iters, dtype=np.float64)
    st = TimeStats()
    o, keep = _run_opts(device, kernel, param, False, x, device_convert, ngpus, iterate, normalize, timing=timing, exchange=exchange,
                        repeat_patience_us=repeat_patience_us)
    _check(lib().smvp_csr_compute(_p(coo), rows, cols, nnz, iters, C.byref(o), _p(y), _p(ms), C.byref(st)),
           "smvp_csr_compute")
    return y[:rows], ms, st


def tjds_compute(coo, rows, cols, iters=1, device=0, ref_quirks=False, x=None, device_convert=False, ngpus=0,
                 iterate=False, normalize=False, mode=TJDS_MODE_AUTO, timing=TIMING_AUTO, exchange=EXCHANGE_AUTO, repeat_patience_us=0):
    nnz = len(coo)
    coo = _arr(coo, COO_DTYPE)
    y = np.zeros(max(rows, 1), dtype=np.float64)
    ms = np.zeros(iters, dtype=np.float64)
    st = TimeStats()
    o, keep = _run_opts(device, CSR_KERNEL_AUTO, 0, ref_quirks, x, device_convert, ngpus, iterate, normalize,
                        tjds_mode=mode, timing=timing, exchange=exchange, repeat_patience_us=repeat_patience_us)
    _check(lib().smvp_tjds_compute(_p(coo), rows, cols, nnz, iters, C.byref(o), _p(y), _p(ms), C.byref(st)),
           "smvp_tjds_compute")
    return y[:rows], ms, st


def time_stats(ms):
    ms = _arr(ms, np.float64)
    st = TimeStats()
    _check(lib().smvp_time_stats(_p(ms), len(ms), C.byref(st)), "smvp_time_stats")
    return st


def generate_report_text(input_name, report_dir, alg_name, nnz, y, iters, stats, unix_time=0):
    rows = len(y)
    y = _arr(y, np.float64)
    out = C.create_string_buffer(4096)
    _check(lib().smvp_generate_report_text(os.fsencode(input_name), os.fsencode(report_dir or ""),
                                           alg_name.encode(), nnz, rows, iters, _p(y), C.byref(stats),
                                           unix_time, out, 4096), "smvp_generate_report_text")
    return out.value.decode()
```

Measured before the change: 916.6 GFLOP/s.

## Add small-overflow owner kernel variant and optional balanced tile dealing

Adds a CSR stream-owner kernel instance whose shared-memory overflow buffer holds 256 entries instead of 1024. Overflow products past that limit are recomputed from global memory during the long-row reduction. A host heuristic, based on long-row share, mean row length and tile overflow lengths, picks this variant to cut LDS use and raise occupancy. An opt-in balanced tile-to-block mapping across the 8 XCDs is also added, and exposed through a new tile_plan query. For short-row matrices such as memplus, the heuristic likely keeps the original kernel, and the balanced mapping is off unless an option is set.

```diff
diff --git a/include/smvp_amd.h b/include/smvp_amd.h
--- a/include/smvp_amd.h
+++ b/include/smvp_amd.h
@@ -117,6 +117,7 @@
     double build_ms;
 } smvp_plan_info_t;
 int smvp_csr_plan_info(const smvp_csr_t *h, smvp_plan_info_t *out);
+int smvp_csr_tile_plan(const smvp_csr_t *h, int *stream_over, int *tile_group);
 int smvp_csr_spmm(smvp_csr_t *h, int k, const double *d_X, long long ldx, double *d_Y, long long ldy, void *stream);
 int smvp_csr_spmm_describe(const smvp_csr_t *h, int k, char *kernel_name, size_t cap, double *alg_bytes, smvp_plan_info_t *plan);
 int smvp_csr_create_transposed(smvp_csr_t **out, const smvp_csr_t *h, void *stream);
diff --git a/smvp-toolkit_amd/csrc/smvp_engine.hip b/smvp-toolkit_amd/csrc/smvp_engine.hip
--- a/smvp-toolkit_amd/csrc/smvp_engine.hip
+++ b/smvp-toolkit_amd/csrc/smvp_engine.hip
@@ -44,6 +44,7 @@
     int *d_run_ptr = nullptr, *d_run_tab = nullptr;
     int runs_total = 0;
     int sweep_alternate = 1, sweep_backward = 0;
+    int stream_over = smvp::kStreamOver, group = 0;
 };
 
 struct SweepPlan {
@@ -350,6 +351,37 @@
 
 constexpr double kSweepAlternateMinBytes = 256.0 * 1024 * 1024;
 
+constexpr double kStreamOverSmallMinLongShare = 0.12, kStreamOverSmallMinMeanRow = 10.0, kStreamOverSmallMaxTailShare = 0.5;
+
+static int choose_stream_over(const smvp_csr *h, int tile, const std::vector<int> &tile_row, const std::vector<int> &tile_next)
+{
+    if (h->kernel != SMVP_CSR_KERNEL_STREAM || h->flavor != smvp::kFlavorCsr || tile != 2048)
+        return smvp::kStreamOver;
+    const int forced = smvp::option("csr_stream_over", -1);
+    if (forced == smvp::kStreamOverSmall || forced == smvp::kStreamOver)
+        return forced;
+    const int *rp = h->h_row_ptr.data();
+    long long in_long_rows = 0;
+    if (h->max_row_len > smvp::kLongRow)
+        for (int r = 0; r < h->rows; ++r)
+            if (rp[r + 1] - rp[r] > smvp::kLongRow)
+                in_long_rows += rp[r + 1] - rp[r];
+    if ((double)in_long_rows <= kStreamOverSmallMinLongShare * (double)h->nnz && (double)h->nnz <= kStreamOverSmallMinMeanRow * (double)h->rows)
+        return smvp::kStreamOver;
+    const int ntiles = (int)tile_next.size();
+    long long owning = 0, long_tail = 0;
+    for (int b = 0; b < ntiles; ++b) {
+        if (tile_row[(size_t)b] == tile_row[(size_t)b + 1])
+            continue;
+        ++owning;
+        const long long e = std::min((long long)(b + 1) * tile, (long long)h->nnz);
+        const long long ext = tile_next[(size_t)b] - e;
+        if (ext > smvp::kStreamOverSmall && ext <= smvp::kStreamOver)
+            ++long_tail;
+    }
+    return (double)long_tail > kStreamOverSmallMaxTailShare * (double)owning ? smvp::kStreamOver : smvp::kStreamOverSmall;
+}
+
 int build_tile_plan(smvp_csr *h)
 {
     TilePlan &t = h->tile;
@@ -395,6 +427,9 @@
         HIP_TRY(hipMemset(t.d_carry, 0, std::max(ntiles, 1) * sizeof(double)));
     }
     t.ntiles = ntiles;
+    t.stream_over = choose_stream_over(h, tile, tile_row, tile_next);
+    const int rounds = smvp::option("csr_tile_rounds", -1);
+    t.group = h->kernel == SMVP_CSR_KERNEL_STREAM && h->flavor == smvp::kFlavorCsr && rounds > 0 ? smvp::tile_group_balanced(ntiles, rounds) : 0;
     const int alternate = smvp::option("csr_sweep_alternate", -1);
     t.sweep_alternate = alternate < 0 ? 12.0 * (double)h->nnz + 12.0 * h->rows + 8.0 * h->cols > kSweepAlternateMinBytes : alternate != 0;
     if (tile_ordered(h->flavor)) {
@@ -711,6 +746,7 @@
     l.rows = h->rows, l.nnz = h->nnz, l.ntiles = h->tile.ntiles;
     l.col16 = h->tile.d_col16, l.col_base = h->tile.d_col_base;
     l.row_rel = h->tile.d_row_rel;
+    l.over = h->tile.stream_over, l.tile_group = h->tile.group;
     l.unit_x = h->src.unit_operand ? 1 : 0;
 }
 
@@ -719,7 +755,7 @@
     if (!h || h->kernel != SMVP_CSR_KERNEL_STREAM || !h->tile.d_tile_row || h->rows <= 0)
         return 0;
     DeviceScope on(h->device);
-    return smvp::owner_repeat_grid(h->vpt, owner_flavor(h), h->tile.ntiles);
+    return smvp::owner_repeat_grid(h->vpt, owner_flavor(h), h->tile.ntiles, h->tile.group);
 }
 
 int smvp::csr_spmv_repeat(smvp_csr_t *h, const double *d_x, double *d_y, void *stream, unsigned long long *stamps, int reps, int grid,
@@ -802,7 +838,7 @@
 
 int smvp::csr_stamp_slots(const smvp_csr_t *h)
 {
-    return h && h->kernel == SMVP_CSR_KERNEL_STREAM && h->tile.d_tile_row ? smvp::owner_stamp_slots(h->tile.ntiles, h->flavor) : 0;
+    return h && h->kernel == SMVP_CSR_KERNEL_STREAM && h->tile.d_tile_row ? smvp::owner_stamp_slots(h->tile.ntiles, h->flavor, h->tile.group) : 0;
 }
 
 std::string smvp::csr_owner_kernel_name(const smvp_csr_t *h)
@@ -887,6 +923,18 @@
         b += h->flavor == smvp::kFlavorTjdsH ? 4.0 * n + 4.0 * (t + 2) + 8.0 * h->tile.runs_total + 2.0 * (n / 32 + 1) : 8.0 * n;
     }
     return b;
+}
+
+extern "C" int smvp_csr_tile_plan(const smvp_csr_t *h, int *stream_over, int *tile_group)
+{
+    if (!h)
+        return smvp::fail(SMVP_ERR_INVALID, "smvp_csr_tile_plan: null handle");
+    const bool on = h->kernel == SMVP_CSR_KERNEL_STREAM && h->tile.d_tile_row;
+    if (stream_over)
+        *stream_over = on ? h->tile.stream_over : 0;
+    if (tile_group)
+        *tile_group = on ? h->tile.group : 0;
+    return SMVP_OK;
 }
 
 extern "C" int smvp_csr_plan_info(const smvp_csr_t *h, smvp_plan_info_t *out)
diff --git a/smvp-toolkit_amd/csrc/smvp_error.cpp b/smvp-toolkit_amd/csrc/smvp_error.cpp
--- a/smvp-toolkit_amd/csrc/smvp_error.cpp
+++ b/smvp-toolkit_amd/csrc/smvp_error.cpp
@@ -34,6 +34,8 @@
     {"csr_col16", {-1}},
     {"csr_rowrel", {-1}},
     {"csr_sweep_alternate", {-1}},
+    {"csr_stream_over", {-1}},
+    {"csr_tile_rounds", {-1}},
     {"binned_near", {-1}},
     {"binned_overlap", {-1}},
     {"tjds_index", {-1}},
diff --git a/smvp-toolkit_amd/csrc/smvp_kernels.h b/smvp-toolkit_amd/csrc/smvp_kernels.h
--- a/smvp-toolkit_amd/csrc/smvp_kernels.h
+++ b/smvp-toolkit_amd/csrc/smvp_kernels.h
@@ -10,6 +10,7 @@
 constexpr int kStreamBlock = 256;
 constexpr int kLongRow = 32;
 constexpr int kStreamOver = 1024;
+constexpr int kStreamOverSmall = 256;
 constexpr int kStreamTileGroup = 64;
 constexpr int kTjdsTileGroup = 32;
 constexpr int kSweepBlock = 256;
@@ -76,15 +77,17 @@
     const unsigned short *row_rel = nullptr;
     int rows = 0, nnz = 0, ntiles = 0;
     int backward = 0;
+    int over = 0;
+    int tile_group = 0;
 };
 hipError_t launch_csr_stream_owner(int vpt, int flavor, const OwnerLaunch &l, hipStream_t stream);
 void debug_owner_phases();
 void debug_binned_phases();
-int owner_stamp_slots(int ntiles, int flavor);
+int owner_stamp_slots(int ntiles, int flavor, int plan_group);
 constexpr int kRepeatCtlWords = 32 * 66;
 constexpr unsigned kRepeatPatienceDefaultUs = 50000;
-int owner_repeat_grid(int vpt, int flavor, int ntiles);
-hipError_t launch_owner_csr_ilp(int vpt, int flavor, const OwnerLaunch &l, const void *extra, unsigned grid_x, int group, hipStream_t stream);
+int owner_repeat_grid(int vpt, int flavor, int ntiles, int plan_group);
+hipError_t launch_owner_csr_ilp(int vpt, int flavor, const OwnerLaunch &l, const void *extra, unsigned grid_x, int group_arg, hipStream_t stream);
 hipError_t launch_csr_stream_owner_repeat(int vpt, int flavor, const OwnerLaunch &l, int reps, int grid, unsigned *ctl_words,
                                           bool first_of_run, unsigned long long patience_ticks, hipStream_t stream);
 inline unsigned long long repeat_patience_ticks(int us) { return us < 0 ? 0ull : 100ull * (unsigned)(us ? us : (int)kRepeatPatienceDefaultUs); }
diff --git a/smvp-toolkit_amd/csrc/smvp_kernels.hip b/smvp-toolkit_amd/csrc/smvp_kernels.hip
--- a/smvp-toolkit_amd/csrc/smvp_kernels.hip
+++ b/smvp-toolkit_amd/csrc/smvp_kernels.hip
@@ -221,7 +221,7 @@
 #define SMVP_TJDS_NEUTRALISE 0
 #endif
 
-template <int VPT, int FLAVOR, bool STAMPED>
+template <int VPT, int FLAVOR, bool STAMPED, int OVER = kStreamOver>
 __device__ __forceinline__ void owner_body(
     const int *__restrict__ row_ptr, const int *__restrict__ col_ind, const double *__restrict__ val,
     const double *__restrict__ x, double *__restrict__ y, const int *__restrict__ tile_row,
@@ -229,14 +229,15 @@
 {
     const OwnerArgs a = {col_ind, val, x, ex.pos, ex.start_pos, ex.ovf_val, ex.ovf_k, FLAVOR == kFlavorTjdsH ? ex.unit_x : 0};
     constexpr int TILE = kStreamBlock * VPT;
-    constexpr int QCAP = (TILE + kStreamOver) / kLongRow + 1;
+    constexpr int QCAP = (TILE + OVER) / kLongRow + 1;
     constexpr bool CSR = FLAVOR == kFlavorCsr || FLAVOR == kFlavorCsr16;
     constexpr bool COL16 = FLAVOR == kFlavorCsr16;
     constexpr bool HALF = FLAVOR == kFlavorTjdsH;
     constexpr bool TJDS = FLAVOR == kFlavorTjdsK || FLAVOR == kFlavorTjdsS || HALF;
     constexpr bool SORTED = FLAVOR == kFlavorTjdsS || HALF;
     static_assert(TILE <= (1 << kSlotBits), "slot bits");
-    __shared__ double prod[TILE + kStreamOver];
+    static_assert(OVER >= kStreamBlock && OVER <= kStreamOver, "every lane's first overflow entry has its LDS slot");
+    __shared__ double prod[TILE + OVER];
     __shared__ int long_rows[QCAP];
     __shared__ int long_a[QCAP];
     __shared__ int long_z[QCAP];
@@ -263,7 +264,11 @@
         return;                                                   \
     } while (0)
 
-    const int b = tile_of_block_swept(block, tile_group_arg, ex.back_grid);
+    int b;
+    if constexpr (FLAVOR == kFlavorCsr || FLAVOR == kFlavorCsr16)
+        b = tile_of_block_dealt(block, tile_group_arg, ex.back_grid, ntiles);
+    else
+        b = tile_of_block_swept(block, tile_group_arg, ex.back_grid);
     if (b >= ntiles)
         SMVP_OWNER_EXIT();
     const int nnz = nnz_arg;
@@ -518,8 +523,9 @@
     }
     if (over0)
         prod[e - lo + t] = po;
+    const int ext_lds = OVER < kStreamOver && ext > OVER ? OVER : ext;
     if (!giant)
-        for (int i = t + kStreamBlock; i < ext; i += kStreamBlock)
+        for (int i = t + kStreamBlock; i < ext_lds; i += kStreamBlock)
             prod[e - lo + i] = owner_overflow_product<FLAVOR>(a, ovf_base, e, i);
     SMVP_PHASE(1);
     __syncthreads();
@@ -576,8 +582,27 @@
     for (int q = t >> 6; q < nlong; q += kStreamBlock / 64) {
         const int zq = long_z[q];
         double acc = 0.0;
-        for (int i = long_a[q] + lane; i < zq; i += 64)
-            acc += prod[i];
+        int i = long_a[q] + lane;
+        if constexpr (OVER < kStreamOver) {
+            const int zl = zq < TILE + OVER ? zq : TILE + OVER;
+            for (; i < zl; i += 64)
+                acc += prod[i];
+            for (; i < zq; i += 4 * 64) {
+                double pg[4];
+#pragma unroll
+                for (int u = 0; u < 4; ++u) {
+                    const int ii = i + u * 64;
+                    pg[u] = ii < zq ? owner_overflow_product<FLAVOR>(a, ovf_base, e, ii - (e - lo)) : 0.0;
+                }
+#pragma unroll
+                for (int u = 0; u < 4; ++u)
+                    if (i + u * 64 < zq)
+                        acc += pg[u];
+            }
+        } else {
+            for (; i < zq; i += 64)
+                acc += prod[i];
+        }
         acc = wave_sum_dpp(acc);
         if (lane == 0)
             y[long_rows[q]] = acc;
@@ -624,6 +649,18 @@
 {
     owner_body<VPT, FLAVOR, STAMPED>(row_ptr, col_ind, val, x, y, tile_row, tile_next, rows, nnz_arg, ntiles, tile_group_arg, ex,
                                      (int)blockIdx.x);
+}
+
+namespace over_small {
+template <int VPT, int FLAVOR, bool STAMPED>
+__global__ __launch_bounds__(kStreamBlock) __attribute__((amdgpu_waves_per_eu(STAMPED ? 8 : 1))) void csr_stream_owner(
+    const int *__restrict__ row_ptr, const int *__restrict__ col_ind, const double *__restrict__ val,
+    const double *__restrict__ x, double *__restrict__ y, const int *__restrict__ tile_row,
+    const int *__restrict__ tile_next, int rows, int nnz_arg, int ntiles, int tile_group_arg, const OwnerExtra ex)
+{
+    owner_body<VPT, FLAVOR, STAMPED, kStreamOverSmall>(row_ptr, col_ind, val, x, y, tile_row, tile_next, rows, nnz_arg, ntiles,
+                                                       tile_group_arg, ex, (int)blockIdx.x);
+}
 }
 
 #ifndef SMVP_TU_ILP
@@ -965,22 +1002,29 @@
 
 static int flavor_group(int flavor) { return flavor == kFlavorTjdsS || flavor == kFlavorTjdsH ? kTjdsTileGroup : kStreamTileGroup; }
 
-int owner_stamp_slots(int ntiles, int flavor)
-{
-    return (int)owner_grid(ntiles, tile_group(ntiles, flavor_group(flavor))) * (kStreamBlock / 64);
+static int launch_group(int ntiles, int flavor, int plan_group)
+{
+    return plan_group > 0 ? plan_group : tile_group(ntiles, flavor_group(flavor));
+}
+
+static int launch_group_arg(int group, int plan_group) { return plan_group > 0 ? -group : group; }
+
+int owner_stamp_slots(int ntiles, int flavor, int plan_group)
+{
+    return (int)owner_grid(ntiles, launch_group(ntiles, flavor, plan_group)) * (kStreamBlock / 64);
 }
 
 hipError_t launch_csr_stream_owner(int vpt, int flavor, const OwnerLaunch &l, hipStream_t stream)
 {
     if (l.rows <= 0)
         return hipSuccess;
-    const int group = tile_group(l.ntiles, flavor_group(flavor));
+    const int group = launch_group(l.ntiles, flavor, l.tile_group);
     const dim3 grid(owner_grid(l.ntiles, group));
     OwnerExtra ex = owner_extra_of(l, l.stamps);
     ex.back_grid = l.backward ? (int)grid.x : 0;
 #define SMVP_OWNER_ST(V, F, S)                                                                                     \
     hipLaunchKernelGGL((csr_stream_owner<V, F, S>), grid, dim3(kStreamBlock), 0, stream, l.row_ptr, l.col_ind, l.val, \
-                       l.x, l.y, l.tile_row, l.tile_next, l.rows, l.nnz, l.ntiles, group, ex)
+                       l.x, l.y, l.tile_row, l.tile_next, l.rows, l.nnz, l.ntiles, launch_group_arg(group, l.tile_group), ex)
 #define SMVP_OWNER(V, F)                  \
     if (vpt == V && flavor == F) {        \
         if (l.stamps)                     \
@@ -997,7 +1041,7 @@
     SMVP_OWNER(8, kFlavorCsr16)
 #else
     if (flavor == kFlavorCsr || flavor == kFlavorCsr16)
-        return launch_owner_csr_ilp(vpt, flavor, l, &ex, grid.x, group, stream);
+        return launch_owner_csr_ilp(vpt, flavor, l, &ex, grid.x, launch_group_arg(group, l.tile_group), stream);
 #endif
     SMVP_OWNER(1, kFlavorTjdsK)
     SMVP_OWNER(4, kFlavorTjdsK)
@@ -1029,7 +1073,7 @@
     X(1, kFlavorCsr) X(4, kFlavorCsr) X(8, kFlavorCsr) X(4, kFlavorCsr16) X(8, kFlavorCsr16) \
     X(1, kFlavorTjdsS) X(4, kFlavorTjdsS) X(8, kFlavorTjdsS) X(1, kFlavorTjdsH) X(4, kFlavorTjdsH) X(8, kFlavorTjdsH)
 
-int owner_repeat_grid(int vpt, int flavor, int ntiles)
+int owner_repeat_grid(int vpt, int flavor, int ntiles, int plan_group)
 {
     if (ntiles <= 0)
         return 0;
@@ -1041,7 +1085,7 @@
 #undef X
     if (cap <= 0)
         return 0;
-    const int full = (int)owner_grid(ntiles, tile_group(ntiles, flavor_group(flavor)));
+    const int full = (int)owner_grid(ntiles, launch_group(ntiles, flavor, plan_group));
     return full <= cap ? full : 0;
 }
 
@@ -1050,7 +1094,7 @@
 {
     if (l.rows <= 0)
         return hipSuccess;
-    const int group = tile_group(l.ntiles, flavor_group(flavor));
+    const int group = launch_group(l.ntiles, flavor, l.tile_group);
     RepeatCtl ctl{};
     ctl.sticky = ctl_words;
     ctl.shard = ctl_words + 32, ctl.go = ctl_words + 32 * (1 + kRepeatMaxShards), ctl.top = ctl_words + kRepeatCtlWords - 32;
@@ -1069,7 +1113,7 @@
 #define X(V, F)                                                                                                                    \
     if (vpt == V && flavor == F) {                                                                                                 \
         hipLaunchKernelGGL((csr_stream_owner_repeat<V, F>), dim3((unsigned)grid), dim3(kStreamBlock), 0, stream, l.row_ptr, l.col_ind, \
-                           l.val, l.x, l.y, l.tile_row, l.tile_next, l.rows, l.nnz, l.ntiles, group, ex, ctl);                     \
+                           l.val, l.x, l.y, l.tile_row, l.tile_next, l.rows, l.nnz, l.ntiles, launch_group_arg(group, l.tile_group), ex, ctl); \
         return hipGetLastError();                                                                                                  \
     }
     SMVP_REPEAT_FORMS(X)
@@ -1169,27 +1213,32 @@
 #ifdef SMVP_ILP_UNIT_UNUSED
 hipError_t launch_owner_csr_ilp(int, int, const OwnerLaunch &, const void *, unsigned, int, hipStream_t) { return hipErrorInvalidValue; }
 #else
-hipError_t launch_owner_csr_ilp(int vpt, int flavor, const OwnerLaunch &l, const void *extra, unsigned grid_x, int group, hipStream_t stream)
+hipError_t launch_owner_csr_ilp(int vpt, int flavor, const OwnerLaunch &l, const void *extra, unsigned grid_x, int group_arg, hipStream_t stream)
 {
     const OwnerExtra &ex = *static_cast<const OwnerExtra *>(extra);
     const dim3 grid(grid_x);
-#define SMVP_OWNER_ST(V, F, S)                                                                                     \
-    hipLaunchKernelGGL((csr_stream_owner<V, F, S>), grid, dim3(kStreamBlock), 0, stream, l.row_ptr, l.col_ind, l.val, \
-                       l.x, l.y, l.tile_row, l.tile_next, l.rows, l.nnz, l.ntiles, group, ex)
-#define SMVP_OWNER(V, F)                  \
-    if (vpt == V && flavor == F) {        \
-        if (l.stamps)                     \
-            SMVP_OWNER_ST(V, F, true);    \
-        else                              \
-            SMVP_OWNER_ST(V, F, false);   \
-        return hipGetLastError();         \
-    }
+    const int over = l.over > 0 ? l.over : kStreamOver;
+#define SMVP_OWNER_ST(K, V, F, S)                                                                            \
+    hipLaunchKernelGGL((K<V, F, S>), grid, dim3(kStreamBlock), 0, stream, l.row_ptr, l.col_ind, l.val, l.x, l.y, \
+                       l.tile_row, l.tile_next, l.rows, l.nnz, l.ntiles, group_arg, ex)
+#define SMVP_OWNER_O(K, V, F, O)                 \
+    if (vpt == V && flavor == F && over == O) {  \
+        if (l.stamps)                            \
+            SMVP_OWNER_ST(K, V, F, true);        \
+        else                                     \
+            SMVP_OWNER_ST(K, V, F, false);       \
+        return hipGetLastError();                \
+    }
+#define SMVP_OWNER(V, F) SMVP_OWNER_O(csr_stream_owner, V, F, kStreamOver)
+    SMVP_OWNER_O(over_small::csr_stream_owner, 8, kFlavorCsr, kStreamOverSmall)
+    SMVP_OWNER_O(over_small::csr_stream_owner, 8, kFlavorCsr16, kStreamOverSmall)
     SMVP_OWNER(1, kFlavorCsr)
     SMVP_OWNER(4, kFlavorCsr)
     SMVP_OWNER(8, kFlavorCsr)
     SMVP_OWNER(4, kFlavorCsr16)
     SMVP_OWNER(8, kFlavorCsr16)
 #undef SMVP_OWNER
+#undef SMVP_OWNER_O
 #undef SMVP_OWNER_ST
     return hipErrorInvalidValue;
 }
diff --git a/smvp-toolkit_amd/csrc/smvp_tile_map.h b/smvp-toolkit_amd/csrc/smvp_tile_map.h
--- a/smvp-toolkit_amd/csrc/smvp_tile_map.h
+++ b/smvp-toolkit_amd/csrc/smvp_tile_map.h
@@ -14,6 +14,15 @@
     return fit < 1 ? 1 : (fit < wanted ? fit : wanted);
 }
 
+inline int tile_group_balanced(int ntiles, int rounds)
+{
+    if (rounds < 1)
+        rounds = 1;
+    const long long per = 8ll * rounds;
+    const long long g = ((long long)ntiles + per - 1) / per;
+    return g < 1 ? 1 : (int)g;
+}
+
 inline unsigned tile_grid_of(int ntiles, int group) { return (unsigned)((ntiles + 8 * group - 1) / (8 * group)) * 8u * group; }
 
 SMVP_HOST_DEVICE inline __attribute__((always_inline)) int tile_of_block(int block, int group)
@@ -27,4 +36,22 @@
     return tile_of_block(back_grid ? back_grid - 1 - block : block, group);
 }
 
+SMVP_HOST_DEVICE inline __attribute__((always_inline)) int tile_of_block_balanced(int block, int group, int ntiles)
+{
+    const int xcd = block & 7, seq = block >> 3;
+    const int turns = (ntiles + 8 * group - 1) / (8 * group) * 8;
+    const int len = ntiles / turns, longer = ntiles - len * turns;
+    const int round = seq / group, at = seq - round * group, turn = round * 8 + xcd;
+    if (turn >= turns || at >= len + (turn < longer ? 1 : 0))
+        return ntiles;
+    return turn * len + (turn < longer ? turn : longer) + at;
 }
+
+SMVP_HOST_DEVICE inline __attribute__((always_inline)) int tile_of_block_dealt(int block, int group_arg, int back_grid, int ntiles)
+{
+    if (group_arg > 0)
+        return tile_of_block_swept(block, group_arg, back_grid);
+    return tile_of_block_balanced(back_grid ? back_grid - 1 - block : block, -group_arg, ntiles);
+}
+
+}
diff --git a/smvp-toolkit_amd/python/smvp_toolkit_amd/__init__.py b/smvp-toolkit_amd/python/smvp_toolkit_amd/__init__.py
--- a/smvp-toolkit_amd/python/smvp_toolkit_amd/__init__.py
+++ b/smvp-toolkit_amd/python/smvp_toolkit_amd/__init__.py
@@ -102,7 +102,7 @@
     "smvp_mm_read_header_path", "smvp_mm_read_coo_path", "smvp_mm_expanded_count", "smvp_mm_expand_symmetric",
     "smvp_cache_write_csr", "smvp_cache_read_header", "smvp_cache_read_csr", "smvp_coo_from_csr",
     "smvp_csr_from_coo", "smvp_tjds_from_coo", "smvp_csr_from_coo_device", "smvp_tjds_from_coo_device",
-    "smvp_device_count", "smvp_device_info", "smvp_csr_plan_info", "smvp_tjds_plan_info",
+    "smvp_device_count", "smvp_device_info", "smvp_csr_plan_info", "smvp_csr_tile_plan", "smvp_tjds_plan_info",
     "smvp_csr_create", "smvp_csr_create_block", "smvp_csr_far_share", "smvp_csr_set_kernel", "smvp_csr_get_kernel", "smvp_csr_gather_spread", "smvp_csr_spmv",
     "smvp_csr_describe", "smvp_csr_plan_launches", "smvp_csr_destroy", "smvp_csr_spmm", "smvp_csr_spmm_describe",
     "smvp_csr_create_transposed", "smvp_csr_device_arrays", "smvp_tjds_spmv_transposed", "smvp_tjds_transposed_describe",
@@ -140,6 +140,8 @@
         L.smvp_csr_describe.argtypes = [vp, C.c_char_p, C.c_size_t, C.POINTER(C.c_double)]
         L.smvp_csr_plan_launches.argtypes = [vp, C.POINTER(ci)]
         L.smvp_csr_plan_info.argtypes = [vp, C.POINTER(PlanInfo)]
+        if hasattr(L, "smvp_csr_tile_plan"):
+            L.smvp_csr_tile_plan.argtypes = [vp, C.POINTER(ci), C.POINTER(ci)]
         L.smvp_tjds_plan_info.argtypes = [vp, C.POINTER(PlanInfo)]
         L.smvp_csr_destroy.argtypes = [vp]
         L.smvp_csr_destroy.restype = None
@@ -500,6 +502,11 @@
         _check(lib().smvp_csr_plan_info(self._h, C.byref(i)), "smvp_csr_plan_info")
         return {"matrix_bytes": i.matrix_bytes, "plan_bytes": i.plan_bytes, "build_ms": i.build_ms}
 
+    def tile_plan(self):
+        o, g = C.c_int(), C.c_int()
+        _check(lib().smvp_csr_tile_plan(self._h, C.byref(o), C.byref(g)), "smvp_csr_tile_plan")
+        return {"stream_over": o.value, "tile_group": g.value}
+
     def far_share(self):
         v = C.c_double()
         _check(lib().smvp_csr_far_share(self._h, C.byref(v)), "smvp_csr_far_share")
```

New measurement: 888.9 GFLOP/s. -3.0%, worse.
